# michelerenzullo/Blur_algorithms

Hardware: AMD Instinct MI355X
Metric: megapixels/sec Gaussian blur (σ=20, 4K RGB) at 1/2/4/8 GPUs; % HBM roofline (higher is better)
Workload: dtype f16 hi+lo operands (u8 pixels exact, taps and intermediate split in two binary16 halves), f32 accumulate

## Files before the change

### blur_algorithms_amd/_lib.py

```python
import ctypes as C
import os

_HERE = os.path.dirname(os.path.abspath(__file__))
LIB_PATH = os.environ.get("BLUR_AMD_LIB") or os.path.join(_HERE, "libblur_amd.so")

BLUR_OK = 0
ERR_NAMES = {1: "BLUR_ERR_INVALID", 2: "BLUR_ERR_UNSUPPORTED", 3: "BLUR_ERR_HIP", 4: "BLUR_ERR_NOMEM"}


class BlurError(RuntimeError):
    def __init__(self, code, msg):
        super().__init__("%s (%d): %s" % (ERR_NAMES.get(code, "BLUR_ERR"), code, msg))
        self.code = code


class BlurOpts(C.Structure):
    _fields_ = [("nyquist_quirk", C.c_int), ("col_group", C.c_int), ("force_generic", C.c_int), ("frames_per_launch", C.c_int),
                ("row_major_planes", C.c_int), ("engine", C.c_int), ("tile_points", C.c_int), ("reserved", C.c_int * 1)]


_P = C.c_void_p
SYMBOLS = {
    "blur_opts_default": (None, [C.POINTER(BlurOpts)]),
    "blur_gaussian_window": (C.c_int, [C.c_double, C.c_int]),
    "blur_get_gaussian": (C.c_int, [_P, C.c_double, C.c_int, C.c_int]),
    "blur_is_valid_size": (C.c_int, [C.c_int]),
    "blur_nearest_transform_size": (C.c_int, [C.c_int]),
    "blur_pffft_sizing": (C.c_int, [C.c_int, C.c_int, C.c_double, C.POINTER(C.c_int)]),
    "blur_kernel_multipliers": (C.c_int, [C.c_double, C.c_int, C.c_int, _P]),
    "blur_fft_plan_radices": (C.c_int, [C.c_int, C.POINTER(C.c_int)]),
    "blur_ctx_create": (C.c_int, [C.POINTER(_P), C.c_int]),
    "blur_ctx_destroy": (C.c_int, [_P]),
    "blur_ctx_set_stream": (C.c_int, [_P, _P]),
    "blur_ctx_synchronize": (C.c_int, [_P]),
    "blur_last_error": (C.c_char_p, [_P]),
    "blur_last_engine": (C.c_int, [_P, C.c_char_p, C.c_size_t]),
    "blur_ctx_timing_enable": (C.c_int, [_P, C.c_int]),
    "blur_ctx_timing": (C.c_int, [_P, C.POINTER(C.c_double), C.POINTER(C.c_int), C.POINTER(C.c_int), C.c_int]),
    "blur_gaussian_u8c3_dev": (C.c_int, [_P, _P, _P, C.c_int, C.c_int, C.c_double, C.POINTER(BlurOpts)]),
    "blur_gaussian_u8c3_batch_dev": (C.c_int, [_P, _P, _P, C.c_int, C.c_int, C.c_int, C.c_double, C.POINTER(BlurOpts)]),
    "blur_gaussian_f32c1_dev": (C.c_int, [_P, _P, _P, C.c_int, C.c_int, C.c_double, C.POINTER(BlurOpts)]),
    "blur_gaussian_u8c3_host": (C.c_int, [_P, _P, _P, C.c_int, C.c_int, C.c_double, C.POINTER(BlurOpts)]),
    "blur_gaussian_u8c3_host_batch": (C.c_int, [_P, _P, _P, C.c_int, C.c_int, C.c_int, C.c_double, C.POINTER(BlurOpts)]),
    "blur_gaussian_u8_batch_dev": (C.c_int, [_P, _P, _P, C.c_int, C.c_int, C.c_int, C.c_int, C.c_double, C.POINTER(BlurOpts)]),
    "blur_gaussian_u8_dev": (C.c_int, [_P, _P, _P, C.c_int, C.c_int, C.c_int, C.c_double, C.POINTER(BlurOpts)]),
    "blur_gaussian_u8_host": (C.c_int, [_P, _P, _P, C.c_int, C.c_int, C.c_int, C.c_double, C.POINTER(BlurOpts)]),
    "blur_gaussian_f32_batch_dev": (C.c_int, [_P, _P, _P, C.c_int, C.c_int, C.c_int, C.c_int, C.c_double, C.POINTER(BlurOpts)]),
    "blur_gaussian_f32_dev": (C.c_int, [_P, _P, _P, C.c_int, C.c_int, C.c_int, C.c_double, C.POINTER(BlurOpts)]),
    "blur_gaussian_f32_host": (C.c_int, [_P, _P, _P, C.c_int, C.c_int, C.c_int, C.c_double, C.POINTER(BlurOpts)]),
    "blur_gaussian_u16_batch_dev": (C.c_int, [_P, _P, _P, C.c_int, C.c_int, C.c_int, C.c_int, C.c_double, C.POINTER(BlurOpts)]),
    "blur_gaussian_u16_dev": (C.c_int, [_P, _P, _P, C.c_int, C.c_int, C.c_int, C.c_double, C.POINTER(BlurOpts)]),
    "blur_gaussian_u16_host": (C.c_int, [_P, _P, _P, C.c_int, C.c_int, C.c_int, C.c_double, C.POINTER(BlurOpts)]),
    "blur_gaussian_f16_batch_dev": (C.c_int, [_P, _P, _P, C.c_int, C.c_int, C.c_int, C.c_int, C.c_double, C.POINTER(BlurOpts)]),
    "blur_gaussian_f16_dev": (C.c_int, [_P, _P, _P, C.c_int, C.c_int, C.c_int, C.c_double, C.POINTER(BlurOpts)]),
    "blur_gaussian_f16_host": (C.c_int, [_P, _P, _P, C.c_int, C.c_int, C.c_int, C.c_double, C.POINTER(BlurOpts)]),
    "blur_gaussian_bf16_batch_dev": (C.c_int, [_P, _P, _P, C.c_int, C.c_int, C.c_int, C.c_int, C.c_double, C.POINTER(BlurOpts)]),
    "blur_gaussian_bf16_dev": (C.c_int, [_P, _P, _P, C.c_int, C.c_int, C.c_int, C.c_double, C.POINTER(BlurOpts)]),
    "blur_gaussian_bf16_host": (C.c_int, [_P, _P, _P, C.c_int, C.c_int, C.c_int, C.c_double, C.POINTER(BlurOpts)]),
    "blur_gaussian_u8c3_host_pitched": (C.c_int, [_P, _P, C.c_size_t, _P, C.c_size_t, C.c_int, C.c_int, C.c_double, C.POINTER(BlurOpts)]),
    "blur_gaussian_f32c1_host": (C.c_int, [_P, _P, _P, C.c_int, C.c_int, C.c_double, C.POINTER(BlurOpts)]),
    "blur_separable_u8c3_dev": (C.c_int, [_P, _P, _P, C.c_int, C.c_int, _P, C.c_int, C.c_int, C.POINTER(BlurOpts)]),
    "blur_boxfft_u8c3_dev": (C.c_int, [_P, _P, _P, C.c_int, C.c_int, C.c_double, C.POINTER(BlurOpts)]),
    "blur_boxfft_sizing": (C.c_int, [C.c_int, C.c_int, C.c_double, C.POINTER(C.c_int)]),
    "blur_box_kernel": (C.c_int, [_P, C.c_int, C.c_int]),
    "blur_rowpass_u8c3_dev": (C.c_int, [_P, _P, _P, C.c_int, C.c_int, C.c_double, C.POINTER(BlurOpts)]),
    "blur_pocketfft2d_sizing": (C.c_int, [C.c_int, C.c_int, C.c_double, C.POINTER(C.c_int * 8)]),
    "blur_pocketfft2d_u8c3_dev": (C.c_int, [_P, _P, _P, C.c_int, C.c_int, C.c_double, C.c_int, _P]),
    "blur_pocketfft2d_u8c3_host": (C.c_int, [_P, _P, _P, C.c_int, C.c_int, C.c_double, C.c_int]),
    "blur_reflect101_u8_dev": (C.c_int, [_P, _P, _P, C.c_int, C.c_int, C.c_int, C.c_int, C.c_int, C.c_int, C.c_int, C.POINTER(C.c_int * 2)]),
    "blur_flip_block_f32_dev": (C.c_int, [_P, _P, _P, C.c_int, C.c_int]),
    "blur_deinterleave_bgr_u8_f32_dev": (C.c_int, [_P, _P, _P, C.c_uint32]),
    "blur_interleave_bgr_f32_u8_dev": (C.c_int, [_P, _P, _P, C.c_uint32]),
    "blur_fastboxblur_u8_dev": (C.c_int, [_P, _P, C.c_int, C.c_int, C.c_int, C.c_int, C.c_int]),
    "blur_fastboxblur_u8_host": (C.c_int, [_P, _P, C.c_int, C.c_int, C.c_int, C.c_int, C.c_int]),
    "blur_fastboxblur_u8_batch_dev": (C.c_int, [_P, _P, C.c_int, C.c_int, C.c_int, C.c_int, C.c_int, C.c_int]),
    "blur_fastboxblur_u8_host_batch": (C.c_int, [_P, _P, C.c_int, C.c_int, C.c_int, C.c_int, C.c_int, C.c_int]),
    "blur_fastboxblur_batch_plan": (C.c_int, [C.c_int, C.c_int, C.c_int, C.c_int, C.c_int, C.c_int, C.POINTER(C.c_int * 4)]),
    "blur_multi_create": (C.c_int, [C.POINTER(_P), C.POINTER(C.c_int), C.c_int]),
    "blur_multi_destroy": (C.c_int, [_P]),
    "blur_multi_shards": (C.c_int, [_P]),
    "blur_multi_last_error": (C.c_char_p, [_P]),
    "blur_gaussian_u8c3_batch_multi_dev": (C.c_int, [_P, _P, _P, C.c_int, C.c_int, C.c_int, C.c_double, C.POINTER(BlurOpts)]),
    "blur_gaussian_u8c3_batch_multi_host": (C.c_int, [_P, _P, _P, C.c_int, C.c_int, C.c_int, C.c_double, C.POINTER(BlurOpts)]),
    "blur_gaussian_u8_batch_multi_dev": (C.c_int, [_P, _P, _P, C.c_int, C.c_int, C.c_int, C.c_int, C.c_double, C.POINTER(BlurOpts)]),
    "blur_gaussian_u8_batch_multi_host": (C.c_int, [_P, _P, _P, C.c_int, C.c_int, C.c_int, C.c_int, C.c_double, C.POINTER(BlurOpts)]),
    "blur_gaussian_f32_batch_multi_dev": (C.c_int, [_P, _P, _P, C.c_int, C.c_int, C.c_int, C.c_int, C.c_double, C.POINTER(BlurOpts)]),
    "blur_gaussian_f32_batch_multi_host": (C.c_int, [_P, _P, _P, C.c_int, C.c_int, C.c_int, C.c_int, C.c_double, C.POINTER(BlurOpts)]),
    "blur_gaussian_u16_batch_multi_dev": (C.c_int, [_P, _P, _P, C.c_int, C.c_int, C.c_int, C.c_int, C.c_double, C.POINTER(BlurOpts)]),
    "blur_gaussian_u16_batch_multi_host": (C.c_int, [_P, _P, _P, C.c_int, C.c_int, C.c_int, C.c_int, C.c_double, C.POINTER(BlurOpts)]),
    "blur_gaussian_f16_batch_multi_dev": (C.c_int, [_P, _P, _P, C.c_int, C.c_int, C.c_int, C.c_int, C.c_double, C.POINTER(BlurOpts)]),
    "blur_gaussian_f16_batch_multi_host": (C.c_int, [_P, _P, _P, C.c_int, C.c_int, C.c_int, C.c_int, C.c_double, C.POINTER(BlurOpts)]),
    "blur_gaussian_bf16_batch_multi_dev": (C.c_int, [_P, _P, _P, C.c_int, C.c_int, C.c_int, C.c_int, C.c_double, C.POINTER(BlurOpts)]),
    "blur_gaussian_bf16_batch_multi_host": (C.c_int, [_P, _P, _P, C.c_int, C.c_int, C.c_int, C.c_int, C.c_double, C.POINTER(BlurOpts)]),
    "blur_gaussian_u8_sigmas_batch_dev": (C.c_int, [_P, _P, _P, C.c_int, C.c_int, C.c_int, C.c_int, C.POINTER(C.c_double), C.POINTER(BlurOpts)]),
    "blur_gaussian_u8_sigmas_dev": (C.c_int, [_P, _P, _P, C.c_int, C.c_int, C.c_int, C.POINTER(C.c_double), C.POINTER(BlurOpts)]),
    "blur_gaussian_u8_sigmas_host": (C.c_int, [_P, _P, _P, C.c_int, C.c_int, C.c_int, C.POINTER(C.c_double), C.POINTER(BlurOpts)]),
    "blur_gaussian_u8_sigmas_batch_multi_dev": (C.c_int, [_P, _P, _P, C.c_int, C.c_int, C.c_int, C.c_int, C.POINTER(C.c_double), C.POINTER(BlurOpts)]),
    "blur_gaussian_u8_sigmas_batch_multi_host": (C.c_int, [_P, _P, _P, C.c_int, C.c_int, C.c_int, C.c_int, C.POINTER(C.c_double), C.POINTER(BlurOpts)]),
    "blur_gaussian_f32_sigmas_batch_dev": (C.c_int, [_P, _P, _P, C.c_int, C.c_int, C.c_int, C.c_int, C.POINTER(C.c_double), C.POINTER(BlurOpts)]),
    "blur_gaussian_f32_sigmas_dev": (C.c_int, [_P, _P, _P, C.c_int, C.c_int, C.c_int, C.POINTER(C.c_double), C.POINTER(BlurOpts)]),
    "blur_gaussian_f32_sigmas_host": (C.c_int, [_P, _P, _P, C.c_int, C.c_int, C.c_int, C.POINTER(C.c_double), C.POINTER(BlurOpts)]),
    "blur_gaussian_f32_sigmas_batch_multi_dev": (C.c_int, [_P, _P, _P, C.c_int, C.c_int, C.c_int, C.c_int, C.POINTER(C.c_double), C.POINTER(BlurOpts)]),
    "blur_gaussian_f32_sigmas_batch_multi_host": (C.c_int, [_P, _P, _P, C.c_int, C.c_int, C.c_int, C.c_int, C.POINTER(C.c_double), C.POINTER(BlurOpts)]),
    "blur_gaussian_u16_sigmas_batch_dev": (C.c_int, [_P, _P, _P, C.c_int, C.c_int, C.c_int, C.c_int, C.POINTER(C.c_double), C.POINTER(BlurOpts)]),
    "blur_gaussian_u16_sigmas_dev": (C.c_int, [_P, _P, _P, C.c_int, C.c_int, C.c_int, C.POINTER(C.c_double), C.POINTER(BlurOpts)]),
    "blur_gaussian_u16_sigmas_host": (C.c_int, [_P, _P, _P, C.c_int, C.c_int, C.c_int, C.POINTER(C.c_double), C.POINTER(BlurOpts)]),
    "blur_gaussian_u16_sigmas_batch_multi_dev": (C.c_int, [_P, _P, _P, C.c_int, C.c_int, C.c_int, C.c_int, C.POINTER(C.c_double), C.POINTER(BlurOpts)]),
    "blur_gaussian_u16_sigmas_batch_multi_host": (C.c_int, [_P, _P, _P, C.c_int, C.c_int, C.c_int, C.c_int, C.POINTER(C.c_double), C.POINTER(BlurOpts)]),
    "blur_gaussian_f16_sigmas_batch_dev": (C.c_int, [_P, _P, _P, C.c_int, C.c_int, C.c_int, C.c_int, C.POINTER(C.c_double), C.POINTER(BlurOpts)]),
    "blur_gaussian_f16_sigmas_dev": (C.c_int, [_P, _P, _P, C.c_int, C.c_int, C.c_int, C.POINTER(C.c_double), C.POINTER(BlurOpts)]),
    "blur_gaussian_f16_sigmas_host": (C.c_int, [_P, _P, _P, C.c_int, C.c_int, C.c_int, C.POINTER(C.c_double), C.POINTER(BlurOpts)]),
    "blur_gaussian_f16_sigmas_batch_multi_dev": (C.c_int, [_P, _P, _P, C.c_int, C.c_int, C.c_int, C.c_int, C.POINTER(C.c_double), C.POINTER(BlurOpts)]),
    "blur_gaussian_f16_sigmas_batch_multi_host": (C.c_int, [_P, _P, _P, C.c_int, C.c_int, C.c_int, C.c_int, C.POINTER(C.c_double), C.POINTER(BlurOpts)]),
    "blur_gaussian_bf16_sigmas_batch_dev": (C.c_int, [_P, _P, _P, C.c_int, C.c_int, C.c_int, C.c_int, C.POINTER(C.c_double), C.POINTER(BlurOpts)]),
    "blur_gaussian_bf16_sigmas_dev": (C.c_int, [_P, _P, _P, C.c_int, C.c_int, C.c_int, C.POINTER(C.c_double), C.POINTER(BlurOpts)]),
    "blur_gaussian_bf16_sigmas_host": (C.c_int, [_P, _P, _P, C.c_int, C.c_int, C.c_int, C.POINTER(C.c_double), C.POINTER(BlurOpts)]),
    "blur_gaussian_bf16_sigmas_batch_multi_dev": (C.c_int, [_P, _P, _P, C.c_int, C.c_int, C.c_int, C.c_int, C.POINTER(C.c_double), C.POINTER(BlurOpts)]),
    "blur_gaussian_bf16_sigmas_batch_multi_host": (C.c_int, [_P, _P, _P, C.c_int, C.c_int, C.c_int, C.c_int, C.POINTER(C.c_double), C.POINTER(BlurOpts)]),
    "blur_gaussian_sigmas_plan": (C.c_int, [C.c_int, C.c_int, C.c_int, C.POINTER(C.c_double), C.POINTER(C.c_int)]),
    "blur_fastboxblur_u8_batch_multi_dev": (C.c_int, [_P, _P, C.c_int, C.c_int, C.c_int, C.c_int, C.c_int, C.c_int]),
    "blur_fastboxblur_u8_batch_multi_host": (C.c_int, [_P, _P, C.c_int, C.c_int, C.c_int, C.c_int, C.c_int, C.c_int]),
    "blur_convolve_lines_c32_dev": (C.c_int, [_P, _P, _P, C.c_int, C.c_int, _P]),
    "blur_wr_length": (C.c_int, [C.c_int, C.c_int]),
    "blur_mx_window_blocks": (C.c_int, [C.c_int]),
    "blur_mx_fragments": (C.c_int, [_P, C.c_int, C.c_int, _P]),
    "blur_wr_kernel_multipliers": (C.c_int, [C.c_double, C.c_int, C.c_int, C.c_int, C.c_int, _P]),
    "blur_malloc": (C.c_int, [_P, C.POINTER(_P), C.c_size_t]),
    "blur_free": (C.c_int, [_P, _P]),
    "blur_host_alloc": (C.c_int, [_P, C.POINTER(_P), C.c_size_t]),
    "blur_host_free": (C.c_int, [_P, _P]),
    "blur_copy_bandwidth": (C.c_int, [_P, C.c_size_t, C.c_int, C.POINTER(C.c_double)]),
    "blur_memcpy_h2d": (C.c_int, [_P, _P, _P, C.c_size_t]),
    "blur_memcpy_d2h": (C.c_int, [_P, _P, _P, C.c_size_t]),
}

_lib = None


def load():
    global _lib
    if _lib is not None:
        return _lib
    if not os.path.exists(LIB_PATH):
        raise ImportError(
            "blur_algorithms_amd: %s is missing -- build it with `python -c 'import __graft_entry__ as g; g.build()'` "
            "or `make -C blur_algorithms_amd/csrc` (hipcc, --offload-arch=gfx950). There is no CPU fallback." % LIB_PATH)
    try:
        import torch
    except Exception:
        pass
    lib = C.CDLL(LIB_PATH)
    for name, (res, args) in SYMBOLS.items():
        fn = getattr(lib, name)
        fn.restype = res
        fn.argtypes = args
    _lib = lib
    return lib
```

### blur_algorithms_amd/csrc/engine.hip

```cpp
#include <hip/hip_runtime.h>

#include <array>
#include <cmath>
#include <cstdio>
#include <cstdlib>
#include <cstring>
#include <functional>
#include <list>
#include <map>
#include <memory>
#include <string>
#include <tuple>
#include <type_traits>
#include <vector>

#include "../../include/blur_amd.h"
#include "fast_registry.hpp"
#include "fft_engine.hpp"
#include "host_math.hpp"
#define BLUR_MX_QUIRK_KERNELS
#include "mx_registry.hpp"
#define BLUR_FX_QUIRK_KERNELS
#include "fx_registry.hpp"
#include "bx_box.hpp"
// ... 449 lines not shown
                stream((x - r - 1) * C, sh_out, gout);
#pragma unroll
                for (int k = 0; k < C; ++k) res[k] = 0;
#pragma unroll
                for (int k = 0; k < 4 * C; ++k) {
                    acc[k % C] += byte_of(gin, k) - byte_of(gout, k);
                    const uint32_t v = static_cast<uint32_t>(static_cast<int>(static_cast<float>(acc[k % C]) * iarr + 0.5f)) & 0xffu;
                    res[k >> 2] |= v << (8 * (k & 3));
                }
#pragma unroll
                for (int k = 0; k < C; ++k) d32[((off0 + x * C) >> 2) + k] = res[k];
            }
        }
        uint8_t* t = a; a = b; b = t;
    }
    __syncthreads();
    if ((rb & 3) == 0 && (reinterpret_cast<uintptr_t>(dst) & 3) == 0) {
        for (int i = threadIdx.x; i < rb / 4; i += 256) reinterpret_cast<uint32_t*>(dst)[i] = reinterpret_cast<const uint32_t*>(a + off0)[i];
    } else {
        for (int i = threadIdx.x; i < rb; i += 256) dst[i] = a[off0 + i];
    }
}


struct Img2dGeom { int rows, cols, s0, s1, top, left; };

__global__ __launch_bounds__(256) void img2d_rows_fwd_kernel(const uint8_t* __restrict__ src, float2* __restrict__ z, Img2dGeom g, int ca, int cb,
                                                             DevPlan plan, const float2* __restrict__ tw)
{
    extern __shared__ float2 lds2d[];
    const int zs = line_stride(plan.n);
    const int y = blockIdx.x;
    const uint8_t* row = src + static_cast<size_t>(refl101(y - g.top, g.rows)) * g.cols * 3;
    for (int x = threadIdx.x; x < g.s1; x += blockDim.x) {
        const uint8_t* px = row + 3 * refl101(x - g.left, g.cols);
        lds2d[phys(x)] = make_float2(static_cast<float>(px[ca]), cb >= 0 ? static_cast<float>(px[cb]) : 0.f);
    }
    __syncthreads();
    fft_forward_lines<1>(lds2d, zs, plan, tw);
    float2* out = z + static_cast<size_t>(y) * g.s1;
    for (int pos = threadIdx.x; pos < g.s1; pos += blockDim.x) out[pos] = lds2d[phys(pos)];
}

template <int G, bool CONV>
__global__ __launch_bounds__(256) void img2d_cols_kernel(float2* __restrict__ z, int s0, int s1, DevPlan plan, const float2* __restrict__ tw,
                                                         const float* __restrict__ mcol, const float* __restrict__ krow_pos)
{
    extern __shared__ float2 lds2d[];
    const int zs = line_stride(plan.n);
    const int x0 = blockIdx.x * G;
    for (int idx = threadIdx.x; idx < s0 * G; idx += blockDim.x) {
        const int y = idx / G, c = idx - y * G, x = x0 + c;
        float2 v = make_float2(0.f, 0.f);
        if (x < s1) {
            v = z[static_cast<size_t>(y) * s1 + x];
            if (CONV) v = cscale(v, krow_pos[x]);
        }
        lds2d[c * zs + phys(y)] = v;
    }
    __syncthreads();
    if (CONV) fftconv_lines<G>(lds2d, zs, plan, tw, mcol);
    else fft_forward_lines<G>(lds2d, zs, plan, tw);
    for (int idx = threadIdx.x; idx < s0 * G; idx += blockDim.x) {
        const int y = idx / G, c = idx - y * G, x = x0 + c;
        if (x < s1) z[static_cast<size_t>(y) * s1 + x] = lds2d[c * zs + phys(y)];
    }
}

__global__ __launch_bounds__(256) void img2d_rows_inv_kernel(const float2* __restrict__ z, uint8_t* __restrict__ dst, float* __restrict__ planes, Img2dGeom g,
                                                             int ca, int cb, DevPlan plan, const float2* __restrict__ tw)
{
    extern __shared__ float2 lds2d[];
    const int zs = line_stride(plan.n);
    const int i = blockIdx.x;
    const float2* in = z + static_cast<size_t>(i + g.top) * g.s1;
    for (int pos = threadIdx.x; pos < g.s1; pos += blockDim.x) lds2d[phys(pos)] = in[pos];
    __syncthreads();
    fft_inverse_lines<1>(lds2d, zs, plan, tw);
    const size_t plane = static_cast<size_t>(g.rows) * g.cols;
    for (int j = threadIdx.x; j < g.cols; j += blockDim.x) {
        const float2 v = lds2d[phys(j + g.left)];
        const size_t px = static_cast<size_t>(i) * g.cols + j;
        dst[3 * px + ca] = static_cast<uint8_t>(static_cast<int>(v.x + 0.5f));
        if (cb >= 0) dst[3 * px + cb] = static_cast<uint8_t>(static_cast<int>(v.y + 0.5f));
        if (planes) {
            planes[ca * plane + px] = v.x;
            if (cb >= 0) planes[cb * plane + px] = v.y;
        }
    }
}

__global__ __launch_bounds__(256) void img2d_logspec_kernel(const float2* __restrict__ z, uint8_t* __restrict__ dst, float* __restrict__ planes, Img2dGeom g,
                                                            int ca, int cb, const int* __restrict__ pos_of_freq_y, const int* __restrict__ pos_of_freq_x)
{
    const size_t plane = static_cast<size_t>(g.rows) * g.cols;
    for (size_t px = blockIdx.x * 256u + threadIdx.x; px < plane; px += static_cast<size_t>(gridDim.x) * 256u) {
        const int i = static_cast<int>(px / g.cols), j = static_cast<int>(px - static_cast<size_t>(i) * g.cols);
        const int row = i + g.top, col = j + g.left;
        const int fy = (row + (g.s0 % 2 == 0 ? g.s0 : g.s0 + 1) / 2) % g.s0;
        const int col_ = (col + (g.s1 % 2 == 0 ? g.s1 : g.s1 + 1) / 2) % g.s1;
        const int fx = col_ < g.s1 / 2 + 1 ? col_ : g.s1 / 2 - col_ % (g.s1 / 2);
        const float2 p = z[static_cast<size_t>(pos_of_freq_y[fy]) * g.s1 + pos_of_freq_x[fx]];
        const float2 q = z[static_cast<size_t>(pos_of_freq_y[(g.s0 - fy) % g.s0]) * g.s1 + pos_of_freq_x[(g.s1 - fx) % g.s1]];
        const float va = 20.f * log10f(fabsf(0.5f * (p.x + q.x)) + 0.00001f);
        dst[3 * px + ca] = static_cast<uint8_t>(static_cast<int>(va + 0.5f));
        if (planes) planes[ca * plane + px] = va;
        if (cb >= 0) {
            const float vb = 20.f * log10f(fabsf(0.5f * (p.y + q.y)) + 0.00001f);
            dst[3 * px + cb] = static_cast<uint8_t>(static_cast<int>(vb + 0.5f));
            if (planes) planes[cb * plane + px] = vb;
        }
    }
}

__global__ __launch_bounds__(256) void copy16_kernel(const uint4* __restrict__ src, uint4* __restrict__ dst, size_t n16)
{
    for (size_t i = blockIdx.x * 256ull + threadIdx.x; i < n16; i += static_cast<size_t>(gridDim.x) * 256ull) dst[i] = src[i];
}

__global__ __launch_bounds__(256) void reflect101_u8_kernel(const uint8_t* __restrict__ in, uint8_t* __restrict__ out, int rows, int cols, int C,
                                                            int top, int left, int out_rows, int out_cols)
{
    const size_t total = static_cast<size_t>(out_rows) * out_cols;
    for (size_t px = blockIdx.x * 256u + threadIdx.x; px < total; px += static_cast<size_t>(gridDim.x) * 256u) {
        const int y = static_cast<int>(px / out_cols), x = static_cast<int>(px - static_cast<size_t>(y) * out_cols);
        const uint8_t* s = in + (static_cast<size_t>(refl101(y - top, rows)) * cols + refl101(x - left, cols)) * C;
        for (int c = 0; c < C; ++c) out[px * C + c] = s[c];
    }
}

}

struct DevicePlan {
    FftPlan host;
    DevPlan dev{};
    float2* d_tw = nullptr;
    const FastEntry* fast = nullptr;
    int key = 0;
    int* d_pos_of_freq = nullptr;
};

struct HostPipe {
    static constexpr int S = 3;
    hipStream_t h2d = nullptr, d2h = nullptr;
    uint8_t* buf[S] = { nullptr, nullptr, nullptr };
    size_t bytes = 0;
    hipEvent_t in_done[S] = {}, comp_done[S] = {}, out_done[S] = {};
    bool ready = false;
};

struct MxTables {
    void* frags_row = nullptr;
    void* frags_col = nullptr;
    float* taps_row = nullptr;
    float dr = 0.f, dc = 0.f;
};

struct blur_ctx {
    int device = 0;
    HostPipe pipe;
    hipStream_t stream = nullptr;
    std::string err;
    std::map<int, std::unique_ptr<DevicePlan>> plans;
    std::map<std::tuple<int, int, int, uint64_t>, float*> spectra;
    std::map<int, float*> last_spectrum;
    int num_cus = 256;
    int num_xcds = 8;
    float2* d_w256 = nullptr;
    std::map<int, float2*> wr_tw0;
    std::map<std::tuple<int, int, int, int, uint64_t>, float*> wr_spectra;
    struct LinesTable { uint64_t hash; std::vector<float> host; float* dev; };
    std::list<LinesTable> lines_tables;
    std::map<std::tuple<int, int, int, int, int, uint64_t>, MxTables> mx_tables;
    uint8_t* fx_strips = nullptr;
    size_t fx_strips_bytes = 0;
    int* fx_sums = nullptr;
    size_t fx_sums_bytes = 0;
    int* tl_sums = nullptr;
    size_t tl_sums_bytes = 0;
    float* tl_terms = nullptr;
    size_t tl_terms_bytes = 0;
    uint8_t* tl_copy = nullptr;
    size_t tl_copy_bytes = 0;
    std::map<std::pair<uint64_t, int>, float*> tl_taps;
    int* mx_sums = nullptr;
    size_t mx_sums_bytes = 0;
    float* mx_terms = nullptr;
    size_t mx_terms_bytes = 0;
    float* work = nullptr;
    size_t work_bytes = 0;
    float* work2 = nullptr;
    size_t work2_bytes = 0;
    uint8_t* box_tmp = nullptr;
    float* ch_planes = nullptr;
    size_t ch_planes_bytes = 0;
    uint8_t* ch_copy = nullptr;
    size_t ch_copy_bytes = 0;
    void* ff_sums = nullptr;
    size_t ff_sums_bytes = 0;
    void* ff_strips = nullptr;
    size_t ff_strips_bytes = 0;
    size_t box_bytes = 0;
    std::string engine_note;
    int last_family = -1;
    void* host_stage = nullptr;
    size_t host_stage_bytes = 0;
    int timing = 0;
    std::vector<std::tuple<hipEvent_t, hipEvent_t, int, int>> ev_busy;
    std::vector<std::pair<hipEvent_t, hipEvent_t>> ev_free;
    double ms[2] = { 0, 0 };
    int launches[2] = { 0, 0 };
    int frames[2] = { 0, 0 };
};

static thread_local std::string g_create_err;

#define HIP_TRY(ctx, call)                                                                          \
    do {                                                                                            \
        hipError_t e_ = (call);                                                                     \
        if (e_ != hipSuccess) {                                                                     \
            (ctx)->err = std::string(#call) + ": " + hipGetErrorString(e_);                         \
            return BLUR_ERR_HIP;                                                                    \
        }                                                                                           \
    } while (0)

static int fail(blur_ctx* ctx, int code, const char* msg)
{
    if (ctx) ctx->err = msg;
    return code;
}

static int get_plan(blur_ctx* ctx, int n, bool want_fast, bool column_role, DevicePlan** out)
{
    const FastEntry* fe = want_fast ? find_fast_entry(n, column_role) : nullptr;
    const int key = 4 * n + (fe ? (column_role ? 2 : 1) : 0);
    auto it = ctx->plans.find(key);
    if (it != ctx->plans.end()) { *out = it->second.get(); return BLUR_OK; }
    auto dp = std::make_unique<DevicePlan>();
    dp->fast = fe;
    dp->key = key;
    const bool ok = fe ? make_plan_radices(n, fe->radix, fe->npass, dp->host) : make_plan(n, dp->host);
    if (!ok) return fail(ctx, BLUR_ERR_UNSUPPORTED, "FFT length is not 2^a 3^b 5^c");
    dp->dev.n = n;
    dp->dev.npass = dp->host.npass;
    for (int i = 0; i < dp->host.npass; ++i) {
        dp->dev.radix[i] = dp->host.radix[i];
        dp->dev.m[i] = dp->host.m[i];
        dp->dev.tw_off[i] = dp->host.tw_off[i];
    }
    const size_t bytes = std::max<size_t>(dp->host.tw.size() * sizeof(float), 16);
    HIP_TRY(ctx, hipMalloc(reinterpret_cast<void**>(&dp->d_tw), bytes));
    if (!dp->host.tw.empty())
        HIP_TRY(ctx, hipMemcpy(dp->d_tw, dp->host.tw.data(), dp->host.tw.size() * sizeof(float), hipMemcpyHostToDevice));
    *out = dp.get();
    ctx->plans[key] = std::move(dp);
    return BLUR_OK;
}

static int get_spectrum(blur_ctx* ctx, const DevicePlan& plan, double sigma, int ksize, bool quirk, float** out)
{
    uint64_t bits;
    std::memcpy(&bits, &sigma, sizeof bits);
    const auto key = std::make_tuple(plan.key, ksize, quirk ? 1 : 0, bits);
    auto it = ctx->spectra.find(key);
    if (it != ctx->spectra.end()) { *out = it->second; return BLUR_OK; }
    const int n = plan.dev.n;
    std::vector<float> m(n / 2 + 1), mp(n);
    kernel_multipliers(sigma, ksize, n, m.data());
    permuted_multipliers(plan.host, m.data(), quirk, mp.data());
    float* d = nullptr;
    HIP_TRY(ctx, hipMalloc(reinterpret_cast<void**>(&d), sizeof(float) * (n + kStampTailFloats)));
    HIP_TRY(ctx, hipMemset(d, 0, sizeof(float) * (n + kStampTailFloats)));
    HIP_TRY(ctx, hipMemcpy(d, mp.data(), sizeof(float) * n, hipMemcpyHostToDevice));
    ctx->spectra[key] = d;
    ctx->last_spectrum[plan.key] = d;
    *out = d;
    return BLUR_OK;
}

static int get_spectrum_custom(blur_ctx* ctx, const DevicePlan& plan, const std::vector<float>& karr, bool quirk, float** out)
{
    uint64_t h = 1469598103934665603ull;
    const unsigned char* bytes = reinterpret_cast<const unsigned char*>(karr.data());
    for (size_t i = 0; i < karr.size() * sizeof(float); ++i) { h ^= bytes[i]; h *= 1099511628211ull; }
    const auto key = std::make_tuple(plan.key, -1, quirk ? 1 : 0, h);
    auto it = ctx->spectra.find(key);
    if (it != ctx->spectra.end()) { *out = it->second; return BLUR_OK; }
    const int n = plan.dev.n;
    std::vector<float> m(n / 2 + 1), mp(n);
    kernel_multipliers_from_array(karr.data(), n, m.data());
    permuted_multipliers(plan.host, m.data(), quirk, mp.data());
    float* d = nullptr;
    HIP_TRY(ctx, hipMalloc(reinterpret_cast<void**>(&d), sizeof(float) * (n + kStampTailFloats)));
    HIP_TRY(ctx, hipMemset(d, 0, sizeof(float) * (n + kStampTailFloats)));
    HIP_TRY(ctx, hipMemcpy(d, mp.data(), sizeof(float) * n, hipMemcpyHostToDevice));
    ctx->spectra[key] = d;
    ctx->last_spectrum[plan.key] = d;
    *out = d;
    return BLUR_OK;
}

static int ensure_host_stage(blur_ctx* ctx, size_t bytes, void** out)
{
    if (ctx->host_stage_bytes < bytes) {
        if (ctx->host_stage) { HIP_TRY(ctx, hipStreamSynchronize(ctx->stream)); HIP_TRY(ctx, hipFree(ctx->host_stage)); ctx->host_stage = nullptr; ctx->host_stage_bytes = 0; }
        HIP_TRY(ctx, hipMalloc(&ctx->host_stage, bytes ? bytes : 1));
// ... 120 lines not shown
        if (int rc = set_lds(ctx, colpass_kernel<OutT, CH, C, 512>, lds)) return rc;
        hipLaunchKernelGGL((colpass_kernel<OutT, CH, C, 512>), dim3(grid), dim3(512), lds, ctx->stream, planes, dst, rows, cols, pad, dv, plan.d_tw, mperm, strips);
    } else {
        if (int rc = set_lds(ctx, colpass_kernel<OutT, CH, C>, lds)) return rc;
        hipLaunchKernelGGL((colpass_kernel<OutT, CH, C>), dim3(grid), dim3(kThreads), lds, ctx->stream, planes, dst, rows, cols, pad, dv, plan.d_tw, mperm, strips);
    }
    HIP_TRY(ctx, hipGetLastError());
    return BLUR_OK;
}

static int colpass_lines(int n, int rows, int col_group, int obpp)
{
    int C = col_group > 0 ? col_group / 2 : 4;
    if (C >= 8) C = 8; else if (C >= 4) C = 4; else if (C >= 2) C = 2; else C = 1;
    while (C > 1 && col_lds_bytes(n, C, rows, obpp) > kLdsLimit) C /= 2;
    return col_lds_bytes(n, C, rows, obpp) > kLdsLimit ? 0 : C;
}

template <typename OutT, int CH>
static int launch_colpass(blur_ctx* ctx, const float* planes, OutT* dst, int rows, int cols, int pad,
                          const DevicePlan& plan, const float* mperm, int col_group, int strips = 0)
{
    const int C = colpass_lines(plan.dev.n, rows, col_group, sizeof(OutT) == 1 ? CH : 0);
    if (!C) return fail(ctx, BLUR_ERR_UNSUPPORTED, "column FFT length exceeds LDS capacity");
    switch (C) {
    case 8: return launch_colpass_c<OutT, CH, 8>(ctx, planes, dst, rows, cols, pad, plan, mperm, strips);
    case 4: return launch_colpass_c<OutT, CH, 4>(ctx, planes, dst, rows, cols, pad, plan, mperm, strips);
    case 2: return launch_colpass_c<OutT, CH, 2>(ctx, planes, dst, rows, cols, pad, plan, mperm, strips);
    default: return launch_colpass_c<OutT, CH, 1>(ctx, planes, dst, rows, cols, pad, plan, mperm, strips);
    }
}

struct Prepared {
    Sizing sz;
    DevicePlan *row = nullptr, *col = nullptr;
    float *m_row = nullptr, *m_col = nullptr;
    int col_group = 0;
    int col_fast_c = 0;
    int tile_w = 0;
    size_t frame_elems = 0;
    int gen_gshift = 0;
    const WrEntry *wr_col = nullptr, *wr_row = nullptr;
    float2 *wr_tw0_col = nullptr, *wr_tw0_row = nullptr;
    float *wr_m_col = nullptr, *wr_m_row = nullptr;
    const MxEntry* mx = nullptr;
    const FxEntry* fx = nullptr;
    const MxTables* mxt = nullptr;
    int mx_vpitch = 0;
    bool mx_quirk = false;
    struct Span { int in0, in1, padmode, v0, v1; };
    std::vector<Span> bands, tiles;
    const WrEntry *tl_col = nullptr;
    std::vector<const WrEntry*> tl_row;
    std::vector<float*> tl_m_row;
    std::vector<float2*> tl_tw0_row;
    float* tl_m_col = nullptr;
    float2* tl_tw0_col = nullptr;
    float tl_dr = 0.f, tl_dc = 0.f;
    float* tl_taps = nullptr;
    bool tiled = false, tl_quirk = false;
};

struct CustomKernel {
    const float* taps = nullptr;
    int ksize = 0;
    int pad = 0;
    int box_klen = 0;
};

static int wr_get_tables(blur_ctx* ctx, const WrEntry* e, float2** tw0)
{
    if (!ctx->d_w256) {
        std::vector<float> w(512);
        wr_w256(w.data());
        HIP_TRY(ctx, hipMalloc(reinterpret_cast<void**>(&ctx->d_w256), w.size() * sizeof(float)));
        HIP_TRY(ctx, hipMemcpy(ctx->d_w256, w.data(), w.size() * sizeof(float), hipMemcpyHostToDevice));
    }
    auto it = ctx->wr_tw0.find(e->r0);
    if (it == ctx->wr_tw0.end()) {
        std::vector<float> t(static_cast<size_t>(e->r0 - 1) * kWrS * 2 + 2);
        wr_tw0(e->r0, t.data());
        float2* d = nullptr;
        HIP_TRY(ctx, hipMalloc(reinterpret_cast<void**>(&d), t.size() * sizeof(float)));
        HIP_TRY(ctx, hipMemcpy(d, t.data(), t.size() * sizeof(float), hipMemcpyHostToDevice));
        it = ctx->wr_tw0.emplace(e->r0, d).first;
    }
    *tw0 = it->second;
    return BLUR_OK;
}

static int wr_get_spectrum(blur_ctx* ctx, const std::tuple<int, int, int, int, uint64_t>& key, const std::vector<float>& karr, int n, int n_ref, bool quirk, float** out)
{
    auto it = ctx->wr_spectra.find(key);
    if (it != ctx->wr_spectra.end()) { *out = it->second; return BLUR_OK; }
    std::vector<float> m(n);
    wr_multipliers(karr.data(), n, n_ref, quirk, m.data());
    float* d = nullptr;
    HIP_TRY(ctx, hipMalloc(reinterpret_cast<void**>(&d), sizeof(float) * (n + kWrStampTailFloats)));
    HIP_TRY(ctx, hipMemset(d, 0, sizeof(float) * (n + kWrStampTailFloats)));
    HIP_TRY(ctx, hipMemcpy(d, m.data(), sizeof(float) * n, hipMemcpyHostToDevice));
    ctx->wr_spectra[key] = d;
    ctx->last_spectrum[-n] = d;
    *out = d;
    return BLUR_OK;
}

static uint64_t fnv1a(const void* data, size_t bytes)
{
    uint64_t h = 1469598103934665603ull;
    const unsigned char* b = static_cast<const unsigned char*>(data);
    for (size_t i = 0; i < bytes; ++i) { h ^= b[i]; h *= 1099511628211ull; }
    return h;
}

static int mx_get_tables(blur_ctx* ctx, int nkb, double sigma, const Sizing& sz, const CustomKernel* ck, const MxTables** out, bool quiet = false)
{
    auto refuse = [&](int code, const char* msg) { return quiet ? code : fail(ctx, code, msg); };
    const int pad = sz.pad;
    std::vector<float> karr[2];
    const int nn[2] = { sz.n_row, sz.n_col };
    uint64_t tag;
    int kkey;
    auto build_arrays = [&]() -> int {
        for (int ax = 0; ax < 2; ++ax) {
            const int n = nn[ax];
            if (ck) {
                karr[ax].assign(n, 0.f);
                if (ck->box_klen > 0) box_kernel_1d(karr[ax].data(), ck->box_klen, n);
                else {
                    if (ck->ksize > n) return refuse(BLUR_ERR_INVALID, "kernel longer than the padded line");
                    const int c = ck->ksize / 2;
                    for (int t = 0; t < ck->ksize; ++t) karr[ax][(t - c + n) % n] += ck->taps[t];
                }
            } else {
                karr[ax].assign(std::max(n, sz.kSize), 0.f);
                get_gaussian(karr[ax].data(), sigma, sz.kSize, n);
            }
        }
        return BLUR_OK;
    };
    if (ck) {
        if (int rc = build_arrays()) return rc;
        kkey = -1;
        tag = fnv1a(karr[0].data(), nn[0] * sizeof(float)) ^ (fnv1a(karr[1].data(), nn[1] * sizeof(float)) * 3);
    } else { kkey = sz.kSize; std::memcpy(&tag, &sigma, sizeof tag); }
    const auto key = std::make_tuple(kkey, pad, nkb, nn[0], nn[1], tag);
    auto it = ctx->mx_tables.find(key);
    if (it != ctx->mx_tables.end()) { *out = &it->second; return BLUR_OK; }
    if (!ck) { if (int rc = build_arrays()) return rc; }
    MxTables t;
    auto release = [&]() {
        if (t.frags_row) (void)hipFree(t.frags_row);
        if (t.frags_col) (void)hipFree(t.frags_col);
        if (t.taps_row) (void)hipFree(t.taps_row);
    };
    for (int ax = 0; ax < 2; ++ax) {
        const int n = nn[ax];
        std::vector<float> taps(2 * pad + 1);
        for (int k = -pad; k <= pad; ++k) taps[k + pad] = karr[ax][(k + n) % n];
        for (int i = pad + 1; i < n - pad; ++i)
            if (karr[ax][i] != 0.f) { release(); return refuse(BLUR_ERR_UNSUPPORTED, "matrix-core engine: kernel wider than 2 pad + 1"); }
        {
            double sum = 0;
            bool neg = false;
            for (float t : taps) { sum += t; neg = neg || t < 0.f; }
            if (neg || sum > 1.0005) { release(); return refuse(BLUR_ERR_UNSUPPORTED, "matrix-core engine: taps must be non-negative with sum <= 1"); }
        }
        std::vector<uint16_t> fr(static_cast<size_t>(2) * nkb * 512);
        mx_fragments(taps.data(), pad, nkb, fr.data());
        long double k0 = 0, kalt = 0;
        for (int i = 0; i < n; ++i) { k0 += karr[ax][i]; kalt += (i & 1) ? -static_cast<long double>(karr[ax][i]) : static_cast<long double>(karr[ax][i]); }
        const float scaler = 1.f / n;
        const float m0 = static_cast<float>(k0) * scaler, mh = static_cast<float>(kalt) * scaler;
        void* dfr = nullptr;
        hipError_t e = hipMalloc(&dfr, fr.size() * sizeof(uint16_t));
        if (e == hipSuccess) {
            (ax ? t.frags_col : t.frags_row) = dfr;
            e = hipMemcpy(dfr, fr.data(), fr.size() * sizeof(uint16_t), hipMemcpyHostToDevice);
        }
        if (e == hipSuccess && ax == 0) {
            e = hipMalloc(reinterpret_cast<void**>(&t.taps_row), taps.size() * sizeof(float));
            if (e == hipSuccess) e = hipMemcpy(t.taps_row, taps.data(), taps.size() * sizeof(float), hipMemcpyHostToDevice);
        }
        if (e != hipSuccess) {
            release();
            (void)hipGetLastError();
            if (!quiet) ctx->err = std::string("matrix-core tables: ") + hipGetErrorString(e);
            return BLUR_ERR_HIP;
        }
        (ax ? t.dc : t.dr) = m0 - mh;
    }
    *out = &(ctx->mx_tables[key] = t);
    return BLUR_OK;
}

struct FftFamilyChoice {
    const WrEntry* wc = nullptr;
    const WrEntry* wr = nullptr;
    bool fits = false;
    bool old_both = false;
    bool wr_pays = false;
};
static FftFamilyChoice fft_family_choice(int rows, int cols, const Sizing& sz)
{
    FftFamilyChoice c;
    c.wc = find_wr_entry(rows + 2 * sz.pad, true);
    c.wr = find_wr_entry(cols + 2 * sz.pad, false);
    c.old_both = find_fast_entry(sz.n_col, true) && find_fast_entry(sz.n_row, false);
    c.fits = c.wc && c.wr && c.wc->col_lds(rows) <= kLdsLimit && c.wr->row_lds(cols) <= kLdsLimit;
    if (c.fits) {
        const int need_c = rows + 2 * sz.pad, need_r = cols + 2 * sz.pad, nc = c.wc->r0 * kWrS, nr = c.wr->r0 * kWrS;
        c.wr_pays = c.old_both ? (c.wc->r0 >= 8 && c.wr->r0 >= 12 && 4 * need_c >= 3 * nc && 4 * need_r >= 3 * nr) : (2 * need_c >= nc && 2 * need_r >= nr);
    }
    return c;
}

static bool plan_spans(int len, int pad, int nmax, int in_max, int align, std::vector<Prepared::Span>& out, bool equal_middle = false, bool edge_max = false)
{
    out.clear();
    if (in_max > nmax) in_max = nmax;
    if (len + 2 * pad <= nmax && len <= in_max) { out.push_back({ 0, len, pad, 0, len }); return true; }
    const int halo = (pad + align - 1) / align * align;
    const int le = std::min(nmax - 2 * pad, in_max), lm = in_max;
    int ve = (le - halo) / align * align, vm = (lm - halo - pad) / align * align;
    if (ve <= 0 || vm <= 0) return false;
    int nsp0 = 2;
    if (len > 2 * ve) nsp0 += (len - 2 * ve + vm - 1) / vm;
    std::vector<int> b;
    int nsp = 0, sm_equal = 0;
    for (int tries = 0; tries < 4 && nsp == 0; ++tries) {
        const int n = nsp0 + tries;
        b.assign(n + 1, 0);
        b[n] = len;
        int e = edge_max ? ve : static_cast<int>(static_cast<long long>(len) / n) / align * align;
        if (e > ve) e = ve;
        if (2 * e >= len) e = (len / 2) / align * align;
        if (e < align) e = align;
        b[1] = e;
        const int rest = len - 2 * e;
        if (equal_middle && n > 2) {
            const int unit = align % 2 == 0 ? align : 2 * align;
            const int sm = ((rest + (n - 2) - 1) / (n - 2) + unit - 1) / unit * unit;
            if (sm > vm || e + (n - 2) * sm + pad > len) continue;
            for (int i = 2; i < n; ++i) b[i] = e + (i - 1) * sm;
            b[n - 1] = len - e;
            if (b[n - 1] <= b[n - 2] - sm) continue;
            nsp = n;
            sm_equal = sm;
            break;
        }
        for (int i = 2; i < n; ++i) b[i] = (e + static_cast<int>(static_cast<long long>(rest) * (i - 1) / (n - 2))) / align * align;
        b[n - 1] = std::max(b[n - 1], (len - ve + align - 1) / align * align);
        bool ok = len - b[n - 1] <= ve && len - b[n - 1] > 0 && b[1] <= ve;
        for (int i = 1; i < n && ok; ++i) ok = b[i] > b[i - 1];
        for (int i = 1; i + 1 < n && ok; ++i) ok = b[i + 1] - b[i] <= vm;
        if (ok) nsp = n;
    }
    if (nsp == 0) return false;
    for (int i = 0; i < nsp; ++i) {
        Prepared::Span sp;
        sp.v0 = b[i];
        sp.v1 = b[i + 1];
        if (i == 0) { sp.in0 = 0; sp.in1 = std::min(len, sp.v1 + pad); sp.padmode = pad; }
        else if (i == nsp - 1) { sp.in0 = sp.v0 - halo; sp.in1 = len; sp.padmode = pad; }
        else {
            if (sm_equal > 0) sp.v1 = sp.v0 + sm_equal;
            sp.in0 = sp.v0 - halo; sp.in1 = std::min(len, sp.v1 + pad); sp.padmode = 0;
        }
        if (sp.in0 < 0 || sp.in1 - sp.in0 + 2 * sp.padmode > nmax || sp.in1 - sp.in0 > in_max || sp.padmode > sp.in1 - sp.in0 - 1) return false;
        out.push_back(sp);
    }
    return true;
}

static float quirk_gain(const float* karr, int n)
{
    long double k0 = 0, kalt = 0;
    for (int i = 0; i < n; ++i) { k0 += karr[i]; kalt += (i & 1) ? -static_cast<long double>(karr[i]) : static_cast<long double>(karr[i]); }
    const float scaler = 1.f / n;
    return static_cast<float>(k0) * scaler - static_cast<float>(kalt) * scaler;
}

static int plan_tiled(blur_ctx* ctx, int rows, int cols, double sigma, bool quirk, int tile_points, Prepared& p)
{
    const int pad = p.sz.pad;
    long long best = -1;
    for (int r0 : { 16, 15, 12, 10, 9, 8, 6, 5, 4, 3 }) {
        const int n = r0 * kWrS;
        if (tile_points > 0 && n > tile_points) continue;
        const WrEntry* e = find_wr_entry(n, true);
        if (!e || e->r0 != r0) continue;
        int in_max = n;
        while (in_max > 0 && e->col_lds(in_max) > kLdsLimit) in_max -= 8;
        std::vector<Prepared::Span> sp;
        if (in_max <= 0 || !plan_spans(rows, pad, n, in_max, 1, sp, true)) continue;
        const long long cost = static_cast<long long>(sp.size()) * n;
        if (best < 0 || cost < best) { best = cost; p.bands = sp; p.tl_col = e; }
    }
    if (best < 0) return BLUR_ERR_UNSUPPORTED;
    best = -1;
    for (int r0 : { 16, 15, 12, 10, 9, 8, 6, 5, 4, 3 }) {
        const int n = r0 * kWrS;
        if (tile_points > 0 && n > tile_points) continue;
        const WrEntry* e = find_wr_entry(n, false);
        if (!e || e->r0 != r0) continue;
        int in_max = n;
        while (in_max > 0 && e->row_lds(in_max) > kLdsLimit) in_max -= 16;
        if (in_max <= 0) continue;
        for (int variant = 0; variant < 2; ++variant) {
            std::vector<Prepared::Span> sp;
            if (!plan_spans(cols, pad, n, in_max, 16, sp, false, variant == 1)) continue;
            long long cost = 0;
            for (const Prepared::Span& t : sp) {
                const WrEntry* te = find_wr_entry(t.in1 - t.in0 + 2 * t.padmode, false);
                cost += te ? te->r0 * kWrS : 1 << 20;
            }
            if (best < 0 || cost < best) { best = cost; p.tiles = sp; }
        }
    }
    if (best < 0) return BLUR_ERR_UNSUPPORTED;
    uint64_t bits;
    std::memcpy(&bits, &sigma, sizeof bits);
    auto spectrum = [&](int n, float** out) -> int {
        const auto key = std::make_tuple(n, 0, p.sz.kSize, 0, bits);
        std::vector<float> karr(n, 0.f);
        if (ctx->wr_spectra.find(key) == ctx->wr_spectra.end()) {
            std::vector<float> k(std::max(n, p.sz.kSize));
            get_gaussian(k.data(), sigma, p.sz.kSize, n);
            std::copy(k.begin(), k.begin() + n, karr.begin());
        }
        return wr_get_spectrum(ctx, key, karr, n, n, false, out);
// ... 738 lines not shown
    }
    ctx->last_family = note.empty() ? 6 : 0;
    ctx->engine_note = note;
    return BLUR_OK;
}

template <typename T>
static int blur_ch_sigmas_host(blur_ctx* ctx, const T* src, T* dst, int rows, int cols, int channels, const double* sigmas, const blur_opts* opts)
{
    SigmaGroups sg;
    if (int rc = check_ch_sigmas_args(ctx, src, dst, 1, rows, cols, channels, sigmas, sg)) return rc;
    HIP_TRY(ctx, hipSetDevice(ctx->device));
    const size_t bytes = static_cast<size_t>(rows) * cols * channels * sizeof(T), half = (bytes + 255) & ~static_cast<size_t>(255);
    void* dv = nullptr;
    if (int rc0 = ensure_host_stage(ctx, 2 * half, &dv)) return rc0;
    char* d = static_cast<char*>(dv);
    int rc = BLUR_OK;
    hipError_t e = hipMemcpyAsync(d, src, bytes, hipMemcpyHostToDevice, ctx->stream);
    if (e == hipSuccess) rc = blur_ch_sigmas_batch_impl(ctx, reinterpret_cast<const T*>(d), reinterpret_cast<T*>(d + half), 1, rows, cols, channels, sigmas, opts);
    if (e == hipSuccess && rc == BLUR_OK) e = hipMemcpyAsync(dst, d + half, bytes, hipMemcpyDeviceToHost, ctx->stream);
    if (e == hipSuccess) e = hipStreamSynchronize(ctx->stream);
    if (e != hipSuccess) { ctx->err = std::string("host blur: ") + hipGetErrorString(e); return BLUR_ERR_HIP; }
    return rc;
}

static int get_pos_of_freq(blur_ctx* ctx, DevicePlan* dp, const int** out)
{
    if (!dp->d_pos_of_freq) {
        const int n = dp->dev.n;
        std::vector<int> inv(n);
        for (int pos = 0; pos < n; ++pos) inv[dp->host.freq_of_pos[pos]] = pos;
        HIP_TRY(ctx, hipMalloc(reinterpret_cast<void**>(&dp->d_pos_of_freq), sizeof(int) * n));
        HIP_TRY(ctx, hipMemcpy(dp->d_pos_of_freq, inv.data(), sizeof(int) * n, hipMemcpyHostToDevice));
    }
    *out = dp->d_pos_of_freq;
    return BLUR_OK;
}

template <bool CONV>
static int launch_img2d_cols(blur_ctx* ctx, float2* z, int s0, int s1, const DevicePlan& plan, const float* mcol, const float* krow_pos)
{
    const size_t line = static_cast<size_t>(line_stride(s0)) * sizeof(float2);
    int G = 8;
    while (G > 1 && G * line > kLdsLimit) G >>= 1;
    if (G * line > kLdsLimit) return fail(ctx, BLUR_ERR_UNSUPPORTED, "2D path: column FFT length exceeds LDS capacity");
    const int grid = (s1 + G - 1) / G;
#define BLUR_IMG2D_COLS(G_)                                                                                                        \
    case G_:                                                                                                                        \
        if (int rc = set_lds(ctx, img2d_cols_kernel<G_, CONV>, G_ * line)) return rc;                                              \
        hipLaunchKernelGGL((img2d_cols_kernel<G_, CONV>), dim3(grid), dim3(kThreads), G_ * line, ctx->stream, z, s0, s1, plan.dev, \
                           plan.d_tw, mcol, krow_pos);                                                                             \
        break;
    switch (G) {
        BLUR_IMG2D_COLS(8)
        BLUR_IMG2D_COLS(4)
        BLUR_IMG2D_COLS(2)
        BLUR_IMG2D_COLS(1)
    }
#undef BLUR_IMG2D_COLS
    HIP_TRY(ctx, hipGetLastError());
    return BLUR_OK;
}

extern "C" {

void blur_opts_default(blur_opts* o)
{
    if (!o) return;
    std::memset(o, 0, sizeof *o);
    o->nyquist_quirk = 1;
}

int blur_gaussian_window(double sigma, int max_width) { return gaussian_window(sigma, max_width); }

int blur_get_gaussian(float* kernel, double sigma, int width, int fft_length)
{
    if (!kernel || !(sigma > 0) || width < 0 || fft_length < 0) return BLUR_ERR_INVALID;
    get_gaussian(kernel, sigma, width, fft_length);
    return BLUR_OK;
}

int blur_is_valid_size(int n) { return is_valid_size(n); }
int blur_nearest_transform_size(int n) { return nearest_transform_size(n); }

int blur_pffft_sizing(int rows, int cols, double sigma, int out[6])
{
    if (!out || rows <= 0 || cols <= 0 || !(sigma > 0)) return BLUR_ERR_INVALID;
    const Sizing s = pffft_sizing(rows, cols, sigma);
    out[0] = s.kSize; out[1] = s.pad; out[2] = s.n_col; out[3] = s.n_row; out[4] = s.tz_col; out[5] = s.tz_row;
    return BLUR_OK;
}

int blur_kernel_multipliers(double sigma, int ksize, int n, float* m)
{
    if (!m || !(sigma > 0) || ksize <= 0 || n < ksize) return BLUR_ERR_INVALID;
    kernel_multipliers(sigma, ksize, n, m);
    return BLUR_OK;
}

int blur_wr_kernel_multipliers(double sigma, int ksize, int n, int n_ref, int quirk, float* m)
{
    if (!m || !(sigma > 0) || ksize <= 0 || n < ksize || (n & 1) || n_ref <= 0) return BLUR_ERR_INVALID;
    std::vector<float> k(std::max(n, ksize));
    get_gaussian(k.data(), sigma, ksize, n);
    wr_multipliers(k.data(), n, n_ref, quirk != 0, m);
    return BLUR_OK;
}

int blur_fft_plan_radices(int n, int* radices)
{
    FftPlan p;
    if (!radices || !make_plan(n, p)) return 0;
    for (int i = 0; i < p.npass; ++i) radices[i] = p.radix[i];
    return p.npass;
}

int blur_ctx_create(blur_ctx** out, int device)
{
    if (!out) return BLUR_ERR_INVALID;
    *out = nullptr;
    int count = 0;
    hipError_t e = hipGetDeviceCount(&count);
    if (e != hipSuccess || count <= 0) {
        g_create_err = std::string("no HIP device available: ") + (e != hipSuccess ? hipGetErrorString(e) : "device count is 0");
        return BLUR_ERR_HIP;
    }
    if (device < 0 || device >= count) { g_create_err = "device ordinal out of range"; return BLUR_ERR_INVALID; }
    e = hipSetDevice(device);
    if (e != hipSuccess) { g_create_err = std::string("hipSetDevice: ") + hipGetErrorString(e); return BLUR_ERR_HIP; }
    blur_ctx* c = new blur_ctx();
    c->device = device;
    hipDeviceProp_t prop;
    if (hipGetDeviceProperties(&prop, device) == hipSuccess && prop.multiProcessorCount > 0) c->num_cus = prop.multiProcessorCount;
    int xccs = 0;
    if (hipDeviceGetAttribute(&xccs, hipDeviceAttributeNumberOfXccs, device) == hipSuccess && xccs > 0) c->num_xcds = xccs;
    *out = c;
    return BLUR_OK;
}

int blur_ctx_destroy(blur_ctx* ctx)
{
    if (!ctx) return BLUR_ERR_INVALID;
    (void)hipSetDevice(ctx->device);
    (void)hipStreamSynchronize(ctx->stream);
    for (auto& kv : ctx->plans) {
        if (kv.second->d_tw) (void)hipFree(kv.second->d_tw);
        if (kv.second->d_pos_of_freq) (void)hipFree(kv.second->d_pos_of_freq);
    }
    for (auto& kv : ctx->spectra) (void)hipFree(kv.second);
    if (ctx->d_w256) (void)hipFree(ctx->d_w256);
    for (auto& kv : ctx->wr_tw0) (void)hipFree(kv.second);
    for (auto& kv : ctx->wr_spectra) (void)hipFree(kv.second);
    for (auto& kv : ctx->mx_tables) {
        (void)hipFree(kv.second.frags_row); (void)hipFree(kv.second.frags_col);
        (void)hipFree(kv.second.taps_row);
    }
    for (auto& lt : ctx->lines_tables) (void)hipFree(lt.dev);
    if (ctx->fx_strips) (void)hipFree(ctx->fx_strips);
    if (ctx->fx_sums) (void)hipFree(ctx->fx_sums);
    if (ctx->tl_sums) (void)hipFree(ctx->tl_sums);
    if (ctx->tl_terms) (void)hipFree(ctx->tl_terms);
    if (ctx->tl_copy) (void)hipFree(ctx->tl_copy);
    for (auto& kv : ctx->tl_taps) (void)hipFree(kv.second);
    if (ctx->mx_sums) (void)hipFree(ctx->mx_sums);
    if (ctx->mx_terms) (void)hipFree(ctx->mx_terms);
    if (ctx->work) (void)hipFree(reinterpret_cast<char*>(ctx->work) - kWorkGuard);
    if (ctx->work2) (void)hipFree(ctx->work2);
    if (ctx->box_tmp) (void)hipFree(ctx->box_tmp);
    if (ctx->ch_planes) (void)hipFree(ctx->ch_planes);
    if (ctx->ch_copy) (void)hipFree(ctx->ch_copy);
    if (ctx->ff_sums) (void)hipFree(ctx->ff_sums);
    if (ctx->ff_strips) (void)hipFree(ctx->ff_strips);
    if (ctx->host_stage) (void)hipFree(ctx->host_stage);
    if (ctx->pipe.ready) {
        (void)hipStreamSynchronize(ctx->pipe.h2d);
        (void)hipStreamSynchronize(ctx->pipe.d2h);
        for (int k = 0; k < HostPipe::S; ++k) {
            if (ctx->pipe.buf[k]) (void)hipFree(ctx->pipe.buf[k]);
            (void)hipEventDestroy(ctx->pipe.in_done[k]);
            (void)hipEventDestroy(ctx->pipe.comp_done[k]);
            (void)hipEventDestroy(ctx->pipe.out_done[k]);
        }
        (void)hipStreamDestroy(ctx->pipe.h2d);
        (void)hipStreamDestroy(ctx->pipe.d2h);
    }
    for (auto& t : ctx->ev_busy) { (void)hipEventDestroy(std::get<0>(t)); (void)hipEventDestroy(std::get<1>(t)); }
    for (auto& t : ctx->ev_free) { (void)hipEventDestroy(t.first); (void)hipEventDestroy(t.second); }
    delete ctx;
    return BLUR_OK;
}

int blur_ctx_set_stream(blur_ctx* ctx, void* hip_stream)
{
    if (!ctx) return BLUR_ERR_INVALID;
    hipStream_t next = static_cast<hipStream_t>(hip_stream);
    if (next != ctx->stream) {
        HIP_TRY(ctx, hipSetDevice(ctx->device));
        HIP_TRY(ctx, hipStreamSynchronize(ctx->stream));
        ctx->stream = next;
    }
    return BLUR_OK;
}

int blur_ctx_synchronize(blur_ctx* ctx)
{
    if (!ctx) return BLUR_ERR_INVALID;
    HIP_TRY(ctx, hipStreamSynchronize(ctx->stream));
    return BLUR_OK;
}

const char* blur_last_error(const blur_ctx* ctx) { return ctx ? ctx->err.c_str() : g_create_err.c_str(); }

int blur_ctx_timing_enable(blur_ctx* ctx, int on)
{
    if (!ctx) return BLUR_ERR_INVALID;
    ctx->timing = on == 2 ? 2 : on != 0 ? 1 : 0;
    return BLUR_OK;
}

int blur_ctx_timing(blur_ctx* ctx, double out_ms[2], int out_launches[2], int out_frames[2], int reset)
{
    if (!ctx) return BLUR_ERR_INVALID;
    if (int rc = timing_drain(ctx)) return rc;
    for (int i = 0; i < 2; ++i) {
        if (out_ms) out_ms[i] = ctx->ms[i];
        if (out_launches) out_launches[i] = ctx->launches[i];
        if (out_frames) out_frames[i] = ctx->frames[i];
        if (reset) { ctx->ms[i] = 0; ctx->launches[i] = 0; ctx->frames[i] = 0; }
    }
    return BLUR_OK;
}

static int run_mx_u8c3(blur_ctx* ctx, const uint8_t* d_src, uint8_t* d_dst, int nframes, int rows, int cols, int chunk, const Prepared& p)
{
    const size_t px = static_cast<size_t>(rows) * cols;
    MxGeom g{ rows, cols, p.sz.pad, p.mx_vpitch, 0, 0, mx_vrows(rows, p.mx->nkb), ctx->num_xcds };
    const int chunks = (cols + kMxRowChunk - 1) / kMxRowChunk, rblocks = g.vrows / 32, zblocks = (g.vrows + 255) / 256;
    const size_t n_spart = static_cast<size_t>(chunks) * rows * 3, n_vpart = static_cast<size_t>(rblocks) * g.vpitch,
                 n_qrow = static_cast<size_t>(3) * g.vrows, n_qcol = g.vpitch, n_zpart = static_cast<size_t>(zblocks) * 3;
    const size_t sums_bytes = n_spart * sizeof(int) * chunk;
    const size_t terms_bytes = ((n_vpart + n_qrow + n_qcol) * sizeof(float) + n_zpart * sizeof(double)) * chunk + 64;
    if (p.mx_quirk) {
        if (ctx->mx_sums_bytes < sums_bytes) {
            if (ctx->mx_sums) { HIP_TRY(ctx, hipStreamSynchronize(ctx->stream)); HIP_TRY(ctx, hipFree(ctx->mx_sums)); ctx->mx_sums = nullptr; ctx->mx_sums_bytes = 0; }
            HIP_TRY(ctx, hipMalloc(reinterpret_cast<void**>(&ctx->mx_sums), sums_bytes));
            ctx->mx_sums_bytes = sums_bytes;
        }
        if (ctx->mx_terms_bytes < terms_bytes) {
            if (ctx->mx_terms) { HIP_TRY(ctx, hipStreamSynchronize(ctx->stream)); HIP_TRY(ctx, hipFree(ctx->mx_terms)); ctx->mx_terms = nullptr; ctx->mx_terms_bytes = 0; }
            HIP_TRY(ctx, hipMalloc(reinterpret_cast<void**>(&ctx->mx_terms), terms_bytes));
            ctx->mx_terms_bytes = terms_bytes;
        }
    }
    for (int f = 0; f < nframes; f += chunk) {
        const int nf = nframes - f < chunk ? nframes - f : chunk;
        const uint8_t* s = d_src + static_cast<size_t>(f) * px * 3;
        uint8_t* d = d_dst + static_cast<size_t>(f) * px * 3;
        g.nframes = nf;
        g.aligned = ((cols & 3) == 0 && (reinterpret_cast<uintptr_t>(s) & 3) == 0) ? 1 : 0;
        int* spart = nullptr;
        float *vpart = nullptr, *qrow = nullptr, *qcol = nullptr;
        double* zpart = nullptr;
        if (p.mx_quirk) {
            spart = ctx->mx_sums;
            zpart = reinterpret_cast<double*>(ctx->mx_terms);
            vpart = reinterpret_cast<float*>(zpart + n_zpart * nf);
            qrow = vpart + n_vpart * nf;
            qcol = qrow + n_qrow * nf;
        }
        { TimedLaunch t(ctx, 0, nf);
          HIP_TRY(ctx, p.mx->row_u8(ctx->stream, s, ctx->work, p.mxt->frags_row, g, ctx->num_cus, spart, vpart)); }
        if (p.mx_quirk) {
            hipLaunchKernelGGL(mx_quirk_rows, dim3(zblocks, nf), dim3(256), 0, ctx->stream, spart, qrow, zpart, g, chunks, 8 * (p.mx->nkb - 2), p.mxt->dr);
            HIP_TRY(ctx, hipGetLastError());
            hipLaunchKernelGGL(mx_quirk_cols, dim3((g.vpitch + 255) / 256, nf), dim3(256), 0, ctx->stream, vpart, zpart, qcol, g, rblocks, zblocks, p.mxt->dr, p.mxt->dc);
            HIP_TRY(ctx, hipGetLastError());
        }
        { TimedLaunch t(ctx, 1, nf);
          HIP_TRY(ctx, p.mx->col_u8(ctx->stream, ctx->work, d, p.mxt->frags_col, g, qcol, ctx->num_cus, qrow)); }
    }
    return BLUR_OK;
}

static int run_fx_u8c3(blur_ctx* ctx, const uint8_t* d_src, uint8_t* d_dst, int nframes, int rows, int cols, const Prepared& p, float* vdump = nullptr, FwChSel chsel = 0)
{
    const size_t px = static_cast<size_t>(rows) * cols;
    const uint8_t* lo = d_src < d_dst ? d_src : d_dst;
    const uint8_t* hi = d_src < d_dst ? d_dst : d_src;
    if (static_cast<size_t>(hi - lo) < px * 3 * nframes) {
        const size_t cap = std::max<size_t>(1, (static_cast<size_t>(1) << 30) / (px * 3));
        if (d_src == d_dst && static_cast<size_t>(nframes) > cap) {
            for (int f0 = 0; f0 < nframes; f0 += static_cast<int>(cap)) {
                const int nf = std::min<int>(static_cast<int>(cap), nframes - f0);
                if (int rc = run_fx_u8c3(ctx, d_src + static_cast<size_t>(f0) * px * 3, d_dst + static_cast<size_t>(f0) * px * 3, nf, rows, cols, p, vdump, chsel)) return rc;
            }
            return BLUR_OK;
        }
        if (int rc = ensure_work(ctx, px * 3 * nframes)) return rc;
        HIP_TRY(ctx, hipMemcpyAsync(ctx->work, d_src, px * 3 * nframes, hipMemcpyDeviceToDevice, ctx->stream));
        d_src = reinterpret_cast<const uint8_t*>(ctx->work);
    }
    const int nkb = p.fx->nkb, pada = 8 * (nkb - 2);
    FxGeom g{ rows, cols, p.sz.pad, nframes, 0, (rows + 31) / 32, fx_right_strips(cols, pada), ctx->num_xcds };
    g.aligned = ((cols & 3) == 0 && (reinterpret_cast<uintptr_t>(d_src) & 3) == 0 && (reinterpret_cast<uintptr_t>(d_dst) & 3) == 0) ? 1 : 0;
    {
        const int win = kFxChunk + 2 * pada, nstrips = fx_left_strips(pada) + g.nright;
        const size_t bytes = static_cast<size_t>(nframes) * nstrips * rows * win * 3 + 64;
        if (ctx->fx_strips_bytes < bytes) {
            if (ctx->fx_strips) { HIP_TRY(ctx, hipStreamSynchronize(ctx->stream)); HIP_TRY(ctx, hipFree(ctx->fx_strips)); ctx->fx_strips = nullptr; ctx->fx_strips_bytes = 0; }
            HIP_TRY(ctx, hipMalloc(reinterpret_cast<void**>(&ctx->fx_strips), bytes));
            ctx->fx_strips_bytes = bytes;
        }
    }
    const int chunks_x = (cols + kFxChunk - 1) / kFxChunk, narrow =
#ifdef FX_FULL_STRIPS
        0;
#else
        p.fx->nkb <= 11 && !chsel ? 1 : 0;
#endif
    int strip_groups = (kFxChunk + 2 * pada) / 4;
    if (narrow) {
        const int gpr = strip_groups, per = (gpr + 7) / 8, nleft = fx_left_strips(pada);
        strip_groups = 0;
        for (int si = 0; si < nleft + g.nright; ++si) {
            int lo, hi;
            fx_strip_range(si < nleft ? si : chunks_x - g.nright + si - nleft, cols, pada, per, &lo, &hi);
            strip_groups = std::max(strip_groups, std::min(8 * hi, gpr) - 8 * lo);
        }
        if (strip_groups < 1) strip_groups = 1;
    }
    const int strip_blocks = (((rows + 3) / 4) * strip_groups + 255) / 256;
    const int n_strip = strip_blocks * (fx_left_strips(pada) + g.nright) * nframes;
    FxQuirk qk{};
    if (!p.mx_quirk) {
        TimedLaunch t(ctx, 1, nframes);
        hipLaunchKernelGGL(fx_prepass<1>, dim3(n_strip), dim3(256), 0, ctx->stream, d_src, nullptr, nullptr, nullptr, ctx->fx_strips, rows, cols, p.sz.pad, pada, 1, 1, 0, chunks_x,
                           g.nright, strip_blocks, kFxSumRows, narrow);
        HIP_TRY(ctx, hipGetLastError());
    }
    if (p.mx_quirk) {
        const int gpt = fx_groups_per_thread(cols);
        const int groups = (cols + 3) / 4;
        const int band_rows = fx_band_rows(rows, cols, nframes, ctx->num_cus), nbands = (rows + band_rows - 1) / band_rows, nbatches = (groups + 256 * gpt - 1) / (256 * gpt);
        auto up4 = [](size_t v) { return (v + 3) & ~static_cast<size_t>(3); };
        const size_t n_srow = up4(static_cast<size_t>(nframes) * nbatches * rows * 3), n_cpart = up4(static_cast<size_t>(nframes) * nbands * 12 * groups);
        const size_t n_z = static_cast<size_t>(nframes) * nbands * nbatches * 3;
        const size_t bytes = (n_srow + n_cpart) * sizeof(int) + n_z * sizeof(long long) + 64;
        if (ctx->fx_sums_bytes < bytes) {
            if (ctx->fx_sums) { HIP_TRY(ctx, hipStreamSynchronize(ctx->stream)); HIP_TRY(ctx, hipFree(ctx->fx_sums)); ctx->fx_sums = nullptr; ctx->fx_sums_bytes = 0; }
            HIP_TRY(ctx, hipMalloc(reinterpret_cast<void**>(&ctx->fx_sums), bytes + bytes / 8));
            ctx->fx_sums_bytes = bytes + bytes / 8;
        }
        int* srow = ctx->fx_sums;
        int* cpart = srow + n_srow;
        long long* zpart = reinterpret_cast<long long*>(cpart + n_cpart);
        { TimedLaunch t(ctx, 1, nframes);
          const int n_alt = nbands * nbatches * nframes;
          auto kern = gpt == 1 ? fx_prepass<1> : (gpt == 2 ? fx_prepass<2> : fx_prepass<4>);
          hipLaunchKernelGGL(kern, dim3(n_alt + n_strip), dim3(256), 0, ctx->stream, d_src, srow, cpart, zpart, ctx->fx_strips, rows, cols, p.sz.pad, pada, nbands,
                             nbatches, n_alt, chunks_x, g.nright, strip_blocks, band_rows, narrow);
          HIP_TRY(ctx, hipGetLastError()); }
        qk.srow_part = srow;
        qk.cpart = cpart;
        qk.zpart = zpart;
        qk.taps = p.mxt->taps_row;
        qk.nbatches = nbatches;
        qk.nbands = nbands;
        qk.cpitch = 12 * groups;
        qk.dr = p.mxt->dr;
        qk.dc = p.mxt->dc;
    }
    unsigned long long* stamps = nullptr;
    if (!p.mx_quirk && !vdump && std::getenv("BLUR_FX_STAMPS")) {
        HIP_TRY(ctx, hipMalloc(reinterpret_cast<void**>(&stamps), 64));
        HIP_TRY(ctx, hipMemset(stamps, 0, 64));
    }
    if (chsel) {
        const Fw3Entry* fe3 = find_fw3_entry(nkb);
        if (!fe3 || vdump || stamps) return fail(ctx, BLUR_ERR_UNSUPPORTED, "fused kernel for a subset of three channels: no kernel instantiated for this pad");
        TimedLaunch t(ctx, 0, nframes);
        HIP_TRY(ctx, fe3->blur_u8(ctx->stream, d_src, d_dst, p.mxt->frags_row, g, ctx->num_cus, p.mx_quirk ? &qk : nullptr, ctx->fx_strips, chsel));
        return BLUR_OK;
    }
    { TimedLaunch t(ctx, 0, nframes);
      HIP_TRY(ctx, p.fx->blur_u8(ctx->stream, d_src, d_dst, p.mxt->frags_row, g, ctx->num_cus, p.mx_quirk ? &qk : nullptr, ctx->fx_strips, vdump, stamps)); }
    if (stamps) {
        unsigned long long h[8];
        HIP_TRY(ctx, hipStreamSynchronize(ctx->stream));
        HIP_TRY(ctx, hipMemcpy(h, stamps, 64, hipMemcpyDeviceToHost));
        HIP_TRY(ctx, hipFree(stamps));
        if (h[7]) {
            std::fprintf(stderr, "fx stamps: steps %llu, cycles per step: A0 %.0f B0 %.0f A1 %.0f B1 %.0f A2 %.0f B2 %.0f, whole task %.0f per step\n", h[7], h[0] / double(h[7]),
                         h[1] / double(h[7]), h[2] / double(h[7]), h[3] / double(h[7]), h[4] / double(h[7]), h[5] / double(h[7]), h[6] / double(h[7]));
        }
    }
    return BLUR_OK;
}

static bool bands_overlap(const uint8_t* lo, const uint8_t* hi, size_t bytes) { return static_cast<size_t>(hi - lo) < bytes; }

static int run_wr_tiled(blur_ctx* ctx, const uint8_t* d_src, uint8_t* d_dst, int nframes, int rows, int cols, const Prepared& p)
{
    const size_t px = static_cast<size_t>(rows) * cols, fb = px * 3;
    const int pad = p.sz.pad;
    const int groups = (cols + 3) / 4, gpt = 1;
    if (p.tl_quirk && cols < 4) return fail(ctx, BLUR_ERR_UNSUPPORTED, "tiled wave-resident path: image narrower than 4 pixels (the quirk's pre-pass)");
    const int pitch = (cols + 7) & ~7;
    int *srow = nullptr, *cpart = nullptr;
    long long* zpart = nullptr;
    float *e = nullptr, *h = nullptr;
    int band_rows = 0, nbands = 0, nbatches = 0;
    if (p.tl_quirk) {
        band_rows = static_cast<long long>(rows) * cols < 4000000ll ? 16 : kFxSumRows;
        while (band_rows < 256 && static_cast<long long>((groups + 255) / 256) * ((rows + 2 * band_rows - 1) / (2 * band_rows)) >= 4ll * ctx->num_cus) band_rows *= 2;
        nbands = (rows + band_rows - 1) / band_rows;
        nbatches = (groups + 256 * gpt - 1) / (256 * gpt);
        auto up4 = [](size_t v) { return (v + 3) & ~static_cast<size_t>(3); };
        const size_t n_srow = up4(static_cast<size_t>(nbatches) * rows * 3), n_cpart = up4(static_cast<size_t>(nbands) * 12 * groups);
        const size_t n_z = static_cast<size_t>(nbands) * nbatches * 3;
        const size_t bytes = (n_srow + n_cpart) * sizeof(int) + n_z * sizeof(long long) + 64;
        if (ctx->tl_sums_bytes < bytes) {
            if (ctx->tl_sums) { HIP_TRY(ctx, hipStreamSynchronize(ctx->stream)); HIP_TRY(ctx, hipFree(ctx->tl_sums)); ctx->tl_sums = nullptr; ctx->tl_sums_bytes = 0; }
            HIP_TRY(ctx, hipMalloc(reinterpret_cast<void**>(&ctx->tl_sums), bytes));
            ctx->tl_sums_bytes = bytes;
        }
        srow = ctx->tl_sums;
        cpart = srow + n_srow;
        zpart = reinterpret_cast<long long*>(cpart + n_cpart);
        const size_t tbytes = (static_cast<size_t>(3) * pitch + static_cast<size_t>(3) * rows) * sizeof(float) + 64;
        if (ctx->tl_terms_bytes < tbytes) {
            if (ctx->tl_terms) { HIP_TRY(ctx, hipStreamSynchronize(ctx->stream)); HIP_TRY(ctx, hipFree(ctx->tl_terms)); ctx->tl_terms = nullptr; ctx->tl_terms_bytes = 0; }
            HIP_TRY(ctx, hipMalloc(reinterpret_cast<void**>(&ctx->tl_terms), tbytes));
            ctx->tl_terms_bytes = tbytes;
        }
        e = ctx->tl_terms;
        h = e + static_cast<size_t>(3) * pitch;
    }
    for (int f = 0; f < nframes; ++f) {
        const uint8_t* src = d_src + static_cast<size_t>(f) * fb;
        uint8_t* dst = d_dst + static_cast<size_t>(f) * fb;
        const uint8_t* lo = src < dst ? src : dst;
        const uint8_t* hi = src < dst ? dst : src;
        if (bands_overlap(lo, hi, fb) && (p.bands.size() > 1 || p.tiles.size() > 1 || src == dst)) {
            if (ctx->tl_copy_bytes < fb) {
                if (ctx->tl_copy) { HIP_TRY(ctx, hipStreamSynchronize(ctx->stream)); HIP_TRY(ctx, hipFree(ctx->tl_copy)); ctx->tl_copy = nullptr; ctx->tl_copy_bytes = 0; }
                HIP_TRY(ctx, hipMalloc(reinterpret_cast<void**>(&ctx->tl_copy), fb));
                ctx->tl_copy_bytes = fb;
            }
            HIP_TRY(ctx, hipMemcpyAsync(ctx->tl_copy, src, fb, hipMemcpyDeviceToDevice, ctx->stream));
            src = ctx->tl_copy;
        }
        if (p.tl_quirk) {
            TimedLaunch t(ctx, 1, 1);
            const int n_alt = nbands * nbatches;
            hipLaunchKernelGGL(fx_prepass<1>, dim3(n_alt), dim3(256), 0, ctx->stream, src, srow, cpart, zpart, nullptr, rows, cols, pad, 0, nbands, nbatches, n_alt, 1, 0, 1, band_rows, 0);
            HIP_TRY(ctx, hipGetLastError());
            const int ne = (pitch + 255) / 256, nh = (rows + 255) / 256;
            const size_t lds = (static_cast<size_t>(3) * (256 + 2 * pad) + (2 * pad + 1) + 3 + 3 * 256) * sizeof(double);
            if (lds > 64 * 1024) HIP_TRY(ctx, hipFuncSetAttribute(reinterpret_cast<const void*>(tl_terms_kernel), hipFuncAttributeMaxDynamicSharedMemorySize, static_cast<int>(lds)));
            hipLaunchKernelGGL(tl_terms_kernel, dim3(ne + nh, 1), dim3(256), lds, ctx->stream, srow, cpart, zpart, p.tl_taps, e, h, rows, cols, pad, pitch, nbatches, nbands,
                               12 * groups, p.tl_dr, p.tl_dc, ne);
            HIP_TRY(ctx, hipGetLastError());
        }
        auto group_of = [&](size_t bi, int& step) -> int {
            const Prepared::Span& b = p.bands[bi];
            const int brows = b.in1 - b.in0;
            int nb = 1;
            step = 0;
            if (b.padmode == 0) {
                while (bi + nb < p.bands.size()) {
                    const Prepared::Span& c = p.bands[bi + nb];
                    const int st = c.in0 - p.bands[bi + nb - 1].in0;
                    if (c.padmode != 0 || c.in1 - c.in0 != brows || c.v0 - c.in0 != b.v0 - b.in0 || c.v1 - c.v0 != b.v1 - b.v0 || (st & 1) || (nb > 1 && st != step)) break;
                    step = st;
                    ++nb;
                }
            }
            if (nb > 1 && wr_frame_floats(brows, cols, b.padmode, p.tl_col->g) * nb * sizeof(float) > (static_cast<size_t>(3) << 30)) { nb = 1; step = 0; }
            return nb;
        };
        {
            size_t need = 0;
            for (size_t bi = 0; bi < p.bands.size();) {
                int step;
                const int nb = group_of(bi, step);
                need = std::max(need, wr_frame_floats(p.bands[bi].in1 - p.bands[bi].in0, cols, p.bands[bi].padmode, p.tl_col->g) * nb * sizeof(float));
                bi += nb;
            }
            if (int rc = ensure_work(ctx, need)) return rc;
        }
        float* const inter = reinterpret_cast<float*>(ctx->work);
        for (size_t bi = 0; bi < p.bands.size();) {
            const Prepared::Span& b = p.bands[bi];
            const int brows = b.in1 - b.in0;
            int step = 0;
            const int nb = group_of(bi, step);
            const int vr_max = bi + nb < p.bands.size() ? p.bands[bi + nb].v0 : rows;
            WrColTerm term;
            if (p.tl_quirk) {
                term.e = e;
                term.pitch = pitch;
                term.sign = ((b.in0 + pad - b.padmode) & 1) ? -1.f : 1.f;
            }
            term.band_step = nb > 1 ? step : 0;
            { TimedLaunch t(ctx, 1, 1);
              HIP_TRY(ctx, p.tl_col->col_u8(ctx->stream, src + static_cast<size_t>(b.in0) * cols * 3, inter, brows, cols, b.padmode, nb, ctx->num_cus, ctx->d_w256, p.tl_tw0_col,
                                            p.tl_m_col, term)); }
            const int g = p.tl_col->g, npairs = wr_npairs(brows, b.padmode), strips_full = (cols + g - 1) / g;
            for (size_t ti = 0; ti < p.tiles.size(); ++ti) {
                const Prepared::Span& t = p.tiles[ti];
                WrRowTile tile;
                tile.h = p.tl_quirk ? h : nullptr;
                tile.rows_full = rows;
                tile.row_base = b.in0;
                tile.vr0 = b.v0;
                tile.vr1 = b.v1;
                tile.ypar = b.padmode & 1;
                tile.dst_pitch = cols * 3;
                tile.dst_x0 = t.in0;
                tile.vc0 = t.v0 - t.in0;
                tile.vc1 = t.v1 - t.in0;
                tile.xpar = (t.in0 + pad) & 1;
                tile.plane_strips = strips_full;
                tile.g = g;
                tile.t0 = (b.v0 - b.in0 + tile.ypar) >> 1;
                tile.tn = ((b.v1 - 1 - b.in0 + tile.ypar) >> 1) - tile.t0 + 1;
                tile.band_step = nb > 1 ? step : 0;
                tile.vr_max = vr_max;
                if (nb == 1 && tile.vr1 > vr_max) tile.vr1 = vr_max;
                TimedLaunch tl(ctx, 0, 1);
                HIP_TRY(ctx, p.tl_row[ti]->row_u8(ctx->stream, inter + static_cast<size_t>(t.in0 / g) * npairs * (2 * g), dst, brows, t.in1 - t.in0, t.padmode, nb, ctx->num_cus,
                                                  ctx->d_w256, p.tl_tw0_row[ti], p.tl_m_row[ti], tile));
            }
            bi += nb;
        }
    }
    return BLUR_OK;
}

static int blur_u8c3_batch_impl(blur_ctx* ctx, const uint8_t* d_src, uint8_t* d_dst, int nframes,
                                int rows, int cols, double sigma, const blur_opts* opts, const CustomKernel* ck)
{
    if (!ctx) return BLUR_ERR_INVALID;
    if (!d_src || !d_dst || nframes < 0) return fail(ctx, BLUR_ERR_INVALID, "null frame pointer or negative frame count");
    Prepared p;
    const bool aligned = ((reinterpret_cast<uintptr_t>(d_src) | reinterpret_cast<uintptr_t>(d_dst)) & 3) == 0;
    if (int rc = prepare(ctx, rows, cols, sigma, opts, p, true, ck, true, aligned)) return rc;
    const size_t px = static_cast<size_t>(rows) * cols;
    if (p.fx) {
        if (nframes == 0) return BLUR_OK;
        ctx->last_family = 6;
        return run_fx_u8c3(ctx, d_src, d_dst, nframes, rows, cols, p);
    }
    if (p.tiled) {
        if (nframes == 0) return BLUR_OK;
        ctx->last_family = 7;
        return run_wr_tiled(ctx, d_src, d_dst, nframes, rows, cols, p);
    }
    int chunk = opts && opts->frames_per_launch > 0 ? opts->frames_per_launch : static_cast<int>((1024u << 20) / (p.frame_elems * sizeof(float)));
    if (chunk < 1) chunk = 1;
    if (chunk > nframes) chunk = nframes;
    if (nframes == 0) return BLUR_OK;
    if (int rc = ensure_work(ctx, p.frame_elems * sizeof(float) * chunk)) return rc;
    ctx->last_family = p.mx ? 4 : p.wr_col ? 2 : ((p.row->fast && p.col->fast) ? 1 : 0);
    if (p.mx) return run_mx_u8c3(ctx, d_src, d_dst, nframes, rows, cols, chunk, p);
    for (int f = 0; f < nframes; f += chunk) {
        const int nf = nframes - f < chunk ? nframes - f : chunk;
        const uint8_t* s = d_src + static_cast<size_t>(f) * px * 3;
        uint8_t* d = d_dst + static_cast<size_t>(f) * px * 3;
        if (p.wr_col) {
            { TimedLaunch t(ctx, 1, nf);
              HIP_TRY(ctx, p.wr_col->col_u8(ctx->stream, s, ctx->work, rows, cols, p.sz.pad, nf, ctx->num_cus, ctx->d_w256, p.wr_tw0_col, p.wr_m_col, WrColTerm{})); }
            { TimedLaunch t(ctx, 0, nf);
              WrRowTile whole;
              whole.g = p.wr_col->g;
              HIP_TRY(ctx, p.wr_row->row_u8(ctx->stream, ctx->work, d, rows, cols, p.sz.pad, nf, ctx->num_cus, ctx->d_w256, p.wr_tw0_row, p.wr_m_row, whole)); }
            continue;
        }
        if (int rc = run_rowpass_u8c3(ctx, s, ctx->work, rows, cols, nf, p, p.tile_w)) return rc;
        if (int rc = run_colpass_u8c3(ctx, ctx->work, d, rows, cols, nf, p)) return rc;
    }
    return BLUR_OK;
}

int blur_gaussian_u8c3_batch_dev(blur_ctx* ctx, const uint8_t* d_src, uint8_t* d_dst, int nframes,
                                 int rows, int cols, double sigma, const blur_opts* opts)
{
    return blur_u8c3_batch_impl(ctx, d_src, d_dst, nframes, rows, cols, sigma, opts, nullptr);
}

int blur_separable_u8c3_dev(blur_ctx* ctx, const uint8_t* d_src, uint8_t* d_dst, int rows, int cols,
                            const float* taps, int ksize, int pad, const blur_opts* opts)
{
    if (!ctx) return BLUR_ERR_INVALID;
    if (!taps || ksize <= 0 || (ksize & 1) == 0 || pad < 0) return fail(ctx, BLUR_ERR_INVALID, "separable kernel: odd tap count and pad >= 0 required");
    for (int t = 0; t < ksize / 2; ++t)
        if (taps[t] != taps[ksize - 1 - t]) return fail(ctx, BLUR_ERR_UNSUPPORTED, "separable kernel must be symmetric (real spectrum, Source.cpp:419)");
    CustomKernel ck;
    ck.taps = taps; ck.ksize = ksize; ck.pad = pad;
    return blur_u8c3_batch_impl(ctx, d_src, d_dst, 1, rows, cols, 0., opts, &ck);
}

int blur_boxfft_sizing(int rows, int cols, double nsmooth, int out[4])
{
    if (!out || rows <= 1 || cols <= 1 || !(nsmooth >= 1)) return BLUR_ERR_INVALID;
    int klen, pad;
    boxfft_sizing(rows, cols, nsmooth, klen, pad);
    const int n0 = rows + 2 * pad, n1 = cols + 2 * pad;
// ... 888 lines not shown
{
    return blur_ch_sigmas_batch_impl(ctx, d_src, d_dst, 1, rows, cols, channels, sigmas, opts);
}

int blur_gaussian_f32_sigmas_host(blur_ctx* ctx, const float* src, float* dst, int rows, int cols, int channels, const double* sigmas, const blur_opts* opts)
{
    return blur_ch_sigmas_host(ctx, src, dst, rows, cols, channels, sigmas, opts);
}

int blur_gaussian_f32_sigmas_batch_multi_dev(blur_multi* m, const float* d_src, float* d_dst, int nframes, int rows, int cols, int channels, const double* sigmas,
                                             const blur_opts* opts)
{
    return blur_ch_sigmas_multi(m, d_src, d_dst, nframes, rows, cols, channels, sigmas, opts, 1);
}

int blur_gaussian_f32_sigmas_batch_multi_host(blur_multi* m, const float* src, float* dst, int nframes, int rows, int cols, int channels, const double* sigmas,
                                              const blur_opts* opts)
{
    return blur_ch_sigmas_multi(m, src, dst, nframes, rows, cols, channels, sigmas, opts, 0);
}

int blur_gaussian_u16_sigmas_batch_dev(blur_ctx* ctx, const uint16_t* d_src, uint16_t* d_dst, int nframes, int rows, int cols, int channels, const double* sigmas,
                                       const blur_opts* opts)
{
    return blur_ch_sigmas_batch_impl(ctx, d_src, d_dst, nframes, rows, cols, channels, sigmas, opts);
}

int blur_gaussian_u16_sigmas_dev(blur_ctx* ctx, const uint16_t* d_src, uint16_t* d_dst, int rows, int cols, int channels, const double* sigmas, const blur_opts* opts)
{
    return blur_ch_sigmas_batch_impl(ctx, d_src, d_dst, 1, rows, cols, channels, sigmas, opts);
}

int blur_gaussian_u16_sigmas_host(blur_ctx* ctx, const uint16_t* src, uint16_t* dst, int rows, int cols, int channels, const double* sigmas, const blur_opts* opts)
{
    return blur_ch_sigmas_host(ctx, src, dst, rows, cols, channels, sigmas, opts);
}

int blur_gaussian_u16_sigmas_batch_multi_dev(blur_multi* m, const uint16_t* d_src, uint16_t* d_dst, int nframes, int rows, int cols, int channels, const double* sigmas,
                                             const blur_opts* opts)
{
    return blur_ch_sigmas_multi(m, d_src, d_dst, nframes, rows, cols, channels, sigmas, opts, 1);
}

int blur_gaussian_u16_sigmas_batch_multi_host(blur_multi* m, const uint16_t* src, uint16_t* dst, int nframes, int rows, int cols, int channels, const double* sigmas,
                                              const blur_opts* opts)
{
    return blur_ch_sigmas_multi(m, src, dst, nframes, rows, cols, channels, sigmas, opts, 0);
}

int blur_gaussian_f16_sigmas_batch_dev(blur_ctx* ctx, const uint16_t* d_src, uint16_t* d_dst, int nframes, int rows, int cols, int channels, const double* sigmas,
                                       const blur_opts* opts)
{
    return blur_ch_sigmas_batch_impl(ctx, reinterpret_cast<const ff_f16*>(d_src), reinterpret_cast<ff_f16*>(d_dst), nframes, rows, cols, channels, sigmas, opts);
}

int blur_gaussian_f16_sigmas_dev(blur_ctx* ctx, const uint16_t* d_src, uint16_t* d_dst, int rows, int cols, int channels, const double* sigmas, const blur_opts* opts)
{
    return blur_ch_sigmas_batch_impl(ctx, reinterpret_cast<const ff_f16*>(d_src), reinterpret_cast<ff_f16*>(d_dst), 1, rows, cols, channels, sigmas, opts);
}

int blur_gaussian_f16_sigmas_host(blur_ctx* ctx, const uint16_t* src, uint16_t* dst, int rows, int cols, int channels, const double* sigmas, const blur_opts* opts)
{
    return blur_ch_sigmas_host(ctx, reinterpret_cast<const ff_f16*>(src), reinterpret_cast<ff_f16*>(dst), rows, cols, channels, sigmas, opts);
}

int blur_gaussian_f16_sigmas_batch_multi_dev(blur_multi* m, const uint16_t* d_src, uint16_t* d_dst, int nframes, int rows, int cols, int channels, const double* sigmas,
                                             const blur_opts* opts)
{
    return blur_ch_sigmas_multi(m, reinterpret_cast<const ff_f16*>(d_src), reinterpret_cast<ff_f16*>(d_dst), nframes, rows, cols, channels, sigmas, opts, 1);
}

int blur_gaussian_f16_sigmas_batch_multi_host(blur_multi* m, const uint16_t* src, uint16_t* dst, int nframes, int rows, int cols, int channels, const double* sigmas,
                                              const blur_opts* opts)
{
    return blur_ch_sigmas_multi(m, reinterpret_cast<const ff_f16*>(src), reinterpret_cast<ff_f16*>(dst), nframes, rows, cols, channels, sigmas, opts, 0);
}

int blur_gaussian_bf16_sigmas_batch_dev(blur_ctx* ctx, const uint16_t* d_src, uint16_t* d_dst, int nframes, int rows, int cols, int channels, const double* sigmas,
                                        const blur_opts* opts)
{
    return blur_ch_sigmas_batch_impl(ctx, reinterpret_cast<const ff_bf16*>(d_src), reinterpret_cast<ff_bf16*>(d_dst), nframes, rows, cols, channels, sigmas, opts);
}

int blur_gaussian_bf16_sigmas_dev(blur_ctx* ctx, const uint16_t* d_src, uint16_t* d_dst, int rows, int cols, int channels, const double* sigmas, const blur_opts* opts)
{
    return blur_ch_sigmas_batch_impl(ctx, reinterpret_cast<const ff_bf16*>(d_src), reinterpret_cast<ff_bf16*>(d_dst), 1, rows, cols, channels, sigmas, opts);
}

int blur_gaussian_bf16_sigmas_host(blur_ctx* ctx, const uint16_t* src, uint16_t* dst, int rows, int cols, int channels, const double* sigmas, const blur_opts* opts)
{
    return blur_ch_sigmas_host(ctx, reinterpret_cast<const ff_bf16*>(src), reinterpret_cast<ff_bf16*>(dst), rows, cols, channels, sigmas, opts);
}

int blur_gaussian_bf16_sigmas_batch_multi_dev(blur_multi* m, const uint16_t* d_src, uint16_t* d_dst, int nframes, int rows, int cols, int channels, const double* sigmas,
                                              const blur_opts* opts)
{
    return blur_ch_sigmas_multi(m, reinterpret_cast<const ff_bf16*>(d_src), reinterpret_cast<ff_bf16*>(d_dst), nframes, rows, cols, channels, sigmas, opts, 1);
}

int blur_gaussian_bf16_sigmas_batch_multi_host(blur_multi* m, const uint16_t* src, uint16_t* dst, int nframes, int rows, int cols, int channels, const double* sigmas,
                                               const blur_opts* opts)
{
    return blur_ch_sigmas_multi(m, reinterpret_cast<const ff_bf16*>(src), reinterpret_cast<ff_bf16*>(dst), nframes, rows, cols, channels, sigmas, opts, 0);
}

int blur_convolve_lines_c32_dev(blur_ctx* ctx, const float* d_in, float* d_out, int nlines, int n, const float* multipliers)
{
    if (!ctx) return BLUR_ERR_INVALID;
    if (!d_in || !d_out || !multipliers || nlines < 0 || n <= 0) return fail(ctx, BLUR_ERR_INVALID, "null pointer or non-positive size");
    HIP_TRY(ctx, hipSetDevice(ctx->device));
    const WrEntry* e = nullptr;
    for (int role = 0; role < 2 && !e; ++role) {
        const WrEntry* c = find_wr_entry(n, role != 0);
        if (c && c->r0 * kWrS == n) e = c;
    }
    if (!e) return fail(ctx, BLUR_ERR_UNSUPPORTED, "no wave-resident kernel for this length (blur_wr_length)");
    float2* tw0 = nullptr;
    if (int rc = wr_get_tables(ctx, e, &tw0)) return rc;
    constexpr size_t kLinesCacheMax = 16;
    float* d_m = nullptr;
    const uint64_t h = fnv1a(multipliers, sizeof(float) * n);
    for (auto it = ctx->lines_tables.begin(); it != ctx->lines_tables.end(); ++it) {
        if (it->hash == h && static_cast<int>(it->host.size()) == n && std::memcmp(it->host.data(), multipliers, sizeof(float) * n) == 0) {
            d_m = it->dev;
            ctx->lines_tables.splice(ctx->lines_tables.begin(), ctx->lines_tables, it);
            break;
        }
    }
    if (!d_m) {
        if (ctx->lines_tables.size() >= kLinesCacheMax) {
            HIP_TRY(ctx, hipStreamSynchronize(ctx->stream));
            (void)hipFree(ctx->lines_tables.back().dev);
            ctx->lines_tables.pop_back();
        }
        HIP_TRY(ctx, hipMalloc(reinterpret_cast<void**>(&d_m), sizeof(float) * (n + kWrStampTailFloats)));
        if (hipMemset(d_m, 0, sizeof(float) * (n + kWrStampTailFloats)) != hipSuccess ||
            hipMemcpy(d_m, multipliers, sizeof(float) * n, hipMemcpyHostToDevice) != hipSuccess) {
            (void)hipFree(d_m);
            return fail(ctx, BLUR_ERR_HIP, "blur_convolve_lines_c32_dev: table upload failed");
        }
        ctx->lines_tables.push_front({ h, std::vector<float>(multipliers, multipliers + n), d_m });
    }
    HIP_TRY(ctx, e->lines(ctx->stream, reinterpret_cast<const float2*>(d_in), reinterpret_cast<float2*>(d_out), nlines, ctx->num_cus, ctx->d_w256, tw0, d_m));
    return BLUR_OK;
}

int blur_mx_fragments(const float* taps, int pad, int nkb, uint16_t* out)
{
    if (!taps || !out || pad < 0 || nkb < mx_nkb(pad)) return BLUR_ERR_INVALID;
    mx_fragments(taps, pad, nkb, out);
    return BLUR_OK;
}

int blur_mx_window_blocks(int pad)
{
    const MxEntry* e = pad >= 0 ? find_mx_entry(pad) : nullptr;
    return e ? e->nkb : 0;
}

int blur_wr_length(int need, int column_role)
{
    const WrEntry* e = find_wr_entry(need, column_role != 0);
    return e ? e->r0 * kWrS : 0;
}

int blur_debug_last_family(const blur_ctx* ctx) { return ctx ? ctx->last_family : -1; }

int blur_last_engine(const blur_ctx* ctx, char* note, size_t n)
{
    if (!ctx) return -1;
    static const char* const names[] = { "run-time-planned FFT kernels", "specialised rows-first FFT kernels", "wave-resident FFT kernels", "whole-image 2D FFT",
                                         "two-kernel matrix-core engine", "?", "fused matrix-core kernel", "tiled wave-resident FFT kernels" };
    if (note && n > 0) {
        std::string t = ctx->last_family >= 0 && ctx->last_family <= 7 ? names[ctx->last_family] : "none yet";
        if (!ctx->engine_note.empty()) t += " (not taken: " + ctx->engine_note + ")";
        std::snprintf(note, n, "%s", t.c_str());
    }
    return ctx->last_family;
}

int blur_debug_check_workspace_guards(blur_ctx* ctx)
{
    if (!ctx) return -1;
    if (!ctx->work) return -1;
    if (hipSetDevice(ctx->device) != hipSuccess || hipStreamSynchronize(ctx->stream) != hipSuccess) return -1;
    std::vector<unsigned char> g(2 * kWorkGuard);
    const char* base = reinterpret_cast<const char*>(ctx->work) - kWorkGuard;
    if (hipMemcpy(g.data(), base, kWorkGuard, hipMemcpyDeviceToHost) != hipSuccess) return -1;
    if (hipMemcpy(g.data() + kWorkGuard, base + kWorkGuard + ctx->work_bytes, kWorkGuard, hipMemcpyDeviceToHost) != hipSuccess) return -1;
    int bad = 0;
    for (unsigned char c : g) bad += c != 0xA5;
    return bad;
}

int blur_debug_read_stamps(blur_ctx* ctx, int n, int role, unsigned long long* out, int count)
{
    if (!ctx || !out) return BLUR_ERR_INVALID;
    auto it = ctx->last_spectrum.find(role < 0 ? -n : 4 * n + role);
    if (it == ctx->last_spectrum.end() || count * sizeof(unsigned long long) > kStampTailFloats * sizeof(float)) return BLUR_ERR_INVALID;
    HIP_TRY(ctx, hipStreamSynchronize(ctx->stream));
    HIP_TRY(ctx, hipMemcpy(out, it->second + n, count * sizeof(unsigned long long), hipMemcpyDeviceToHost));
    return BLUR_OK;
}

int blur_malloc(blur_ctx* ctx, void** d_ptr, size_t bytes)
{
    if (!ctx || !d_ptr) return BLUR_ERR_INVALID;
    HIP_TRY(ctx, hipSetDevice(ctx->device));
    HIP_TRY(ctx, hipMalloc(d_ptr, bytes ? bytes : 1));
    return BLUR_OK;
}

int blur_host_alloc(blur_ctx* ctx, void** h_ptr, size_t bytes)
{
    if (!ctx || !h_ptr) return BLUR_ERR_INVALID;
    HIP_TRY(ctx, hipSetDevice(ctx->device));
    HIP_TRY(ctx, hipHostMalloc(h_ptr, bytes ? bytes : 1, hipHostMallocDefault));
    return BLUR_OK;
}

int blur_host_free(blur_ctx* ctx, void* h_ptr)
{
    if (!ctx) return BLUR_ERR_INVALID;
    HIP_TRY(ctx, hipHostFree(h_ptr));
    return BLUR_OK;
}

int blur_free(blur_ctx* ctx, void* d_ptr)
{
    if (!ctx) return BLUR_ERR_INVALID;
    HIP_TRY(ctx, hipFree(d_ptr));
    return BLUR_OK;
}

int blur_memcpy_h2d(blur_ctx* ctx, void* d_dst, const void* src, size_t bytes)
{
    if (!ctx) return BLUR_ERR_INVALID;
    HIP_TRY(ctx, hipMemcpyAsync(d_dst, src, bytes, hipMemcpyHostToDevice, ctx->stream));
    HIP_TRY(ctx, hipStreamSynchronize(ctx->stream));
    return BLUR_OK;
}

int blur_memcpy_d2h(blur_ctx* ctx, void* dst, const void* d_src, size_t bytes)
{
    if (!ctx) return BLUR_ERR_INVALID;
    HIP_TRY(ctx, hipMemcpyAsync(dst, d_src, bytes, hipMemcpyDeviceToHost, ctx->stream));
    HIP_TRY(ctx, hipStreamSynchronize(ctx->stream));
    return BLUR_OK;
}

int blur_copy_bandwidth(blur_ctx* ctx, size_t bytes, int reps, double* gbs)
{
    if (!ctx || !gbs || reps <= 0 || bytes < 4096) return BLUR_ERR_INVALID;
    HIP_TRY(ctx, hipSetDevice(ctx->device));
    const size_t n16 = bytes / 16;
    uint4 *a = nullptr, *b = nullptr;
    HIP_TRY(ctx, hipMalloc(reinterpret_cast<void**>(&a), n16 * 16));
    if (hipMalloc(reinterpret_cast<void**>(&b), n16 * 16) != hipSuccess) { (void)hipFree(a); return fail(ctx, BLUR_ERR_NOMEM, "blur_copy_bandwidth: out of device memory"); }
    (void)hipMemsetAsync(a, 0x5a, n16 * 16, ctx->stream);
    hipEvent_t e0 = nullptr, e1 = nullptr;
    (void)hipEventCreate(&e0);
    (void)hipEventCreate(&e1);
    const int grid = ctx->num_cus * 8;
    hipLaunchKernelGGL(copy16_kernel, dim3(grid), dim3(256), 0, ctx->stream, a, b, n16);
    (void)hipEventRecord(e0, ctx->stream);
    for (int i = 0; i < reps; ++i) hipLaunchKernelGGL(copy16_kernel, dim3(grid), dim3(256), 0, ctx->stream, a, b, n16);
    (void)hipEventRecord(e1, ctx->stream);
    hipError_t err = hipEventSynchronize(e1);
    float ms = 0.f;
    if (err == hipSuccess) err = hipEventElapsedTime(&ms, e0, e1);
    (void)hipEventDestroy(e0);
    (void)hipEventDestroy(e1);
    (void)hipFree(a);
    (void)hipFree(b);
    if (err != hipSuccess || !(ms > 0.f)) return fail(ctx, BLUR_ERR_HIP, "blur_copy_bandwidth: timing failed");
    *gbs = 2.0 * static_cast<double>(n16) * 16.0 * reps / (ms * 1e-3) / 1e9;
    return BLUR_OK;
}

}
```

### blur_algorithms_amd/csrc/fx_kernels.hpp

```cpp
#pragma once
#include "mx_kernels.hpp"
#include <atomic>

#if !defined(FX_NO_SGB) && !defined(FX_SGB)
#define FX_SGB 1
#endif
#ifndef FX_SGB_A
#define FX_SGB_A 5
#endif
#ifndef FX_SGB_B
#define FX_SGB_B 6
#endif

namespace blur_amd {

struct FxGeom {
    int rows, cols, pad;
    int nframes;
    int aligned;
    int ntiles;
    int nright;
    int nxcd;
};

constexpr int kFxChunk = 128;
constexpr int kFxMaxBatches = 4;
__host__ __device__ constexpr int fx_left_strips(int pada) { return pada > 0 ? (pada + kFxChunk - 1) / kFxChunk : 1; }
__host__ __device__ inline void fx_strip_range(int xc, int cols, int pada, int per, int* lo, int* hi)
{
    const int x0 = kFxChunk * xc;
    const bool left = x0 - pada < 0, right = x0 + kFxChunk + pada > cols;
    if (left && right) { *lo = 0; *hi = per; }
    else if (left) { const int gl = (pada - x0 + 3) / 4; const int h = (gl + 7) / 8; *lo = 0; *hi = h < per ? h : per; }
    else if (right) { const int gb = (cols - (x0 - pada)) / 4; *lo = gb / 8; *hi = per; }
    else { *lo = 0; *hi = 0; }
}

template <int NKB> struct FxCfg {
    static constexpr int PADA = 8 * (NKB - 2), WIN = kFxChunk + 2 * PADA, GPR = WIN / 4, PER = (GPR + 7) / 8;
    static constexpr int fx_pitch() { int dw = 16 * PER; while ((dw & 7) != 4) ++dw; return 2 * dw; }
    static constexpr int PW = fx_pitch();
    static constexpr int NT = (NKB - 1) / 2;
    static constexpr int BUF = 3 * 32 * PW * 2;
    static constexpr int QOFF = 2 * BUF;
    static constexpr int LDS = QOFF + 2 * 2 * 256 * 4;
};

constexpr float kFxRowUnscale = 1024.f;

__host__ __device__ constexpr uint32_t fx_sel1(int B, int da, int db) { return (B >> 2) == db ? static_cast<uint32_t>(B & 3) : static_cast<uint32_t>(4 + (B & 3)); }

template <int NKB> struct FxRaw { uint32_t d[FxCfg<NKB>::PER][3]; };

__device__ __forceinline__ void fx_swap4(uint32_t& a0, uint32_t& b0, uint32_t& a1, uint32_t& b1, uint32_t& a2, uint32_t& b2, uint32_t& a3, uint32_t& b3)
{
    asm("s_nop 1\n\tv_permlane32_swap_b32 %0, %1\n\tv_permlane32_swap_b32 %2, %3\n\tv_permlane32_swap_b32 %4, %5\n\tv_permlane32_swap_b32 %6, %7"
        : "+v"(a0), "+v"(b0), "+v"(a1), "+v"(b1), "+v"(a2), "+v"(b2), "+v"(a3), "+v"(b3));
}

template <int CTRL> __device__ __forceinline__ uint32_t fx_dpp(uint32_t x)
{
    return static_cast<uint32_t>(__builtin_amdgcn_update_dpp(0, static_cast<int>(x), CTRL, 0xf, 0xf, true));
}

#ifdef FX_ABL_M16
typedef float fx_f4 __attribute__((ext_vector_type(4)));
struct fx_tile { fx_f4 q[4]; };
#define FX_EL(t, i) ((t).q[(i) >> 2][(i) & 3])
#define FX_PIN(t) asm volatile("" : "+a"((t).q[0]), "+a"((t).q[1]), "+a"((t).q[2]), "+a"((t).q[3]))
__device__ __forceinline__ void fx_mma(mx_half8 a, mx_half8 b, fx_tile& t, int pair)
{
    t.q[2 * pair] = __builtin_amdgcn_mfma_f32_16x16x32_f16(a, b, t.q[2 * pair], 0, 0, 0);
    t.q[2 * pair + 1] = __builtin_amdgcn_mfma_f32_16x16x32_f16(a, b, t.q[2 * pair + 1], 0, 0, 0);
}
#else
typedef mx_float16 fx_tile;
#define FX_EL(t, i) ((t)[i])
#define FX_PIN(t) asm volatile("" : "+a"(t))
__device__ __forceinline__ void fx_mma(mx_half8 a, mx_half8 b, fx_tile& t, int) { t = __builtin_amdgcn_mfma_f32_32x32x16_f16(a, b, t, 0, 0, 0); }
#endif

__device__ __forceinline__ uint32_t fx_quad_transpose(uint32_t p, uint32_t sel1, uint32_t sel2)
{
    const uint32_t t = fx_dpp<0xb1>(p);
    const uint32_t q = __builtin_amdgcn_perm(t, p, sel1);
    const uint32_t u = fx_dpp<0x4e>(q);
    return __builtin_amdgcn_perm(u, q, sel2);
}

struct FxQuirk {
    const int* srow_part;
    const int* cpart;
    const long long* zpart;
    const float* taps;
    int nbatches, nbands;
    int cpitch;
    float dr, dc;
};

template <int NCH>
__device__ __forceinline__ void fx_quirk_cols_tile(unsigned char* scratch, float* qc, const FxQuirk& q, int f, int x0, int c0, int cols, int pad, int tid)
{
    const int win = kFxChunk + 2 * pad, nval = NCH * win, ntap = 2 * pad + 1;
    double* cc = reinterpret_cast<double*>(scratch);
    double* tp = cc + nval;
    double* zs = tp + ntap;
    int* S = reinterpret_cast<int*>(zs + 4 + ((nval + ntap) & 1));
    const size_t bstride = static_cast<size_t>(q.cpitch);
    const int wlo = x0 - pad, whi = min(x0 + kFxChunk, cols) + pad;
    int xlo = max(wlo, 0), xhi = min(whi, cols);
    if (wlo < 0) xhi = max(xhi, min(cols, 1 - wlo));
    if (whi > cols) xlo = min(xlo, max(0, 2 * cols - 1 - whi));
    {
        typedef int i4u __attribute__((ext_vector_type(4), aligned(4)));
        typedef int i4 __attribute__((ext_vector_type(4)));
        constexpr int BG = 17;
        const int quads = (3 * (xhi - xlo) + 3) / 4;
        const int* base = q.cpart + static_cast<size_t>(f) * q.nbands * bstride + 3 * xlo;
        for (int qd = tid; qd < quads; qd += 256) {
            const int* cp = base + 4 * qd;
            i4 sum = { 0, 0, 0, 0 };
            for (int b0 = 0; b0 < q.nbands; b0 += BG) {
                i4 t[BG];
#pragma unroll
                for (int j = 0; j < BG; ++j) t[j] = *reinterpret_cast<const i4u*>(cp + static_cast<size_t>(min(b0 + j, q.nbands - 1)) * bstride);
#pragma unroll
                for (int j = 0; j < BG; ++j)
                    if (b0 + j < q.nbands) sum += t[j];
            }
            *reinterpret_cast<i4*>(S + 4 * qd) = sum;
        }
    }
    for (int i = tid; i < ntap; i += 256) tp[i] = static_cast<double>(q.taps[i]);
    {
        const int w = tid >> 6, l = tid & 63, nz = q.nbands * q.nbatches;
        if (w < 3 && (NCH == 3 || w == c0)) {
            const long long* zp = q.zpart + static_cast<size_t>(f) * nz * 3 + w;
            long long z = 0;
            for (int i0 = l; i0 < nz; i0 += 256) {
                long long t[4];
#pragma unroll
                for (int j = 0; j < 4; ++j) t[j] = zp[static_cast<size_t>(min(i0 + 64 * j, nz - 1)) * 3];
#pragma unroll
                for (int j = 0; j < 4; ++j) z += i0 + 64 * j < nz ? t[j] : 0;
            }
            for (int o = 32; o >= 1; o >>= 1) z += __shfl_xor(z, o, 64);
            if (l == 0) zs[w] = static_cast<double>(z);
        }
    }
    __syncthreads();
    for (int i = tid; i < nval; i += 256) {
        const int p = i / NCH, ch = NCH == 3 ? i - 3 * p : c0;
        const int xr = min(max(mx_refl(x0 - pad + p, cols), xlo), xhi - 1);
        cc[i] = static_cast<double>(S[3 * (xr - xlo) + ch]);
    }
    __syncthreads();
    const double sp = (pad & 1) ? -1.0 : 1.0;
    for (int e = tid; e < NCH * kFxChunk; e += 256) {
        const int xl = e / NCH, c = NCH == 3 ? e - 3 * xl : c0, x = x0 + xl;
        float out = 0.f;
        if (x < cols) {
            const double* ccx = cc + NCH * xl + (NCH == 3 ? c : 0);
            double acc[4] = { 0, 0, 0, 0 };
            int t = 0;
            for (; t + 8 <= ntap; t += 8) {
                double a[8], v[8];
#pragma unroll
                for (int j = 0; j < 8; ++j) { a[j] = tp[t + j]; v[j] = ccx[NCH * (t + j)]; }
#pragma unroll
                for (int j = 0; j < 8; ++j) acc[j & 3] = __builtin_fma(a[j], v[j], acc[j & 3]);
            }
            for (; t < ntap; ++t) acc[t & 3] = __builtin_fma(tp[t], ccx[NCH * t], acc[t & 3]);
            const double sx = ((x + pad) & 1) ? -1.0 : 1.0;
            out = static_cast<float>(static_cast<double>(q.dc) * sp * (((acc[0] + acc[1]) + (acc[2] + acc[3])) + static_cast<double>(q.dr) * sx * zs[c]));
        }
        qc[e] = out;
    }
    __syncthreads();
}

template <int NKB, bool QUIRK, bool DUMPV = false, bool RAGGED = false>
__global__ __launch_bounds__(256, 1) void fx_blur_u8(const uint8_t* __restrict__ src, uint8_t* __restrict__ dst, const mx_half8* __restrict__ frags, FxGeom g,
                                                     int chunks, int tps, int nseg, int ntasks, FxQuirk qk, const uint8_t* __restrict__ strips,
                                                     float* __restrict__ vdump)
{
    using C = FxCfg<NKB>;
    constexpr int PADA = C::PADA, PW = C::PW, NT = C::NT, PER = C::PER;
    static_assert(PER <= 9, "three staging chunks of three 12-byte groups");
    extern __shared__ __attribute__((aligned(16))) unsigned char fx_lds[];
    const int tid = threadIdx.x, lane = tid & 63, wave = tid >> 6, m = lane & 31, h = lane >> 5;

    const int nx = g.nxcd, xcd = blockIdx.x % nx, in_xcd = blockIdx.x / nx, per_xcd = (ntasks + nx - 1) / nx, task = xcd * per_xcd + in_xcd;
    if (in_xcd >= per_xcd || task >= ntasks) return;
    const int xc = task % chunks, seg = (task / chunks) % nseg, f = task / (chunks * nseg);
    const int x0 = xc * kFxChunk;
    const int tile0 = seg * tps, tile1 = min(tile0 + tps, g.ntiles);
    const uint8_t* img = src + static_cast<size_t>(f) * g.rows * g.cols * 3;
    uint8_t* out = dst + static_cast<size_t>(f) * g.rows * g.cols * 3;

    mx_half8 th[NKB], tl[NKB];
#pragma unroll
    for (int kb = 0; kb < NKB; ++kb) {
        th[kb] = frags[kb * 64 + lane];
        tl[kb] = frags[(NKB + kb) * 64 + lane];
    }

    const uint32_t sel1 = (lane & 1) ? 0x03070105u : 0x06020400u, sel2 = (lane & 2) ? 0x03020706u : 0x05040100u;
    const int Q = m >> 2, q = m & 3;
    const int xpix = x0 + 32 * wave + 4 * Q;
    const bool in_cols = xpix + 3 < g.cols;
    const int tail_bytes = RAGGED && !in_cols && xpix < g.cols ? 3 * (g.cols - xpix) : 0;
    float cpos[3], cneg[3];
    const int qrows = 32 * (g.ntiles + NT);
    const double qrs = QUIRK ? static_cast<double>(qk.dr) * ((g.pad & 1) ? -1.0 : 1.0) : 0.0;

#ifdef FX_ABL_M16
    const fx_f4 zero4 = { 0.f, 0.f, 0.f, 0.f };
    const fx_tile zero = { { zero4, zero4, zero4, zero4 } };
#else
    const fx_tile zero = { 0.f, 0.f, 0.f, 0.f, 0.f, 0.f, 0.f, 0.f, 0.f, 0.f, 0.f, 0.f, 0.f, 0.f, 0.f, 0.f };
#endif
    fx_tile acc[3][NT];
#pragma unroll
    for (int c = 0; c < 3; ++c)
#pragma unroll
        for (int k = 0; k < NT; ++k) acc[c][k] = zero;
    fx_tile arow = zero;
    uint32_t hl[2][8];
    uint32_t rr[3][4];

    const int s0 = tile0, s1 = tile1 + NT;
    FxRaw<NKB> raw;
    int qpart[kFxMaxBatches] = {};
    constexpr int NLEFT = fx_left_strips(PADA);
    const int sidx = xc < NLEFT ? xc : (xc >= chunks - g.nright ? NLEFT + xc - (chunks - g.nright) : -1);
    int ka_lo = 0, ka_hi = 0;
#ifdef FX_FULL_STRIPS
    if (sidx >= 0) ka_hi = PER;
#else
    if (sidx >= 0) fx_strip_range(xc, g.cols, PADA, PER, &ka_lo, &ka_hi);
#endif
    const uint32_t pitch_s = 3u * C::WIN, pitch_i = 3u * static_cast<uint32_t>(g.cols);
    const uint8_t* ibase = img + 3 * (x0 - PADA);
    const uint32_t ibytes = (static_cast<uint32_t>(g.rows) * g.cols - static_cast<uint32_t>(x0 - PADA)) * 3u;
    const __amdgpu_buffer_rsrc_t rimg = __builtin_amdgcn_make_buffer_rsrc(const_cast<uint8_t*>(ibase), 0, ibytes, kMxRsrcWord3);
    const __amdgpu_buffer_rsrc_t rstrip = sidx >= 0 ? __builtin_amdgcn_make_buffer_rsrc(const_cast<uint8_t*>(strips + (static_cast<size_t>(f) * (NLEFT + g.nright) + sidx) * g.rows * (3 * C::WIN)),
                                                                                        0, static_cast<uint32_t>(g.rows) * 3u * C::WIN, kMxRsrcWord3) : rimg;
#ifdef FX_STAGE_LINEAR
    const int srow = tid >> 3;
#else
    const int srow = 8 * (tid >> 6) + ((tid >> 4) & 3) + 4 * ((tid >> 3) & 1);
#endif
    auto issue_chunk = [&](int s, int j) __attribute__((always_inline)) {
        const int row = srow, g0 = tid & 7;
#ifdef FX_ABL_NOLOAD
        if (s >= 0) return;
#endif
        const int r = mx_refl(32 * s - PADA + row, g.rows);
        const uint32_t off_i = static_cast<uint32_t>(r) * pitch_i + 12u * g0, off_s = static_cast<uint32_t>(r) * pitch_s + 12u * g0;
        typedef uint32_t u3 __attribute__((ext_vector_type(3)));
#pragma unroll
        for (int k = 3 * j; k < 3 * j + 3 && k < PER; ++k) {
            const bool in = (C::GPR % 8 == 0) || k < PER - 1 || g0 < C::GPR % 8;
            const bool from_strip = k >= ka_lo && k < ka_hi;
            const uint32_t off = from_strip ? off_s : off_i;
            const u3 t = __builtin_amdgcn_raw_buffer_load_b96(from_strip ? rstrip : rimg, off + 96u * (in ? k : (k > 0 ? k - 1 : 0)), 0, 0);
            raw.d[k][0] = t[0]; raw.d[k][1] = t[1]; raw.d[k][2] = t[2];
        }
        if (QUIRK && j == 0) {
            const int c = min(tid >> 5, 2), re = min(32 * s + (tid & 31), qrows - 1);
            const int* sp = qk.srow_part + (static_cast<size_t>(f) * qk.nbatches * g.rows + mx_refl(re - PADA, g.rows)) * 3 + c;
#pragma unroll
            for (int b = 0; b < kFxMaxBatches; ++b) qpart[b] = sp[static_cast<size_t>(min(b, qk.nbatches - 1)) * g.rows * 3];
        }
    };
    auto commit_item = [&](int buf, int k, int c) __attribute__((always_inline)) {
#ifdef FX_ABL_NOCOMMIT
        if (buf >= 0) return;
#endif
        const int row = srow, g0 = tid & 7;
        if (k >= PER) return;
        {
            _Float16* base = reinterpret_cast<_Float16*>(fx_lds + buf * C::BUF) + row * PW + 4 * g0;
            auto pick = [&](int B0, int B1) __attribute__((always_inline)) {
                const int da = B1 >> 2, db = B0 >> 2;
                const uint32_t sel = fx_sel1(B0, da, db) | (0x0cu << 8) | (fx_sel1(B1, da, db) << 16) | (0x0cu << 24);
                return __builtin_amdgcn_perm(raw.d[k][da], raw.d[k][db], sel);
            };
            uint2 wd;
#ifdef FX_ABL_NOPERM
            wd.x = raw.d[k][c]; wd.y = raw.d[k][(c + 1) % 3];
#else
            wd.x = pick(c, 3 + c);
            wd.y = pick(6 + c, 9 + c);
#endif
#ifdef FX_ABL_NODSWRITE
            asm volatile("" ::"v"(wd.x), "v"(wd.y));
#else
            *reinterpret_cast<uint2*>(base + c * 32 * PW + 32 * k) = wd;
#endif
        }
    };
    auto commit_q = [&](int buf) __attribute__((always_inline)) {
        if (QUIRK) {
            int v = qpart[0];
#pragma unroll
            for (int b = 1; b < kFxMaxBatches; ++b) v += b < qk.nbatches ? qpart[b] : 0;
            const float qraw = static_cast<float>(qrs * v);
            float* qs = reinterpret_cast<float*>(fx_lds + C::QOFF) + buf * 512 + tid;
            qs[0] = qraw;
            qs[256] = -qraw;
        }
    };
    auto commit_chunk = [&](int buf, int j) __attribute__((always_inline)) {
#pragma unroll
        for (int i = 0; i < 9; ++i) commit_item(buf, 3 * j + i / 3, i % 3);
        if (j == 0) commit_q(buf);
    };
    auto rowpass = [&](int buf, int c, auto beside) __attribute__((always_inline)) {
        const _Float16* base = reinterpret_cast<const _Float16*>(fx_lds + buf * C::BUF) + (c * 32 + m) * PW + wave * 32 + 8 * h;
        fx_tile a = zero;
        mx_half8 x[4];
#pragma unroll
#ifdef FX_ABL_NOXREAD
        for (int kb = 0; kb < 4; ++kb) x[kb] = th[kb];
#else
        for (int kb = 0; kb < 3 && kb < NKB; ++kb) x[kb] = *reinterpret_cast<const mx_half8*>(base + 16 * kb);
#endif
#pragma unroll
        for (int kb = 0; kb < NKB; ++kb) {
#ifndef FX_ABL_NOXREAD
            if (kb + 3 < NKB) x[(kb + 3) & 3] = *reinterpret_cast<const mx_half8*>(base + 16 * (kb + 3));
#endif
            fx_mma(x[kb & 3], th[kb], a, 0);
            fx_mma(x[kb & 3], tl[kb], a, 1);
            FX_PIN(a);
            beside(kb);
#ifdef FX_SGB
            __builtin_amdgcn_sched_group_barrier(0x100, 1, 0);
            __builtin_amdgcn_sched_group_barrier(0x008, 1, 0);
            __builtin_amdgcn_sched_group_barrier(0x002, FX_SGB_A, 0);
            __builtin_amdgcn_sched_group_barrier(0x008, 1, 0);
            __builtin_amdgcn_sched_group_barrier(0x002, FX_SGB_A, 0);
#endif
#ifndef FX_NOSB
            __builtin_amdgcn_sched_barrier(0);
#endif
        }
        arow = a;
    };
    float sv[16];
    auto split_piece = [&](int buf, int c, int piece, int sprod = 0) __attribute__((always_inline)) {
        const int hf = piece / 4, sub = piece % 4;
        uint32_t (&hp)[8] = hl[0];
        uint32_t (&lp)[8] = hl[1];
#ifdef FX_ABL_NOSPLIT
        if (sub == 0) {
#pragma unroll
            for (int k = 0; k < 4; ++k) { hp[4 * hf + k] = __builtin_bit_cast(uint32_t, FX_EL(arow, 8 * hf + k)); lp[4 * hf + k] = __builtin_bit_cast(uint32_t, FX_EL(arow, 8 * hf + 4 + k)); }
        }
        return;
#endif
        if (sub == 0) {
            if (QUIRK) {
                const float* qs4 = reinterpret_cast<const float*>(fx_lds + C::QOFF) + buf * 512 + (m & 1) * 256 + c * 32 + 4 * h;
#pragma unroll
                for (int k = 0; k < 2; ++k) {
                    const float4 t4 = *reinterpret_cast<const float4*>(qs4 + 8 * (2 * hf + k));
                    sv[8 * hf + 4 * k] = __builtin_fmaf(FX_EL(arow, 8 * hf + 4 * k), kFxRowUnscale, t4.x);
                    sv[8 * hf + 4 * k + 1] = __builtin_fmaf(FX_EL(arow, 8 * hf + 4 * k + 1), kFxRowUnscale, t4.y);
                    sv[8 * hf + 4 * k + 2] = __builtin_fmaf(FX_EL(arow, 8 * hf + 4 * k + 2), kFxRowUnscale, t4.z);
                    sv[8 * hf + 4 * k + 3] = __builtin_fmaf(FX_EL(arow, 8 * hf + 4 * k + 3), kFxRowUnscale, t4.w);
                }
            } else {
#pragma unroll
                for (int k = 0; k < 8; ++k) sv[8 * hf + k] = FX_EL(arow, 8 * hf + k) * kFxRowUnscale;
            }
            if (DUMPV) {
                const int x = x0 + 32 * wave + m;
#pragma unroll
                for (int k = 0; k < 8; ++k) {
                    const int reg = 8 * hf + k, r = 32 * sprod + (reg & 3) + 8 * (reg >> 2) + 4 * h - PADA;
                    if (r >= 0 && r < g.rows && x < g.cols) vdump[((static_cast<size_t>(f) * 3 + c) * g.rows + r) * g.cols + x] = sv[8 * hf + k];
                }
            }
        } else if (sub == 1 || sub == 2) {
#pragma unroll
            for (int k = 2 * (sub - 1); k < 2 * sub; ++k) {
                typedef float f2 __attribute__((ext_vector_type(2)));
                typedef _Float16 h2 __attribute__((ext_vector_type(2)));
                const f2 vv = { sv[8 * hf + 2 * k], sv[8 * hf + 2 * k + 1] };
                hp[4 * hf + k] = __builtin_bit_cast(uint32_t, __builtin_convertvector(vv, h2));
                float r0, r1;
                mx_remainder(hp[4 * hf + k], vv[0], vv[1], r0, r1);
                const f2 rem = { r0, r1 };
                lp[4 * hf + k] = __builtin_bit_cast(uint32_t, __builtin_convertvector(rem, h2));
            }
        } else {
#ifndef FX_ABL_NOSWAP
            fx_swap4(hp[4 * hf], hp[4 * hf + 2], hp[4 * hf + 1], hp[4 * hf + 3], lp[4 * hf], lp[4 * hf + 2], lp[4 * hf + 1], lp[4 * hf + 3]);
#endif
        }
    };
    fx_tile tfin = zero;
    auto emit_piece = [&](int c, int gq) __attribute__((always_inline)) {
#ifdef FX_ABL_NOEMIT
        rr[c][gq] = __builtin_bit_cast(uint32_t, FX_EL(tfin, 5 * gq));
        return;
#endif
        float fv[4];
#pragma unroll
        for (int k = 0; k < 4; ++k) {
            const int reg = 4 * gq + k;
            fv[k] = __builtin_fmaf(FX_EL(tfin, reg), kMxUnscale, (reg & 1) ? cneg[c] : cpos[c]);
        }
        uint32_t pk = static_cast<uint32_t>(static_cast<int>(fv[0]));
        asm("v_cvt_i32_f32_sdwa %0, %1 dst_sel:BYTE_1 dst_unused:UNUSED_PRESERVE src0_sel:DWORD" : "+v"(pk) : "v"(fv[1]));
        asm("v_cvt_i32_f32_sdwa %0, %1 dst_sel:BYTE_2 dst_unused:UNUSED_PRESERVE src0_sel:DWORD" : "+v"(pk) : "v"(fv[2]));
        asm("v_cvt_i32_f32_sdwa %0, %1 dst_sel:BYTE_3 dst_unused:UNUSED_PRESERVE src0_sel:DWORD" : "+v"(pk) : "v"(fv[3]));
        rr[c][gq] = fx_quad_transpose(pk, sel1, sel2);
    };
    auto colpass = [&](int c, int qs, int ri, auto beside) __attribute__((always_inline)) {
        typedef uint32_t u4 __attribute__((ext_vector_type(4)));
        mx_half8 v1[2], v2[2];
#pragma unroll
        for (int b = 0; b < 2; ++b) {
            const u4 w1 = { hl[0][4 * b], hl[0][4 * b + 1], hl[0][4 * b + 2], hl[0][4 * b + 3] };
            const u4 w2 = { hl[1][4 * b], hl[1][4 * b + 1], hl[1][4 * b + 2], hl[1][4 * b + 3] };
            v1[b] = __builtin_bit_cast(mx_half8, w1);
            v2[b] = __builtin_bit_cast(mx_half8, w2);
        }
#pragma unroll
        for (int it = 0; it < NKB; ++it) {
            const int d = it == 0 ? NKB - 1 : (it >= NKB - 2 ? it - (NKB - 2) : it + 1);
            const int b = d & 1, a2 = d >> 1, slot = (qs - a2 + 2 * NT) % NT;
            if (ri < 0 || a2 <= ri) {
                fx_tile t = d == 0 ? zero : acc[c][slot];
                fx_mma(th[d], v1[b], t, 0);
                fx_mma(tl[d], v1[b], t, 1);
                fx_mma(th[d], v2[b], t, 0);
                FX_PIN(t);
                if (it == 0) tfin = t; else acc[c][slot] = t;
            }
            beside(it);
#ifdef FX_SGB
            __builtin_amdgcn_sched_group_barrier(0x008, 1, 0);
            __builtin_amdgcn_sched_group_barrier(0x002, FX_SGB_B, 0);
            __builtin_amdgcn_sched_group_barrier(0x008, 1, 0);
            __builtin_amdgcn_sched_group_barrier(0x002, FX_SGB_B, 0);
            __builtin_amdgcn_sched_group_barrier(0x008, 1, 0);
            __builtin_amdgcn_sched_group_barrier(0x002, FX_SGB_B, 0);
#endif
#ifndef FX_NOSB
            __builtin_amdgcn_sched_barrier(0);
#endif
        }
    };
    const __amdgpu_buffer_rsrc_t rout = __builtin_amdgcn_make_buffer_rsrc(out, 0, static_cast<uint32_t>(g.rows) * g.cols * 3u, kMxRsrcWord3);
    const uint32_t lane_out = (static_cast<uint32_t>(4 * h + q) * g.cols + static_cast<uint32_t>(xpix)) * 3u;
    auto store_group = [&](int tile, bool valid, int gq) __attribute__((always_inline)) {
        {
            const uint32_t r0 = rr[0][gq], r1 = rr[1][gq], r2 = rr[2][gq];
            const uint32_t X = __builtin_amdgcn_perm(r1, r0, 0x05010400u);
            const uint32_t Y = __builtin_amdgcn_perm(r1, r0, 0x07030602u);
            const uint32_t w0 = __builtin_amdgcn_perm(r2, X, 0x02040100u);
            const uint32_t Z = __builtin_amdgcn_perm(r2, X, 0x0c0c0503u);
            const uint32_t w1 = __builtin_amdgcn_perm(Y, Z, 0x05040100u);
            const uint32_t w2 = __builtin_amdgcn_perm(r2, Y, 0x07030206u);
            typedef uint32_t u3 __attribute__((ext_vector_type(3)));
            const u3 w = { w0, w1, w2 };
            const uint32_t rowoff = static_cast<uint32_t>(32 * tile + 8 * gq) * g.cols * 3u;
#ifdef FX_ABL_NOSTORE
            const bool ok = false;
#else
            const bool ok = valid && in_cols && 32 * tile + 8 * gq + 4 * h + q < g.rows;
#endif
            __builtin_amdgcn_raw_buffer_store_b96(w, rout, ok ? lane_out + rowoff : 0xfffffff0u, 0, 0);
            if (RAGGED) {
                const bool rok = valid && 32 * tile + 8 * gq + 4 * h + q < g.rows;
#pragma unroll
                for (int b = 0; b < 9; ++b) {
                    const uint32_t word = b < 4 ? w0 : (b < 8 ? w1 : w2);
                    __builtin_amdgcn_raw_buffer_store_b8(static_cast<uint8_t>(word >> (8 * (b & 3))), rout, (rok && b < tail_bytes) ? lane_out + rowoff + b : 0xfffffff0u, 0, 0);
                }
            }
        }
    };
    auto store_tile = [&](int tile, bool valid) __attribute__((always_inline)) {
#pragma unroll
        for (int gq = 0; gq < 4; ++gq) store_group(tile, valid, gq);
    };

#pragma unroll
    for (int j = 0; j < 3; ++j) issue_chunk(s0, j);
    if (QUIRK) {
        static_assert(C::BUF >= 8 * (3 * C::WIN + 2 * PADA + 1 + 6) + 4 * (3 * C::WIN + 4), "fx_quirk_cols_tile's scratch fits window buffer 0");
        float* qc = reinterpret_cast<float*>(fx_lds + C::BUF);
        fx_quirk_cols_tile<3>(fx_lds, qc, qk, f, x0, 0, g.cols, g.pad, tid);
#pragma unroll
        for (int c = 0; c < 3; ++c) {
            const float v = qc[3 * (32 * wave + m) + c];
            cpos[c] = 0.5f + v;
            cneg[c] = 0.5f - v;
        }
        __syncthreads();
    } else {
#pragma unroll
        for (int c = 0; c < 3; ++c) cpos[c] = cneg[c] = 0.5f;
    }
#pragma unroll
    for (int j = 0; j < 3; ++j) commit_chunk(0, j);
    issue_chunk(s0 + 1, 0);
    commit_chunk(1, 0);
    issue_chunk(s0 + 1, 1);
    issue_chunk(s0 + 1, 2);
    issue_chunk(s0 + 2, 0);
    __syncthreads();
    rowpass(0, 0, [](int) {});
    split_piece(0, 0, 0, s0);
    split_piece(0, 0, 4, s0);

#ifdef FX_STAMPS
    unsigned long long st_acc[6] = { 0, 0, 0, 0, 0, 0 }, st_prev = __builtin_amdgcn_s_memtime(), st_begin = st_prev;
#define FX_STAMP(i) { const unsigned long long t_ = __builtin_amdgcn_s_memtime(); st_acc[i] += t_ - st_prev; st_prev = t_; }
#else
#define FX_STAMP(i)
#endif
    auto step = [&](int s, int qs, int ri) __attribute__((always_inline)) {
        {
            const int cur = (s - s0) & 1;
#pragma unroll
            for (int c = 0; c < 3; ++c) {
#ifndef FX_ABL_NOBARRIER
                if (c == 2) __syncthreads();
#endif
#ifndef FX_NOSB
                __builtin_amdgcn_sched_barrier(0);
#endif
                {
                    const int jc = c == 2 ? 0 : c + 1, cbuf = c == 2 ? cur : cur ^ 1, snext = c == 2 ? s + 3 : s + 2;
                    const bool tvalid = s - 1 - NT >= tile0 && s > s0;
                    constexpr int NI = NKB >= 11 ? 1 : (NKB >= 6 ? 2 : (NKB >= 4 ? 3 : 5));
                    auto beside = [&](int kb) __attribute__((always_inline)) {
                        if (NKB >= 11) {
                            if (kb == 0) split_piece(cur, c, 1);
                            if (kb == 1) split_piece(cur, c, 2);
                            if (kb == 2) { split_piece(cur, c, 3); split_piece(cur, c, 5); }
                            if (kb == 3) split_piece(cur, c, 6);
                            if (kb == 4) split_piece(cur, c, 7);
                            if (c == 0 && kb >= 5 && kb <= 8) store_group(s - 1 - NT, tvalid, kb - 5);
#ifdef FX_NO_BALANCE
                            if (kb >= 2) commit_item(cbuf, 3 * jc + (kb - 2) / 3, (kb - 2) % 3);
                            if (kb == NKB - 1) { if (jc == 0) commit_q(cbuf); issue_chunk(snext, jc); }
#else
                            (void)jc; (void)cbuf; (void)snext;
#endif
                        } else {
                            if (kb == 0) { split_piece(cur, c, 1); split_piece(cur, c, 2); split_piece(cur, c, 3); split_piece(cur, c, 5); split_piece(cur, c, 6); split_piece(cur, c, 7); }
#pragma unroll
                            for (int i = NI * kb; i < NI * kb + NI && i < 9; ++i) commit_item(cbuf, 3 * jc + i / 3, i % 3);
                            if (kb == NKB - 1) { if (jc == 0) commit_q(cbuf); issue_chunk(snext, jc); }
                            if (c == 0 && kb == NKB - 1) store_tile(s - 1 - NT, tvalid);
                        }
                    };
                    if (c == 2) rowpass(cur ^ 1, 0, beside); else rowpass(cur, c + 1, beside);
                }
#ifndef FX_NOSB
                __builtin_amdgcn_sched_barrier(0);
#endif
                FX_STAMP(2 * c)
                {
                    const int nbuf = c == 2 ? cur ^ 1 : cur, nc = c == 2 ? 0 : c + 1;
                    auto beside = [&](int it) __attribute__((always_inline)) {
                        if (NKB >= 11) {
                            if (it == 1) split_piece(nbuf, nc, 0, c == 2 ? s + 1 : s);
                            if (it == 2) split_piece(nbuf, nc, 4, c == 2 ? s + 1 : s);
                            if (it >= 3 && it <= 6) emit_piece(c, it - 3);
#ifndef FX_NO_BALANCE
                            {
                                const int jc = c == 2 ? 0 : c + 1, cbuf = c == 2 ? cur : cur ^ 1, snext = c == 2 ? s + 3 : s + 2;
                                const int sl = it == 0 ? 0 : it - 6;
                                if (it == 0 || it >= 7) {
                                    commit_item(cbuf, 3 * jc + (2 * sl) / 3, (2 * sl) % 3);
                                    if (sl < 4) commit_item(cbuf, 3 * jc + (2 * sl + 1) / 3, (2 * sl + 1) % 3);
                                }
                                if (it == NKB - 1) { if (jc == 0) commit_q(cbuf); issue_chunk(snext, jc); }
                            }
#endif
                        } else {
                            if (it == (NKB >= 5 ? 1 : 0)) { split_piece(nbuf, nc, 0, c == 2 ? s + 1 : s); split_piece(nbuf, nc, 4, c == 2 ? s + 1 : s); }
                            if (it == (NKB >= 5 ? NKB - 3 : 0)) {
#pragma unroll
                                for (int gq = 0; gq < 4; ++gq) emit_piece(c, gq);
                            }
                        }
                    };
                    colpass(c, qs, ri, beside);
                }
#ifndef FX_NOSB
                __builtin_amdgcn_sched_barrier(0);
#endif
                FX_STAMP(2 * c + 1)
            }
        }
    };
#ifndef FX_NO_PEEL
#pragma unroll
    for (int j = 0; j < NT; ++j) step(s0 + j, j, j);
    for (int sb = s0 + NT; sb < s1; sb += NT) {
#else
    for (int sb = s0; sb < s1; sb += NT) {
#endif
#pragma unroll
        for (int qs = 0; qs < NT; ++qs) {
            const int s = sb + qs;
            if (s >= s1) break;
            step(s, qs, -1);
        }
    }
    store_tile(s1 - 1 - NT, s1 - 1 - NT >= tile0);
#ifdef FX_STAMPS
    if (!QUIRK && !DUMPV && vdump && blockIdx.x == 0 && tid == 0) {
        unsigned long long* o = reinterpret_cast<unsigned long long*>(vdump);
        for (int i = 0; i < 6; ++i) o[i] = st_acc[i];
        o[6] = __builtin_amdgcn_s_memtime() - st_begin;
        o[7] = static_cast<unsigned long long>(s1 - s0);
    }
#endif
}

#ifdef BLUR_FX_QUIRK_KERNELS
inline int fx_right_strips(int cols, int pada)
{
    const int chunks = (cols + kFxChunk - 1) / kFxChunk;
    int n = 0;
    for (int xc = chunks - 1; xc >= fx_left_strips(pada) && kFxChunk * xc + kFxChunk + pada > cols; --xc) ++n;
    return n;
}

__device__ __forceinline__ void fx_edge_strips_body(const uint8_t* __restrict__ src, uint8_t* __restrict__ strips, int rows, int cols, int pada, int chunks, int nright,
                                                    int bx, int sidx, int f, int narrow)
{
    const int win = kFxChunk + 2 * pada, gpr = win / 4;
    const int nleft = fx_left_strips(pada);
    const int xc = sidx < nleft ? sidx : chunks - nright + sidx - nleft, x0 = kFxChunk * xc;
    int glo = 0, gn = gpr;
    if (narrow) {
        int lo, hi;
        fx_strip_range(xc, cols, pada, (gpr + 7) / 8, &lo, &hi);
        glo = 8 * lo;
        gn = min(8 * hi, gpr) - glo;
    }
    const int i = bx * 256 + threadIdx.x, rq = (rows + 3) / 4;
    if (i >= rq * gn) return;
    const int r4 = i / gn, gidx = glo + i - r4 * gn;
    const int X = x0 - pada + 4 * gidx;
    const bool mir = X < 0 || X >= cols;
    const int xs = X < 0 ? -X - 3 : (X >= cols ? 2 * cols - 5 - X : X);
    const bool fast = xs >= 0 && xs + 3 < cols;
    typedef uint32_t u3 __attribute__((ext_vector_type(3)));
    const uint8_t* img = src + static_cast<size_t>(f) * rows * cols * 3;
    uint8_t* sbase = strips + (static_cast<size_t>(f) * (nleft + nright) + sidx) * rows * (3 * win) + 12 * gidx;
    u3 d[4];
    if (fast) {
#pragma unroll
        for (int k = 0; k < 4; ++k) d[k] = *reinterpret_cast<const u3*>(img + (static_cast<size_t>(min(4 * r4 + k, rows - 1)) * cols + xs) * 3);
    }
#pragma unroll
    for (int k = 0; k < 4; ++k) {
        const int r = 4 * r4 + k;
        if (r >= rows) break;
        u3 o;
        if (fast) {
            o = d[k];
            if (mir) {
                o[0] = __builtin_amdgcn_perm(d[k][2], d[k][1], 0x02070605u);
                o[1] = (d[k][1] >> 24) | ((d[k][2] & 0xffu) << 8) | ((d[k][0] >> 24) << 16) | ((d[k][1] & 0xffu) << 24);
                o[2] = __builtin_amdgcn_perm(d[k][1], d[k][0], 0x02010005u);
            }
        } else {
            const uint8_t* line = img + static_cast<size_t>(r) * cols * 3;
            uint32_t b[12];
#pragma unroll
            for (int qd = 0; qd < 4; ++qd) {
                const uint8_t* px = line + 3 * mx_refl(X + qd, cols);
                b[3 * qd] = px[0]; b[3 * qd + 1] = px[1]; b[3 * qd + 2] = px[2];
            }
            o[0] = b[0] | (b[1] << 8) | (b[2] << 16) | (b[3] << 24);
            o[1] = b[4] | (b[5] << 8) | (b[6] << 16) | (b[7] << 24);
            o[2] = b[8] | (b[9] << 8) | (b[10] << 16) | (b[11] << 24);
        }
        *reinterpret_cast<u3*>(sbase + static_cast<size_t>(r) * (3 * win)) = o;
    }
}

constexpr int kFxSumRows = 32;
inline int fx_groups_per_thread(int cols)
{
    const int groups = (cols + 3) / 4;
    for (int g = 1; g <= 4; g *= 2)
        if (groups <= 256 * g * kFxMaxBatches) return g;
    return 0;
}
inline int fx_band_rows(int rows, int cols, int nframes, int num_cus)
{
    if (static_cast<long long>(rows) * cols < 4000000ll) return 16;
    const int gpt = fx_groups_per_thread(cols);
    const long long nbatches = ((cols + 3) / 4 + 256 * gpt - 1) / (256 * (gpt > 0 ? gpt : 1));
    int br = kFxSumRows;
#ifndef FX_BAND_WGS
#define FX_BAND_WGS 4
#endif
    while (br < 128 && nbatches * ((rows + 2 * br - 1) / (2 * br)) * nframes >= static_cast<long long>(FX_BAND_WGS) * num_cus) br *= 2;
    return br;
}

template <int G>
__device__ __forceinline__ void fx_altsums_body(const uint8_t* __restrict__ src, int* __restrict__ srow_part, int* __restrict__ cpart, long long* __restrict__ zpart,
                                                int rows, int cols, int pad, int nbands, int nbatches, int band, int batch, int f, int (*sred)[3][64], int band_rows)
{
    const int tid = threadIdx.x;
    const uint8_t* img = src + static_cast<size_t>(f) * rows * cols * 3;
    const __amdgpu_buffer_rsrc_t rimg = __builtin_amdgcn_make_buffer_rsrc(const_cast<uint8_t*>(img), 0, static_cast<uint32_t>(rows) * cols * 3u, kMxRsrcWord3);
    const int groups = (cols + 3) / 4, r0 = band * band_rows, r1 = min(r0 + band_rows, rows);
    const int flip = (pad & 1) ? -1 : 1;
    const int over = (4 - (cols & 3)) & 3;
    int gi[G], wq[G][4];
    bool act[G], plain[G], last[G];
    uint32_t col0[G];
#pragma unroll
    for (int j = 0; j < G; ++j) {
        gi[j] = (batch * G + j) * 256 + tid;
        act[j] = gi[j] < groups;
        last[j] = over != 0 && gi[j] == groups - 1;
        const int x = 4 * gi[j] - (last[j] ? over : 0);
        plain[j] = !last[j] && x > pad && x + 3 < cols - 1 - pad;
#pragma unroll
        for (int q = 0; q < 4; ++q) wq[j][q] = (act[j] && !(last[j] && q < over)) ? mx_alt_weight(x + q, cols, pad) : 0;
        col0[j] = act[j] ? 3u * static_cast<uint32_t>(x) : 0u;
    }
    int o[G][12];
#pragma unroll
    for (int j = 0; j < G; ++j)
#pragma unroll
        for (int k = 0; k < 12; ++k) o[j][k] = 0;
    long long zacc = 0;
    typedef uint32_t u3 __attribute__((ext_vector_type(3)));
    for (int rs = r0; rs < r1; rs += kFxSumRows) {
        const int re = min(rs + kFxSumRows, r1);
        for (int i = tid; i < kFxSumRows * 3 * 64; i += 256) (&sred[0][0][0])[i] = 0;
        __syncthreads();
        uint32_t accp[G][6], accn[G][6];
#pragma unroll
        for (int j = 0; j < G; ++j)
#pragma unroll
            for (int k = 0; k < 6; ++k) accp[j][k] = accn[j][k] = 0;
#ifndef FX_PRE_RB
#define FX_PRE_RB 8
#endif
        constexpr int RB = G == 1 ? FX_PRE_RB : (G == 2 ? 4 : 2);
        for (int rb = rs; rb < re; rb += RB) {
            u3 d[RB][G];
#pragma unroll
            for (int i = 0; i < RB; ++i) {
                const int r = min(rb + i, re - 1);
#pragma unroll
                for (int j = 0; j < G; ++j) d[i][j] = __builtin_amdgcn_raw_buffer_load_b96(rimg, col0[j] + static_cast<uint32_t>(r) * static_cast<uint32_t>(cols) * 3u, 0, 0);
            }
#pragma unroll
            for (int i = 0; i < RB; ++i) {
                const int r = rb + i;
                if (r < re) {
                    const int wy = mx_alt_weight(r, rows, pad);
                    const uint32_t aw = static_cast<uint32_t>(wy < 0 ? -wy : wy);
                    int s[3] = { 0, 0, 0 };
#pragma unroll
                    for (int j = 0; j < G; ++j) {
                        const u3 dd = d[i][j];
                        if (plain[j]) {
                            const int e0 = static_cast<int>(dd[0] ^ 0x80808080u), e1 = static_cast<int>(dd[1] ^ 0x80808080u), e2 = static_cast<int>(dd[2] ^ 0x80808080u);
                            int t0 = __builtin_amdgcn_sdot4(e0, static_cast<int>(0xff000001u), 0, false);
                            t0 = __builtin_amdgcn_sdot4(e1, 0x00010000, t0, false);
                            t0 = __builtin_amdgcn_sdot4(e2, 0x0000ff00, t0, false);
                            int t1 = __builtin_amdgcn_sdot4(e0, 0x00000100, 0, false);
                            t1 = __builtin_amdgcn_sdot4(e1, 0x010000ff, t1, false);
                            t1 = __builtin_amdgcn_sdot4(e2, 0x00ff0000, t1, false);
                            int t2 = __builtin_amdgcn_sdot4(e0, 0x00010000, 0, false);
                            t2 = __builtin_amdgcn_sdot4(e1, 0x0000ff00, t2, false);
                            t2 = __builtin_amdgcn_sdot4(e2, static_cast<int>(0xff000001u), t2, false);
                            s[0] += flip * t0; s[1] += flip * t1; s[2] += flip * t2;
                        } else {
#pragma unroll
                            for (int q = 0; q < 4; ++q)
#pragma unroll
                                for (int c = 0; c < 3; ++c) {
                                    const int byte = 3 * q + c;
                                    s[c] += wq[j][q] * static_cast<int>((dd[byte >> 2] >> (8 * (byte & 3))) & 0xffu);
                                }
                        }
#pragma unroll
                        for (int k = 0; k < 3; ++k) {
                            uint32_t lo = __builtin_amdgcn_perm(0u, dd[k], 0x0c020c00u), hi = __builtin_amdgcn_perm(0u, dd[k], 0x0c030c01u);
                            if (aw != 1) { lo *= aw; hi *= aw; }
                            if (wy > 0) { accp[j][2 * k] += lo; accp[j][2 * k + 1] += hi; }
                            else { accn[j][2 * k] += lo; accn[j][2 * k + 1] += hi; }
                        }
                    }
#pragma unroll
                    for (int c = 0; c < 3; ++c) atomicAdd(&sred[r - rs][c][tid & 63], s[c]);
                }
            }
        }
#pragma unroll
        for (int j = 0; j < G; ++j)
#pragma unroll
            for (int k = 0; k < 3; ++k) {
                o[j][4 * k] += static_cast<int>(accp[j][2 * k] & 0xffffu) - static_cast<int>(accn[j][2 * k] & 0xffffu);
                o[j][4 * k + 2] += static_cast<int>(accp[j][2 * k] >> 16) - static_cast<int>(accn[j][2 * k] >> 16);
                o[j][4 * k + 1] += static_cast<int>(accp[j][2 * k + 1] & 0xffffu) - static_cast<int>(accn[j][2 * k + 1] & 0xffffu);
                o[j][4 * k + 3] += static_cast<int>(accp[j][2 * k + 1] >> 16) - static_cast<int>(accn[j][2 * k + 1] >> 16);
            }
        __syncthreads();
        if (tid < (re - rs) * 3) {
            const int* p64 = &sred[0][0][0] + 64 * tid;
            int v = 0;
#pragma unroll 8
            for (int k = 0; k < 64; ++k) v += p64[(k + tid) & 63];
            srow_part[((static_cast<size_t>(f) * nbatches + batch) * rows + rs) * 3 + tid] = v;
            zacc += static_cast<long long>(mx_alt_weight(rs + tid / 3, rows, pad)) * v;
        }
        __syncthreads();
    }
    if (over != 0) {
#pragma unroll
        for (int j = 0; j < G; ++j)
#pragma unroll
            for (int k = 0; k < 9; ++k) {
                const int v3 = o[j][k + 3], v6 = k + 6 < 12 ? o[j][k + 6] : 0, v9 = k + 9 < 12 ? o[j][k + 9] : 0;
                o[j][k] = last[j] ? (over == 1 ? v3 : (over == 2 ? v6 : v9)) : o[j][k];
            }
    }
#pragma unroll
    for (int j = 0; j < G; ++j)
        if (act[j]) {
            int4* dstp = reinterpret_cast<int4*>(cpart + (static_cast<size_t>(f) * nbands + band) * (12 * static_cast<size_t>(groups)) + 12 * gi[j]);
            dstp[0] = make_int4(o[j][0], o[j][1], o[j][2], o[j][3]);
            dstp[1] = make_int4(o[j][4], o[j][5], o[j][6], o[j][7]);
            dstp[2] = make_int4(o[j][8], o[j][9], o[j][10], o[j][11]);
        }
    long long* zs = reinterpret_cast<long long*>(&sred[0][0][0]);
    if (tid < 96) zs[tid] = zacc;
    __syncthreads();
    if (tid < 3) {
        long long z = 0;
        for (int k = 0; k < kFxSumRows; ++k) z += zs[3 * k + tid];
        zpart[((static_cast<size_t>(f) * nbands + band) * nbatches + batch) * 3 + tid] = z;
    }
}

template <int G>
__global__ __launch_bounds__(256) void fx_prepass(const uint8_t* __restrict__ src, int* __restrict__ srow_part, int* __restrict__ cpart, long long* __restrict__ zpart,
                                                  uint8_t* __restrict__ strips, int rows, int cols, int pad, int pada, int nbands, int nbatches, int n_alt, int chunks,
                                                  int nright, int strip_blocks, int band_rows, int narrow)
{
    __shared__ int sred[kFxSumRows][3][64];
    int b = blockIdx.x;
    if (b < n_alt) {
        const int band = b % nbands, batch = (b / nbands) % nbatches, f = b / (nbands * nbatches);
        fx_altsums_body<G>(src, srow_part, cpart, zpart, rows, cols, pad, nbands, nbatches, band, batch, f, sred, band_rows);
    } else {
        b -= n_alt;
        const int nstrips = fx_left_strips(pada) + nright, bx = b % strip_blocks, sidx = (b / strip_blocks) % nstrips, f = b / (strip_blocks * nstrips);
        fx_edge_strips_body(src, strips, rows, cols, pada, chunks, nright, bx, sidx, f, narrow);
    }
}
#endif

struct FxLaunch {
    int chunks = 0, nseg = 1, tps = 0;
    long long ntasks = 0;
    dim3 grid;
};
inline FxLaunch fx_plan_launch(FxGeom& g, int nch, int nt, int num_cus)
{
    FxLaunch l;
    l.chunks = (g.cols + kFxChunk - 1) / kFxChunk;
    const long long nstripes = static_cast<long long>(l.chunks) * g.nframes * nch;
    if (nstripes <= 0) return l;
    l.tps = g.ntiles;
    long long best = -1;
    for (int n = 1; n <= g.ntiles; ++n) {
        const int t = (g.ntiles + n - 1) / n, ns = (g.ntiles + t - 1) / t;
        const long long rounds = (nstripes * ns + num_cus - 1) / num_cus, span = rounds * (t + nt);
        if (best < 0 || span < best) { best = span; l.nseg = ns; l.tps = t; }
    }
    l.ntasks = nstripes * l.nseg;
    if (g.nxcd < 1) g.nxcd = 1;
    const int per_xcd = static_cast<int>((l.ntasks + g.nxcd - 1) / g.nxcd);
    l.grid = dim3(static_cast<unsigned>(g.nxcd * per_xcd));
    return l;
}

template <class... K> hipError_t fx_set_lds(std::atomic<unsigned long long>& done, int lds, K... kernels)
{
    int dev = -1;
    const bool known = hipGetDevice(&dev) == hipSuccess && dev >= 0 && dev < 64;
    if (known && ((done.load(std::memory_order_acquire) >> dev) & 1ull)) return hipSuccess;
    for (const void* k : { reinterpret_cast<const void*>(kernels)... }) {
        const hipError_t e = hipFuncSetAttribute(k, hipFuncAttributeMaxDynamicSharedMemorySize, lds);
        if (e != hipSuccess) return e;
    }
    if (known) done.fetch_or(1ull << dev, std::memory_order_release);
    return hipSuccess;
}

struct FxEntry {
    int nkb;
    hipError_t (*blur_u8)(hipStream_t, const uint8_t* src, uint8_t* dst, const void* frags, FxGeom g, int num_cus, const FxQuirk* qk, const uint8_t* strips,
                          float* vdump, unsigned long long* stamps);
};

template <int NKB> hipError_t fx_launch_u8(hipStream_t st, const uint8_t* src, uint8_t* dst, const void* frags, FxGeom g, int num_cus, const FxQuirk* qk,
                                           const uint8_t* strips, float* vdump, unsigned long long* stamps)
{
    using C = FxCfg<NKB>;
    const FxLaunch l = fx_plan_launch(g, 1, C::NT, num_cus);
    if (l.ntasks == 0) return hipSuccess;
    static std::atomic<unsigned long long> attr_done{ 0 };
    const hipError_t e = fx_set_lds(attr_done, C::LDS, fx_blur_u8<NKB, true, false>, fx_blur_u8<NKB, false, false>, fx_blur_u8<NKB, true, true>,
                                    fx_blur_u8<NKB, false, true>, fx_blur_u8<NKB, true, false, true>, fx_blur_u8<NKB, false, false, true>);
    if (e != hipSuccess) return e;
#define FX_LAUNCH(Q_, D_, R_)                                                                                                                              \
    hipLaunchKernelGGL((fx_blur_u8<NKB, Q_, D_, R_>), l.grid, dim3(256), C::LDS, st, src, dst, static_cast<const mx_half8*>(frags), g, l.chunks, l.tps, \
                       l.nseg, static_cast<int>(l.ntasks), qk ? *qk : FxQuirk{}, strips, vdump ? vdump : reinterpret_cast<float*>(stamps))
    const bool ragged = (g.cols & 3) != 0;
    if (vdump) {
        if (ragged) return hipErrorNotSupported;
        if (qk) FX_LAUNCH(true, true, false); else FX_LAUNCH(false, true, false);
    } else if (ragged) { if (qk) FX_LAUNCH(true, false, true); else FX_LAUNCH(false, false, true); }
    else { if (qk) FX_LAUNCH(true, false, false); else FX_LAUNCH(false, false, false); }
#undef FX_LAUNCH
    return hipGetLastError();
}

#define BLUR_FX(NKB_)                                                                                       \
    namespace blur_amd {                                                                                    \
    const FxEntry* fx_entry_##NKB_()                                                                        \
    {                                                                                                       \
        static const FxEntry e = { NKB_, fx_launch_u8<NKB_> };                                              \
        return &e;                                                                                          \
    }                                                                                                       \
    }

}
```

### blur_algorithms_amd/csrc/host_math.cpp

```cpp
#include "host_math.hpp"

#include <algorithm>
#include <cmath>
#include <cstring>
#include <numeric>

namespace blur_amd {

int gaussian_window(double sigma, int max_width)
{
    const float radius = static_cast<float>(sigma * std::sqrt(2 * std::log(255)) - 1);
    int width = static_cast<int>(radius * 2 + .5f);
    if (max_width) width = std::min(width, max_width);
    return width | 1;
}

void get_gaussian(float* kernel, double sigma, int width, int fft_length)
{
    if (!width) width = gaussian_window(sigma);
    const int len = fft_length ? fft_length : width;
    const double two_s2 = 2. * sigma * sigma;
    const double norm = 3.14159265358979323846 * two_s2;
    const float half = (width - 1) / 2.f;
    std::vector<float> taps(width);
// ... 153 lines not shown
    while (c5 > 0) { out.push_back(5); --c5; }
    while (c3 >= 2) { out.push_back(9); c3 -= 2; }
    while (c3 > 0 && c2 > 0 && c2 % 4 != 0) { out.push_back(6); --c3; --c2; }
    while (c3 > 0) { out.push_back(3); --c3; }
    while (c2 >= 4) { out.push_back(16); c2 -= 4; }
    if (c2 == 3) out.push_back(8);
    if (c2 == 2) out.push_back(4);
    if (c2 == 1) out.push_back(2);
    std::sort(out.begin(), out.end(), std::greater<int>());
}

bool make_plan(int n, FftPlan& p)
{
    std::vector<int> rad;
    choose_radices(n, rad);
    if (n < 2 || rad.empty()) return false;
    return make_plan_radices(n, rad.data(), static_cast<int>(rad.size()), p);
}

bool make_plan_radices(int n, const int* radices, int npass, FftPlan& p)
{
    if (n < 2 || npass < 1 || npass > kMaxPasses) return false;
    long long prod = 1;
    for (int i = 0; i < npass; ++i) prod *= radices[i];
    if (prod != n) return false;
    const std::vector<int> rad(radices, radices + npass);
    p = FftPlan{};
    p.n = n;
    p.npass = static_cast<int>(rad.size());
    const long double two_pi = 6.283185307179586476925286766559L;
    int len = n, off = 0;
    for (int i = 0; i < p.npass; ++i) {
        const int R = rad[i], m = len / R;
        p.radix[i] = R;
        p.m[i] = m;
        p.tw_off[i] = off;
        if (m > 1) {
            p.tw.resize(static_cast<size_t>(off + (R - 1) * m) * 2);
            for (int q = 1; q < R; ++q)
                for (int j = 0; j < m; ++j) {
                    const long double a = -two_pi * static_cast<long double>((static_cast<long long>(j) * q) % len) / len;
                    const size_t e = static_cast<size_t>(off + (q - 1) * m + j) * 2;
                    p.tw[e] = static_cast<float>(cosl(a));
                    p.tw[e + 1] = static_cast<float>(sinl(a));
                }
            off += (R - 1) * m;
        }
        len = m;
    }
    p.freq_of_pos.resize(n);
    for (int pos = 0; pos < n; ++pos) {
        int rem = pos, f = 0, w = 1;
        for (int i = 0; i < p.npass; ++i) {
            const int q = rem / p.m[i];
            rem -= q * p.m[i];
            f += q * w;
            w *= p.radix[i];
        }
        p.freq_of_pos[pos] = f;
    }
    return true;
}

void permuted_multipliers(const FftPlan& plan, const float* m, bool quirk, float* mperm)
{
    const int n = plan.n;
    for (int pos = 0; pos < n; ++pos) {
        int f = plan.freq_of_pos[pos];
        if (f > n / 2) f = n - f;
        if (quirk && f == n / 2) f = 0;
        mperm[pos] = m[f];
    }
}

void wr_w256(float* w256)
{
    const long double two_pi = 6.283185307179586476925286766559L;
    for (int m = 0; m < 256; ++m) {
        const long double a = -two_pi * m / 256;
        w256[2 * m] = static_cast<float>(cosl(a));
        w256[2 * m + 1] = static_cast<float>(sinl(a));
    }
}

void wr_tw0(int r0, float* tw0)
{
    const long double two_pi = 6.283185307179586476925286766559L;
    const int n = 256 * r0;
    for (int q = 1; q < r0; ++q)
        for (int j = 0; j < 256; ++j) {
            const long double a = -two_pi * static_cast<long double>((j * q) % n) / n;
            const size_t e = static_cast<size_t>((q - 1) * 256 + j) * 2;
            tw0[e] = static_cast<float>(cosl(a));
            tw0[e + 1] = static_cast<float>(sinl(a));
        }
}

void wr_multipliers(const float* karr, int n, int n_ref, bool quirk, float* mult)
{
    const long double two_pi = 6.283185307179586476925286766559L;
    std::vector<int> nz;
    for (int i = 0; i < n; ++i) if (karr[i] != 0.f) nz.push_back(i);
    long double k0 = 0, kalt = 0;
    for (int i : nz) { k0 += karr[i]; kalt += (i & 1) ? -static_cast<long double>(karr[i]) : static_cast<long double>(karr[i]); }
    for (int f = 0; f <= n / 2; ++f) {
        long double acc = 0;
        for (int i : nz) acc += static_cast<long double>(karr[i]) * cosl(two_pi * static_cast<long double>((static_cast<long long>(f) * i) % n) / n);
        if (quirk && f == n / 2) acc = kalt + (k0 - kalt) * static_cast<long double>(n) / n_ref;
        mult[f] = static_cast<float>(acc / n);
        if (f > 0 && f < n / 2) mult[n - f] = mult[f];
    }
}

uint16_t f32_to_f16(float f)
{
    uint32_t x;
    std::memcpy(&x, &f, 4);
    const uint32_t sign = (x >> 16) & 0x8000u;
    x &= 0x7fffffffu;
    if (x >= 0x7f800000u) return static_cast<uint16_t>(sign | 0x7c00u | (x > 0x7f800000u ? 0x200u : 0));
    if (x >= 0x477ff000u) return static_cast<uint16_t>(sign | 0x7c00u);
    if (x < 0x33000001u) return static_cast<uint16_t>(sign);
    const int e = static_cast<int>(x >> 23) - 127;
    uint32_t mant = (x & 0x7fffffu) | 0x800000u;
    int shift;
    uint32_t base;
    if (e >= -14) { shift = 13; base = static_cast<uint32_t>(e + 15) << 10; mant &= 0x7fffffu; }
    else { shift = 13 + (-14 - e); base = 0; }
    const uint32_t kept = mant >> shift, rem = mant & ((1u << shift) - 1), half = 1u << (shift - 1);
    uint32_t h = base + kept;
    if (rem > half || (rem == half && (kept & 1u))) ++h;
    return static_cast<uint16_t>(sign | h);
}

float f16_to_f32(uint16_t h)
{
    const uint32_t sign = static_cast<uint32_t>(h & 0x8000u) << 16;
    const uint32_t e = (h >> 10) & 0x1fu, m = h & 0x3ffu;
    uint32_t x;
    if (e == 0) {
        if (m == 0) x = sign;
        else {
            const float v = std::ldexp(static_cast<float>(m), -24);
            std::memcpy(&x, &v, 4);
            x |= sign;
        }
    } else if (e == 31) x = sign | 0x7f800000u | (m << 13);
    else x = sign | ((e + 112) << 23) | (m << 13);
    float f;
    std::memcpy(&f, &x, 4);
    return f;
}

void mx_fragments(const float* taps, int pad, int nkb, uint16_t* out)
{
    const int pada = 8 * (nkb - 2);
    const float scale = std::ldexp(1.f, kMxScaleLog2);
    for (int kb = 0; kb < nkb; ++kb)
        for (int l = 0; l < 64; ++l)
            for (int j = 0; j < 8; ++j) {
                const int w = 16 * kb + 8 * (l >> 5) + j, o = l & 31, t = w - o - pada;
                uint16_t hi = 0, lo = 0;
                if (t >= -pad && t <= pad) {
                    const float v = taps[t + pad] * scale;
                    hi = f32_to_f16(v);
                    lo = f32_to_f16(v - f16_to_f32(hi));
                }
                const size_t e = (static_cast<size_t>(kb) * 64 + l) * 8 + j;
                out[e] = hi;
                out[static_cast<size_t>(nkb) * 512 + e] = lo;
            }
}

}
```

### blur_algorithms_amd/csrc/host_math.hpp

```cpp
#pragma once
#include <cstdint>
#include <vector>

namespace blur_amd {

int gaussian_window(double sigma, int max_width = 0);
void get_gaussian(float* kernel, double sigma, int width, int fft_length);
int is_valid_size(int n);
int nearest_transform_size(int n);

struct Sizing {
    int kSize, pad;
    int n_col;
    int n_row;
    int tz_col, tz_row;
};
Sizing pffft_sizing(int rows, int cols, double sigma);

struct Sizing2D {
    int kSize, pad;
    int s0, s1;
    int top, bottom, left, right;
};
Sizing2D pocketfft2d_sizing(int rows, int cols, double sigma);

void kernel_multipliers(double sigma, int ksize, int n, float* m);

void box_kernel_1d(float* kernel, int klen, int n);
void boxfft_sizing(int rows, int cols, double nsmooth, int& klen, int& pad);
void kernel_multipliers_from_array(const float* k, int n, float* m);

constexpr int kMaxPasses = 8;
struct FftPlan {
    int n = 0;
    int npass = 0;
    int radix[kMaxPasses] = {};
    int m[kMaxPasses] = {};
    int tw_off[kMaxPasses] = {};
    std::vector<float> tw;
    std::vector<int> freq_of_pos;
};
bool make_plan(int n, FftPlan& plan);
bool make_plan_radices(int n, const int* radices, int npass, FftPlan& plan);

void permuted_multipliers(const FftPlan& plan, const float* m, bool quirk, float* mperm);

void wr_w256(float* w256);
void wr_tw0(int r0, float* tw0);
void wr_multipliers(const float* karr, int n, int n_ref, bool quirk, float* mult);

uint16_t f32_to_f16(float f);
float f16_to_f32(uint16_t h);
constexpr int kMxScaleLog2 = 14;
inline int mx_pada(int pad) { return (pad + 7) & ~7; }
inline int mx_nkb(int pad) { return 2 + mx_pada(pad) / 8; }
void mx_fragments(const float* taps, int pad, int nkb, uint16_t* out);

}
```

### include/blur_amd.h

```cpp
#ifndef BLUR_AMD_H
#define BLUR_AMD_H

#include <stddef.h>
#include <stdint.h>

#ifdef __cplusplus
extern "C" {
#endif

#define BLUR_AMD_VERSION 100

enum {
    BLUR_OK = 0,
    BLUR_ERR_INVALID = 1,
    BLUR_ERR_UNSUPPORTED = 2,
    BLUR_ERR_HIP = 3,
    BLUR_ERR_NOMEM = 4
};

typedef struct blur_ctx blur_ctx;

enum blur_engine {
    BLUR_ENGINE_AUTO = 0,
    BLUR_ENGINE_FFT_ROWS_FIRST = 1,
// ... 71 lines not shown
                          const blur_opts* opts);
int blur_gaussian_u16_host(blur_ctx* ctx, const uint16_t* src, uint16_t* dst, int rows, int cols, int channels, double sigma,
                           const blur_opts* opts);

int blur_gaussian_f16_batch_dev(blur_ctx* ctx, const uint16_t* d_src, uint16_t* d_dst, int nframes, int rows, int cols, int channels,
                                double sigma, const blur_opts* opts);
int blur_gaussian_f16_dev(blur_ctx* ctx, const uint16_t* d_src, uint16_t* d_dst, int rows, int cols, int channels, double sigma,
                          const blur_opts* opts);
int blur_gaussian_f16_host(blur_ctx* ctx, const uint16_t* src, uint16_t* dst, int rows, int cols, int channels, double sigma,
                           const blur_opts* opts);
int blur_gaussian_bf16_batch_dev(blur_ctx* ctx, const uint16_t* d_src, uint16_t* d_dst, int nframes, int rows, int cols, int channels,
                                 double sigma, const blur_opts* opts);
int blur_gaussian_bf16_dev(blur_ctx* ctx, const uint16_t* d_src, uint16_t* d_dst, int rows, int cols, int channels, double sigma,
                           const blur_opts* opts);
int blur_gaussian_bf16_host(blur_ctx* ctx, const uint16_t* src, uint16_t* dst, int rows, int cols, int channels, double sigma,
                            const blur_opts* opts);

int blur_gaussian_u8c3_host(blur_ctx* ctx, const uint8_t* src, uint8_t* dst,
                            int rows, int cols, double sigma, const blur_opts* opts);
int blur_gaussian_f32c1_host(blur_ctx* ctx, const float* src, float* dst,
                             int rows, int cols, double sigma, const blur_opts* opts);
int blur_gaussian_u8c3_host_batch(blur_ctx* ctx, const uint8_t* src, uint8_t* dst, int nframes,
                                  int rows, int cols, double sigma, const blur_opts* opts);
int blur_gaussian_u8c3_host_pitched(blur_ctx* ctx, const uint8_t* src, size_t src_pitch, uint8_t* dst, size_t dst_pitch,
                                    int rows, int cols, double sigma, const blur_opts* opts);

int blur_rowpass_u8c3_dev(blur_ctx* ctx, const uint8_t* d_src, float* d_planes,
                          int rows, int cols, double sigma, const blur_opts* opts);


int blur_separable_u8c3_dev(blur_ctx* ctx, const uint8_t* d_src, uint8_t* d_dst, int rows, int cols,
                            const float* taps, int ksize, int pad, const blur_opts* opts);

int blur_boxfft_u8c3_dev(blur_ctx* ctx, const uint8_t* d_src, uint8_t* d_dst, int rows, int cols,
                         double nsmooth, const blur_opts* opts);
int blur_boxfft_sizing(int rows, int cols, double nsmooth, int out[4]);
int blur_box_kernel(float* kernel, int klen, int fft_length);


int blur_pocketfft2d_sizing(int rows, int cols, double sigma, int out[8]);
int blur_pocketfft2d_u8c3_dev(blur_ctx* ctx, const uint8_t* d_src, uint8_t* d_dst, int rows, int cols, double sigma,
                              int dft_image, float* d_planes);
int blur_pocketfft2d_u8c3_host(blur_ctx* ctx, const uint8_t* src, uint8_t* dst, int rows, int cols, double sigma, int dft_image);


int blur_reflect101_u8_dev(blur_ctx* ctx, const uint8_t* d_in, uint8_t* d_out, int rows, int cols, int channels,
                           int top, int bottom, int left, int right, int out_size[2]);

int blur_flip_block_f32_dev(blur_ctx* ctx, const float* d_in, float* d_out, int w, int h);

int blur_deinterleave_bgr_u8_f32_dev(blur_ctx* ctx, const uint8_t* d_in, float* d_planes, uint32_t total);
int blur_interleave_bgr_f32_u8_dev(blur_ctx* ctx, const float* d_planes, uint8_t* d_out, uint32_t total);

int blur_fastboxblur_u8_dev(blur_ctx* ctx, uint8_t* d_inout, int w, int h, int channels,
                            int ksize, int passes);
int blur_fastboxblur_u8_host(blur_ctx* ctx, uint8_t* inout, int w, int h, int channels,
                             int ksize, int passes);

int blur_fastboxblur_u8_batch_dev(blur_ctx* ctx, uint8_t* d_inout, int nframes, int w, int h, int channels,
                                  int ksize, int passes);
int blur_fastboxblur_u8_host_batch(blur_ctx* ctx, uint8_t* inout, int nframes, int w, int h, int channels,
                                   int ksize, int passes);
int blur_fastboxblur_batch_plan(int nframes, int w, int h, int channels, int ksize, int passes, int out[4]);

typedef struct blur_multi blur_multi;
int blur_multi_create(blur_multi** out, const int* devices, int ndevices);
int blur_multi_destroy(blur_multi* m);
int blur_multi_shards(const blur_multi* m);
const char* blur_multi_last_error(const blur_multi* m);
int blur_gaussian_u8c3_batch_multi_dev(blur_multi* m, const uint8_t* d_src, uint8_t* d_dst, int nframes, int rows, int cols,
                                       double sigma, const blur_opts* opts);
int blur_gaussian_u8c3_batch_multi_host(blur_multi* m, const uint8_t* src, uint8_t* dst, int nframes, int rows, int cols,
                                        double sigma, const blur_opts* opts);
int blur_gaussian_u8_batch_multi_dev(blur_multi* m, const uint8_t* d_src, uint8_t* d_dst, int nframes, int rows, int cols, int channels,
                                     double sigma, const blur_opts* opts);
int blur_gaussian_u8_batch_multi_host(blur_multi* m, const uint8_t* src, uint8_t* dst, int nframes, int rows, int cols, int channels,
                                      double sigma, const blur_opts* opts);
int blur_gaussian_f32_batch_multi_dev(blur_multi* m, const float* d_src, float* d_dst, int nframes, int rows, int cols, int channels,
                                      double sigma, const blur_opts* opts);
int blur_gaussian_f32_batch_multi_host(blur_multi* m, const float* src, float* dst, int nframes, int rows, int cols, int channels,
                                       double sigma, const blur_opts* opts);
int blur_gaussian_u16_batch_multi_dev(blur_multi* m, const uint16_t* d_src, uint16_t* d_dst, int nframes, int rows, int cols, int channels,
                                      double sigma, const blur_opts* opts);
int blur_gaussian_u16_batch_multi_host(blur_multi* m, const uint16_t* src, uint16_t* dst, int nframes, int rows, int cols, int channels,
                                       double sigma, const blur_opts* opts);
int blur_gaussian_f16_batch_multi_dev(blur_multi* m, const uint16_t* d_src, uint16_t* d_dst, int nframes, int rows, int cols, int channels,
                                      double sigma, const blur_opts* opts);
int blur_gaussian_f16_batch_multi_host(blur_multi* m, const uint16_t* src, uint16_t* dst, int nframes, int rows, int cols, int channels,
                                       double sigma, const blur_opts* opts);
int blur_gaussian_bf16_batch_multi_dev(blur_multi* m, const uint16_t* d_src, uint16_t* d_dst, int nframes, int rows, int cols, int channels,
                                       double sigma, const blur_opts* opts);
int blur_gaussian_bf16_batch_multi_host(blur_multi* m, const uint16_t* src, uint16_t* dst, int nframes, int rows, int cols, int channels,
                                        double sigma, const blur_opts* opts);
int blur_gaussian_u8_sigmas_batch_dev(blur_ctx* ctx, const uint8_t* d_src, uint8_t* d_dst, int nframes, int rows, int cols, int channels,
                                      const double* sigmas, const blur_opts* opts);
int blur_gaussian_u8_sigmas_dev(blur_ctx* ctx, const uint8_t* d_src, uint8_t* d_dst, int rows, int cols, int channels,
                                const double* sigmas, const blur_opts* opts);
int blur_gaussian_u8_sigmas_host(blur_ctx* ctx, const uint8_t* src, uint8_t* dst, int rows, int cols, int channels,
                                 const double* sigmas, const blur_opts* opts);
int blur_gaussian_u8_sigmas_batch_multi_dev(blur_multi* m, const uint8_t* d_src, uint8_t* d_dst, int nframes, int rows, int cols, int channels,
                                            const double* sigmas, const blur_opts* opts);
int blur_gaussian_u8_sigmas_batch_multi_host(blur_multi* m, const uint8_t* src, uint8_t* dst, int nframes, int rows, int cols, int channels,
                                             const double* sigmas, const blur_opts* opts);
int blur_gaussian_f32_sigmas_batch_dev(blur_ctx* ctx, const float* d_src, float* d_dst, int nframes, int rows, int cols, int channels,
                                       const double* sigmas, const blur_opts* opts);
int blur_gaussian_f32_sigmas_dev(blur_ctx* ctx, const float* d_src, float* d_dst, int rows, int cols, int channels,
                                 const double* sigmas, const blur_opts* opts);
int blur_gaussian_f32_sigmas_host(blur_ctx* ctx, const float* src, float* dst, int rows, int cols, int channels,
                                  const double* sigmas, const blur_opts* opts);
int blur_gaussian_f32_sigmas_batch_multi_dev(blur_multi* m, const float* d_src, float* d_dst, int nframes, int rows, int cols, int channels,
                                             const double* sigmas, const blur_opts* opts);
int blur_gaussian_f32_sigmas_batch_multi_host(blur_multi* m, const float* src, float* dst, int nframes, int rows, int cols, int channels,
                                              const double* sigmas, const blur_opts* opts);
int blur_gaussian_u16_sigmas_batch_dev(blur_ctx* ctx, const uint16_t* d_src, uint16_t* d_dst, int nframes, int rows, int cols, int channels,
                                       const double* sigmas, const blur_opts* opts);
int blur_gaussian_u16_sigmas_dev(blur_ctx* ctx, const uint16_t* d_src, uint16_t* d_dst, int rows, int cols, int channels,
                                 const double* sigmas, const blur_opts* opts);
int blur_gaussian_u16_sigmas_host(blur_ctx* ctx, const uint16_t* src, uint16_t* dst, int rows, int cols, int channels,
                                  const double* sigmas, const blur_opts* opts);
int blur_gaussian_u16_sigmas_batch_multi_dev(blur_multi* m, const uint16_t* d_src, uint16_t* d_dst, int nframes, int rows, int cols, int channels,
                                             const double* sigmas, const blur_opts* opts);
int blur_gaussian_u16_sigmas_batch_multi_host(blur_multi* m, const uint16_t* src, uint16_t* dst, int nframes, int rows, int cols, int channels,
                                              const double* sigmas, const blur_opts* opts);
int blur_gaussian_f16_sigmas_batch_dev(blur_ctx* ctx, const uint16_t* d_src, uint16_t* d_dst, int nframes, int rows, int cols, int channels,
                                       const double* sigmas, const blur_opts* opts);
int blur_gaussian_f16_sigmas_dev(blur_ctx* ctx, const uint16_t* d_src, uint16_t* d_dst, int rows, int cols, int channels,
                                 const double* sigmas, const blur_opts* opts);
int blur_gaussian_f16_sigmas_host(blur_ctx* ctx, const uint16_t* src, uint16_t* dst, int rows, int cols, int channels,
                                  const double* sigmas, const blur_opts* opts);
int blur_gaussian_f16_sigmas_batch_multi_dev(blur_multi* m, const uint16_t* d_src, uint16_t* d_dst, int nframes, int rows, int cols, int channels,
                                             const double* sigmas, const blur_opts* opts);
int blur_gaussian_f16_sigmas_batch_multi_host(blur_multi* m, const uint16_t* src, uint16_t* dst, int nframes, int rows, int cols, int channels,
                                              const double* sigmas, const blur_opts* opts);
int blur_gaussian_bf16_sigmas_batch_dev(blur_ctx* ctx, const uint16_t* d_src, uint16_t* d_dst, int nframes, int rows, int cols, int channels,
                                        const double* sigmas, const blur_opts* opts);
int blur_gaussian_bf16_sigmas_dev(blur_ctx* ctx, const uint16_t* d_src, uint16_t* d_dst, int rows, int cols, int channels,
                                  const double* sigmas, const blur_opts* opts);
int blur_gaussian_bf16_sigmas_host(blur_ctx* ctx, const uint16_t* src, uint16_t* dst, int rows, int cols, int channels,
                                   const double* sigmas, const blur_opts* opts);
int blur_gaussian_bf16_sigmas_batch_multi_dev(blur_multi* m, const uint16_t* d_src, uint16_t* d_dst, int nframes, int rows, int cols, int channels,
                                              const double* sigmas, const blur_opts* opts);
int blur_gaussian_bf16_sigmas_batch_multi_host(blur_multi* m, const uint16_t* src, uint16_t* dst, int nframes, int rows, int cols, int channels,
                                               const double* sigmas, const blur_opts* opts);
int blur_gaussian_sigmas_plan(int rows, int cols, int channels, const double* sigmas, int* out);

int blur_fastboxblur_u8_batch_multi_dev(blur_multi* m, uint8_t* d_inout, int nframes, int w, int h, int channels,
                                        int ksize, int passes);
int blur_fastboxblur_u8_batch_multi_host(blur_multi* m, uint8_t* inout, int nframes, int w, int h, int channels,
                                         int ksize, int passes);

int blur_convolve_lines_c32_dev(blur_ctx* ctx, const float* d_in, float* d_out, int nlines, int n, const float* multipliers);
int blur_mx_window_blocks(int pad);
int blur_mx_fragments(const float* taps, int pad, int nkb, uint16_t* out);

int blur_wr_length(int need, int column_role);
int blur_wr_kernel_multipliers(double sigma, int ksize, int n, int n_ref, int quirk, float* m);

int blur_malloc(blur_ctx* ctx, void** d_ptr, size_t bytes);
int blur_free(blur_ctx* ctx, void* d_ptr);
int blur_memcpy_h2d(blur_ctx* ctx, void* d_dst, const void* src, size_t bytes);
int blur_memcpy_d2h(blur_ctx* ctx, void* dst, const void* d_src, size_t bytes);
int blur_host_alloc(blur_ctx* ctx, void** h_ptr, size_t bytes);
int blur_host_free(blur_ctx* ctx, void* h_ptr);

int blur_copy_bandwidth(blur_ctx* ctx, size_t bytes, int reps, double* gbs);

#ifdef __cplusplus
}
#endif
#endif
```

Before: 190,600.

## Tighten fx window origin to pad and skip last k-block MMA with scalar fix

Builds a second fragment table whose window origin is the exact pad instead of the 8-aligned pada, and shifts strip and row offsets to match. When the shift is 7, a TIGHT kernel variant drops the final MFMA k-block. It uses the accumulator slot directly and adds two scalar correction terms, obtained via a permlane32 swap, for the rows the dropped block would have covered. This is meant to save one block of matrix work per tile, at the cost of more template instantiations and an extra fragment table.

```diff
diff --git a/blur_algorithms_amd/_lib.py b/blur_algorithms_amd/_lib.py
--- a/blur_algorithms_amd/_lib.py
+++ b/blur_algorithms_amd/_lib.py
@@ -124,6 +124,8 @@
     "blur_wr_length": (C.c_int, [C.c_int, C.c_int]),
     "blur_mx_window_blocks": (C.c_int, [C.c_int]),
     "blur_mx_fragments": (C.c_int, [_P, C.c_int, C.c_int, _P]),
+    "blur_fx_window_blocks": (C.c_int, [C.c_int]),
+    "blur_fx_fragments": (C.c_int, [_P, C.c_int, C.c_int, _P]),
     "blur_wr_kernel_multipliers": (C.c_int, [C.c_double, C.c_int, C.c_int, C.c_int, C.c_int, _P]),
     "blur_malloc": (C.c_int, [_P, C.POINTER(_P), C.c_size_t]),
     "blur_free": (C.c_int, [_P, _P]),
diff --git a/blur_algorithms_amd/csrc/engine.hip b/blur_algorithms_amd/csrc/engine.hip
--- a/blur_algorithms_amd/csrc/engine.hip
+++ b/blur_algorithms_amd/csrc/engine.hip
@@ -625,6 +625,8 @@
 struct MxTables {
     void* frags_row = nullptr;
     void* frags_col = nullptr;
+    void* frags_fx = nullptr;
+    float fix_a = 0.f, fix_b = 0.f;
     float* taps_row = nullptr;
     float dr = 0.f, dc = 0.f;
 };
@@ -1051,6 +1053,7 @@
     auto release = [&]() {
         if (t.frags_row) (void)hipFree(t.frags_row);
         if (t.frags_col) (void)hipFree(t.frags_col);
+        if (t.frags_fx) (void)hipFree(t.frags_fx);
         if (t.taps_row) (void)hipFree(t.taps_row);
     };
     for (int ax = 0; ax < 2; ++ax) {
@@ -1076,6 +1079,14 @@
         if (e == hipSuccess) {
             (ax ? t.frags_col : t.frags_row) = dfr;
             e = hipMemcpy(dfr, fr.data(), fr.size() * sizeof(uint16_t), hipMemcpyHostToDevice);
+        }
+        if (e == hipSuccess && ax == 0 && nkb <= 11) {
+            mx_fragments(taps.data(), pad, nkb, fr.data(), pad);
+            e = hipMalloc(&t.frags_fx, fr.size() * sizeof(uint16_t));
+            if (e == hipSuccess) e = hipMemcpy(t.frags_fx, fr.data(), fr.size() * sizeof(uint16_t), hipMemcpyHostToDevice);
+            const float scale = std::ldexp(1.f, kMxScaleLog2);
+            t.fix_a = taps[2 * pad] * scale;
+            t.fix_b = pad > 0 ? taps[2 * pad - 1] * scale : 0.f;
         }
         if (e == hipSuccess && ax == 0) {
             e = hipMalloc(reinterpret_cast<void**>(&t.taps_row), taps.size() * sizeof(float));
@@ -2120,7 +2131,7 @@
     for (auto& kv : ctx->wr_tw0) (void)hipFree(kv.second);
     for (auto& kv : ctx->wr_spectra) (void)hipFree(kv.second);
     for (auto& kv : ctx->mx_tables) {
-        (void)hipFree(kv.second.frags_row); (void)hipFree(kv.second.frags_col);
+        (void)hipFree(kv.second.frags_row); (void)hipFree(kv.second.frags_col); (void)hipFree(kv.second.frags_fx);
         (void)hipFree(kv.second.taps_row);
     }
     for (auto& lt : ctx->lines_tables) (void)hipFree(lt.dev);
@@ -2269,10 +2280,15 @@
         d_src = reinterpret_cast<const uint8_t*>(ctx->work);
     }
     const int nkb = p.fx->nkb, pada = 8 * (nkb - 2);
-    FxGeom g{ rows, cols, p.sz.pad, nframes, 0, (rows + 31) / 32, fx_right_strips(cols, pada), ctx->num_xcds };
+    const bool fxk = nkb <= 11 && !chsel;
+    const int org = fxk ? p.sz.pad : pada;
+    FxGeom g{ rows, cols, p.sz.pad, nframes, 0, (rows + 31) / 32, fx_right_strips(cols, org), ctx->num_xcds };
+    g.sh = pada - org;
+    g.fix_a = p.mxt->fix_a;
+    g.fix_b = p.mxt->fix_b;
     g.aligned = ((cols & 3) == 0 && (reinterpret_cast<uintptr_t>(d_src) & 3) == 0 && (reinterpret_cast<uintptr_t>(d_dst) & 3) == 0) ? 1 : 0;
     {
-        const int win = kFxChunk + 2 * pada, nstrips = fx_left_strips(pada) + g.nright;
+        const int win = kFxChunk + 2 * pada, nstrips = fx_left_strips(org) + g.nright;
         const size_t bytes = static_cast<size_t>(nframes) * nstrips * rows * win * 3 + 64;
         if (ctx->fx_strips_bytes < bytes) {
             if (ctx->fx_strips) { HIP_TRY(ctx, hipStreamSynchronize(ctx->stream)); HIP_TRY(ctx, hipFree(ctx->fx_strips)); ctx->fx_strips = nullptr; ctx->fx_strips_bytes = 0; }
@@ -2284,26 +2300,26 @@
 #ifdef FX_FULL_STRIPS
         0;
 #else
-        p.fx->nkb <= 11 && !chsel ? 1 : 0;
+        fxk ? 1 : 0;
 #endif
     int strip_groups = (kFxChunk + 2 * pada) / 4;
     if (narrow) {
-        const int gpr = strip_groups, per = (gpr + 7) / 8, nleft = fx_left_strips(pada);
+        const int gpr = strip_groups, per = (gpr + 7) / 8, nleft = fx_left_strips(org);
         strip_groups = 0;
         for (int si = 0; si < nleft + g.nright; ++si) {
             int lo, hi;
-            fx_strip_range(si < nleft ? si : chunks_x - g.nright + si - nleft, cols, pada, per, &lo, &hi);
+            fx_strip_range(si < nleft ? si : chunks_x - g.nright + si - nleft, cols, org, per, &lo, &hi);
             strip_groups = std::max(strip_groups, std::min(8 * hi, gpr) - 8 * lo);
         }
         if (strip_groups < 1) strip_groups = 1;
     }
     const int strip_blocks = (((rows + 3) / 4) * strip_groups + 255) / 256;
-    const int n_strip = strip_blocks * (fx_left_strips(pada) + g.nright) * nframes;
+    const int n_strip = strip_blocks * (fx_left_strips(org) + g.nright) * nframes;
     FxQuirk qk{};
     if (!p.mx_quirk) {
         TimedLaunch t(ctx, 1, nframes);
         hipLaunchKernelGGL(fx_prepass<1>, dim3(n_strip), dim3(256), 0, ctx->stream, d_src, nullptr, nullptr, nullptr, ctx->fx_strips, rows, cols, p.sz.pad, pada, 1, 1, 0, chunks_x,
-                           g.nright, strip_blocks, kFxSumRows, narrow);
+                           g.nright, strip_blocks, kFxSumRows, narrow, org);
         HIP_TRY(ctx, hipGetLastError());
     }
     if (p.mx_quirk) {
@@ -2326,7 +2342,7 @@
           const int n_alt = nbands * nbatches * nframes;
           auto kern = gpt == 1 ? fx_prepass<1> : (gpt == 2 ? fx_prepass<2> : fx_prepass<4>);
           hipLaunchKernelGGL(kern, dim3(n_alt + n_strip), dim3(256), 0, ctx->stream, d_src, srow, cpart, zpart, ctx->fx_strips, rows, cols, p.sz.pad, pada, nbands,
-                             nbatches, n_alt, chunks_x, g.nright, strip_blocks, band_rows, narrow);
+                             nbatches, n_alt, chunks_x, g.nright, strip_blocks, band_rows, narrow, org);
           HIP_TRY(ctx, hipGetLastError()); }
         qk.srow_part = srow;
         qk.cpart = cpart;
@@ -2351,7 +2367,7 @@
         return BLUR_OK;
     }
     { TimedLaunch t(ctx, 0, nframes);
-      HIP_TRY(ctx, p.fx->blur_u8(ctx->stream, d_src, d_dst, p.mxt->frags_row, g, ctx->num_cus, p.mx_quirk ? &qk : nullptr, ctx->fx_strips, vdump, stamps)); }
+      HIP_TRY(ctx, p.fx->blur_u8(ctx->stream, d_src, d_dst, fxk ? p.mxt->frags_fx : p.mxt->frags_row, g, ctx->num_cus, p.mx_quirk ? &qk : nullptr, ctx->fx_strips, vdump, stamps)); }
     if (stamps) {
         unsigned long long h[8];
         HIP_TRY(ctx, hipStreamSynchronize(ctx->stream));
@@ -2421,7 +2437,7 @@
         if (p.tl_quirk) {
             TimedLaunch t(ctx, 1, 1);
             const int n_alt = nbands * nbatches;
-            hipLaunchKernelGGL(fx_prepass<1>, dim3(n_alt), dim3(256), 0, ctx->stream, src, srow, cpart, zpart, nullptr, rows, cols, pad, 0, nbands, nbatches, n_alt, 1, 0, 1, band_rows, 0);
+            hipLaunchKernelGGL(fx_prepass<1>, dim3(n_alt), dim3(256), 0, ctx->stream, src, srow, cpart, zpart, nullptr, rows, cols, pad, 0, nbands, nbatches, n_alt, 1, 0, 1, band_rows, 0, 0);
             HIP_TRY(ctx, hipGetLastError());
             const int ne = (pitch + 255) / 256, nh = (rows + 255) / 256;
             const size_t lds = (static_cast<size_t>(3) * (256 + 2 * pad) + (2 * pad + 1) + 3 + 3 * 256) * sizeof(double);
@@ -3616,6 +3632,19 @@
     return BLUR_OK;
 }
 
+int blur_fx_window_blocks(int pad)
+{
+    const FxEntry* e = pad >= 0 ? find_fx_entry(pad) : nullptr;
+    return e && e->nkb <= 11 ? e->nkb : 0;
+}
+
+int blur_fx_fragments(const float* taps, int pad, int nkb, uint16_t* out)
+{
+    if (!taps || !out || pad < 0 || nkb < mx_nkb(pad)) return BLUR_ERR_INVALID;
+    mx_fragments(taps, pad, nkb, out, pad);
+    return BLUR_OK;
+}
+
 int blur_mx_window_blocks(int pad)
 {
     const MxEntry* e = pad >= 0 ? find_mx_entry(pad) : nullptr;
diff --git a/blur_algorithms_amd/csrc/fx_kernels.hpp b/blur_algorithms_amd/csrc/fx_kernels.hpp
--- a/blur_algorithms_amd/csrc/fx_kernels.hpp
+++ b/blur_algorithms_amd/csrc/fx_kernels.hpp
@@ -21,6 +21,8 @@
     int ntiles;
     int nright;
     int nxcd;
+    int sh;
+    float fix_a, fix_b;
 };
 
 constexpr int kFxChunk = 128;
@@ -179,7 +181,7 @@
     __syncthreads();
 }
 
-template <int NKB, bool QUIRK, bool DUMPV = false, bool RAGGED = false>
+template <int NKB, bool QUIRK, bool DUMPV = false, bool RAGGED = false, bool TIGHT = false>
 __global__ __launch_bounds__(256, 1) void fx_blur_u8(const uint8_t* __restrict__ src, uint8_t* __restrict__ dst, const mx_half8* __restrict__ frags, FxGeom g,
                                                      int chunks, int tps, int nseg, int ntasks, FxQuirk qk, const uint8_t* __restrict__ strips,
                                                      float* __restrict__ vdump)
@@ -187,6 +189,7 @@
     using C = FxCfg<NKB>;
     constexpr int PADA = C::PADA, PW = C::PW, NT = C::NT, PER = C::PER;
     static_assert(PER <= 9, "three staging chunks of three 12-byte groups");
+    const int ORG = PADA - g.sh;
     extern __shared__ __attribute__((aligned(16))) unsigned char fx_lds[];
     const int tid = threadIdx.x, lane = tid & 63, wave = tid >> 6, m = lane & 31, h = lane >> 5;
 
@@ -238,11 +241,11 @@
 #ifdef FX_FULL_STRIPS
     if (sidx >= 0) ka_hi = PER;
 #else
-    if (sidx >= 0) fx_strip_range(xc, g.cols, PADA, PER, &ka_lo, &ka_hi);
+    if (sidx >= 0) fx_strip_range(xc, g.cols, ORG, PER, &ka_lo, &ka_hi);
 #endif
     const uint32_t pitch_s = 3u * C::WIN, pitch_i = 3u * static_cast<uint32_t>(g.cols);
-    const uint8_t* ibase = img + 3 * (x0 - PADA);
-    const uint32_t ibytes = (static_cast<uint32_t>(g.rows) * g.cols - static_cast<uint32_t>(x0 - PADA)) * 3u;
+    const uint8_t* ibase = img + 3 * (x0 - ORG);
+    const uint32_t ibytes = (static_cast<uint32_t>(g.rows) * g.cols - static_cast<uint32_t>(x0 - ORG)) * 3u;
     const __amdgpu_buffer_rsrc_t rimg = __builtin_amdgcn_make_buffer_rsrc(const_cast<uint8_t*>(ibase), 0, ibytes, kMxRsrcWord3);
     const __amdgpu_buffer_rsrc_t rstrip = sidx >= 0 ? __builtin_amdgcn_make_buffer_rsrc(const_cast<uint8_t*>(strips + (static_cast<size_t>(f) * (NLEFT + g.nright) + sidx) * g.rows * (3 * C::WIN)),
                                                                                         0, static_cast<uint32_t>(g.rows) * 3u * C::WIN, kMxRsrcWord3) : rimg;
@@ -256,7 +259,7 @@
 #ifdef FX_ABL_NOLOAD
         if (s >= 0) return;
 #endif
-        const int r = mx_refl(32 * s - PADA + row, g.rows);
+        const int r = mx_refl(32 * s - ORG + row, g.rows);
         const uint32_t off_i = static_cast<uint32_t>(r) * pitch_i + 12u * g0, off_s = static_cast<uint32_t>(r) * pitch_s + 12u * g0;
         typedef uint32_t u3 __attribute__((ext_vector_type(3)));
 #pragma unroll
@@ -269,7 +272,7 @@
         }
         if (QUIRK && j == 0) {
             const int c = min(tid >> 5, 2), re = min(32 * s + (tid & 31), qrows - 1);
-            const int* sp = qk.srow_part + (static_cast<size_t>(f) * qk.nbatches * g.rows + mx_refl(re - PADA, g.rows)) * 3 + c;
+            const int* sp = qk.srow_part + (static_cast<size_t>(f) * qk.nbatches * g.rows + mx_refl(re - ORG, g.rows)) * 3 + c;
 #pragma unroll
             for (int b = 0; b < kFxMaxBatches; ++b) qpart[b] = sp[static_cast<size_t>(min(b, qk.nbatches - 1)) * g.rows * 3];
         }
@@ -380,7 +383,7 @@
                 const int x = x0 + 32 * wave + m;
 #pragma unroll
                 for (int k = 0; k < 8; ++k) {
-                    const int reg = 8 * hf + k, r = 32 * sprod + (reg & 3) + 8 * (reg >> 2) + 4 * h - PADA;
+                    const int reg = 8 * hf + k, r = 32 * sprod + (reg & 3) + 8 * (reg >> 2) + 4 * h - ORG;
                     if (r >= 0 && r < g.rows && x < g.cols) vdump[((static_cast<size_t>(f) * 3 + c) * g.rows + r) * g.cols + x] = sv[8 * hf + k];
                 }
             }
@@ -402,8 +405,10 @@
 #endif
         }
     };
-    fx_tile tfin = zero;
-    auto emit_piece = [&](int c, int gq) __attribute__((always_inline)) {
+    fx_tile tfin0 = zero;
+    float efix[2] = { 0.f, 0.f };
+    auto emit_piece = [&](int c, int gq, int fs) __attribute__((always_inline)) {
+        const fx_tile& tfin = TIGHT ? acc[c][fs] : tfin0;
 #ifdef FX_ABL_NOEMIT
         rr[c][gq] = __builtin_bit_cast(uint32_t, FX_EL(tfin, 5 * gq));
         return;
@@ -412,7 +417,8 @@
 #pragma unroll
         for (int k = 0; k < 4; ++k) {
             const int reg = 4 * gq + k;
-            fv[k] = __builtin_fmaf(FX_EL(tfin, reg), kMxUnscale, (reg & 1) ? cneg[c] : cpos[c]);
+            const float tv = TIGHT && reg >= 14 ? FX_EL(tfin, reg) + efix[reg - 14] : FX_EL(tfin, reg);
+            fv[k] = __builtin_fmaf(tv, kMxUnscale, (reg & 1) ? cneg[c] : cpos[c]);
         }
         uint32_t pk = static_cast<uint32_t>(static_cast<int>(fv[0]));
         asm("v_cvt_i32_f32_sdwa %0, %1 dst_sel:BYTE_1 dst_unused:UNUSED_PRESERVE src0_sel:DWORD" : "+v"(pk) : "v"(fv[1]));
@@ -434,13 +440,24 @@
         for (int it = 0; it < NKB; ++it) {
             const int d = it == 0 ? NKB - 1 : (it >= NKB - 2 ? it - (NKB - 2) : it + 1);
             const int b = d & 1, a2 = d >> 1, slot = (qs - a2 + 2 * NT) % NT;
+            if (TIGHT && it == 0) {
+                {
+                    uint32_t u0 = 0, u1 = 0, w0 = __builtin_bit_cast(uint32_t, sv[0]), w1 = __builtin_bit_cast(uint32_t, sv[1]);
+                    asm("s_nop 1\n\tv_permlane32_swap_b32 %0, %1\n\tv_permlane32_swap_b32 %2, %3" : "+v"(u0), "+v"(w0), "+v"(u1), "+v"(w1));
+                    const float r0 = __builtin_bit_cast(float, u0), r1 = __builtin_bit_cast(float, u1);
+                    efix[0] = g.fix_a * r0;
+                    efix[1] = __builtin_fmaf(g.fix_a, r1, g.fix_b * r0);
+                    FX_PIN(acc[c][slot]);
+                    emit_piece(c, 3, slot);
+                }
+            } else
             if (ri < 0 || a2 <= ri) {
                 fx_tile t = d == 0 ? zero : acc[c][slot];
                 fx_mma(th[d], v1[b], t, 0);
                 fx_mma(tl[d], v1[b], t, 1);
                 fx_mma(th[d], v2[b], t, 0);
                 FX_PIN(t);
-                if (it == 0) tfin = t; else acc[c][slot] = t;
+                if (it == 0) tfin0 = t; else acc[c][slot] = t;
             }
             beside(it);
 #ifdef FX_SGB
@@ -575,7 +592,7 @@
                         if (NKB >= 11) {
                             if (it == 1) split_piece(nbuf, nc, 0, c == 2 ? s + 1 : s);
                             if (it == 2) split_piece(nbuf, nc, 4, c == 2 ? s + 1 : s);
-                            if (it >= 3 && it <= 6) emit_piece(c, it - 3);
+                            if (it >= 3 && it <= (TIGHT ? 5 : 6)) emit_piece(c, it - 3, qs);
 #ifndef FX_NO_BALANCE
                             {
                                 const int jc = c == 2 ? 0 : c + 1, cbuf = c == 2 ? cur : cur ^ 1, snext = c == 2 ? s + 3 : s + 2;
@@ -591,7 +608,7 @@
                             if (it == (NKB >= 5 ? 1 : 0)) { split_piece(nbuf, nc, 0, c == 2 ? s + 1 : s); split_piece(nbuf, nc, 4, c == 2 ? s + 1 : s); }
                             if (it == (NKB >= 5 ? NKB - 3 : 0)) {
 #pragma unroll
-                                for (int gq = 0; gq < 4; ++gq) emit_piece(c, gq);
+                                for (int gq = 0; gq < (TIGHT ? 3 : 4); ++gq) emit_piece(c, gq, qs);
                             }
                         }
                     };
@@ -639,7 +656,7 @@
 }
 
 __device__ __forceinline__ void fx_edge_strips_body(const uint8_t* __restrict__ src, uint8_t* __restrict__ strips, int rows, int cols, int pada, int chunks, int nright,
-                                                    int bx, int sidx, int f, int narrow)
+                                                    int bx, int sidx, int f, int narrow, int org)
 {
     const int win = kFxChunk + 2 * pada, gpr = win / 4;
     const int nleft = fx_left_strips(pada);
@@ -647,14 +664,14 @@
     int glo = 0, gn = gpr;
     if (narrow) {
         int lo, hi;
-        fx_strip_range(xc, cols, pada, (gpr + 7) / 8, &lo, &hi);
+        fx_strip_range(xc, cols, org, (gpr + 7) / 8, &lo, &hi);
         glo = 8 * lo;
         gn = min(8 * hi, gpr) - glo;
     }
     const int i = bx * 256 + threadIdx.x, rq = (rows + 3) / 4;
     if (i >= rq * gn) return;
     const int r4 = i / gn, gidx = glo + i - r4 * gn;
-    const int X = x0 - pada + 4 * gidx;
+    const int X = x0 - org + 4 * gidx;
     const bool mir = X < 0 || X >= cols;
     const int xs = X < 0 ? -X - 3 : (X >= cols ? 2 * cols - 5 - X : X);
     const bool fast = xs >= 0 && xs + 3 < cols;
@@ -861,7 +878,7 @@
 template <int G>
 __global__ __launch_bounds__(256) void fx_prepass(const uint8_t* __restrict__ src, int* __restrict__ srow_part, int* __restrict__ cpart, long long* __restrict__ zpart,
                                                   uint8_t* __restrict__ strips, int rows, int cols, int pad, int pada, int nbands, int nbatches, int n_alt, int chunks,
-                                                  int nright, int strip_blocks, int band_rows, int narrow)
+                                                  int nright, int strip_blocks, int band_rows, int narrow, int org)
 {
     __shared__ int sred[kFxSumRows][3][64];
     int b = blockIdx.x;
@@ -871,7 +888,7 @@
     } else {
         b -= n_alt;
         const int nstrips = fx_left_strips(pada) + nright, bx = b % strip_blocks, sidx = (b / strip_blocks) % nstrips, f = b / (strip_blocks * nstrips);
-        fx_edge_strips_body(src, strips, rows, cols, pada, chunks, nright, bx, sidx, f, narrow);
+        fx_edge_strips_body(src, strips, rows, cols, pada, chunks, nright, bx, sidx, f, narrow, org);
     }
 }
 #endif
@@ -928,17 +945,26 @@
     if (l.ntasks == 0) return hipSuccess;
     static std::atomic<unsigned long long> attr_done{ 0 };
     const hipError_t e = fx_set_lds(attr_done, C::LDS, fx_blur_u8<NKB, true, false>, fx_blur_u8<NKB, false, false>, fx_blur_u8<NKB, true, true>,
-                                    fx_blur_u8<NKB, false, true>, fx_blur_u8<NKB, true, false, true>, fx_blur_u8<NKB, false, false, true>);
+                                    fx_blur_u8<NKB, false, true>, fx_blur_u8<NKB, true, false, true>, fx_blur_u8<NKB, false, false, true>,
+                                    fx_blur_u8<NKB, true, false, false, true>, fx_blur_u8<NKB, false, false, false, true>,
+                                    fx_blur_u8<NKB, true, false, true, true>, fx_blur_u8<NKB, false, false, true, true>);
     if (e != hipSuccess) return e;
-#define FX_LAUNCH(Q_, D_, R_)                                                                                                                              \
-    hipLaunchKernelGGL((fx_blur_u8<NKB, Q_, D_, R_>), l.grid, dim3(256), C::LDS, st, src, dst, static_cast<const mx_half8*>(frags), g, l.chunks, l.tps, \
+    const bool tight = g.sh == 7 && !vdump;
+#define FX_LAUNCH(Q_, D_, R_, T_)                                                                                                                          \
+    hipLaunchKernelGGL((fx_blur_u8<NKB, Q_, D_, R_, T_>), l.grid, dim3(256), C::LDS, st, src, dst, static_cast<const mx_half8*>(frags), g, l.chunks, l.tps, \
                        l.nseg, static_cast<int>(l.ntasks), qk ? *qk : FxQuirk{}, strips, vdump ? vdump : reinterpret_cast<float*>(stamps))
+#define FX_LAUNCH_QT(D_, R_)                                                                                                                               \
+    do {                                                                                                                                                   \
+        if (tight && !(D_)) { if (qk) FX_LAUNCH(true, false, R_, true); else FX_LAUNCH(false, false, R_, true); }                                         \
+        else { if (qk) FX_LAUNCH(true, D_, R_, false); else FX_LAUNCH(false, D_, R_, false); }                                                            \
+    } while (0)
     const bool ragged = (g.cols & 3) != 0;
     if (vdump) {
         if (ragged) return hipErrorNotSupported;
-        if (qk) FX_LAUNCH(true, true, false); else FX_LAUNCH(false, true, false);
-    } else if (ragged) { if (qk) FX_LAUNCH(true, false, true); else FX_LAUNCH(false, false, true); }
-    else { if (qk) FX_LAUNCH(true, false, false); else FX_LAUNCH(false, false, false); }
+        FX_LAUNCH_QT(true, false);
+    } else if (ragged) FX_LAUNCH_QT(false, true);
+    else FX_LAUNCH_QT(false, false);
+#undef FX_LAUNCH_QT
 #undef FX_LAUNCH
     return hipGetLastError();
 }
diff --git a/blur_algorithms_amd/csrc/host_math.cpp b/blur_algorithms_amd/csrc/host_math.cpp
--- a/blur_algorithms_amd/csrc/host_math.cpp
+++ b/blur_algorithms_amd/csrc/host_math.cpp
@@ -329,9 +329,9 @@
     return f;
 }
 
-void mx_fragments(const float* taps, int pad, int nkb, uint16_t* out)
-{
-    const int pada = 8 * (nkb - 2);
+void mx_fragments(const float* taps, int pad, int nkb, uint16_t* out, int origin)
+{
+    const int pada = origin >= 0 ? origin : 8 * (nkb - 2);
     const float scale = std::ldexp(1.f, kMxScaleLog2);
     for (int kb = 0; kb < nkb; ++kb)
         for (int l = 0; l < 64; ++l)
diff --git a/blur_algorithms_amd/csrc/host_math.hpp b/blur_algorithms_amd/csrc/host_math.hpp
--- a/blur_algorithms_amd/csrc/host_math.hpp
+++ b/blur_algorithms_amd/csrc/host_math.hpp
@@ -54,6 +54,6 @@
 constexpr int kMxScaleLog2 = 14;
 inline int mx_pada(int pad) { return (pad + 7) & ~7; }
 inline int mx_nkb(int pad) { return 2 + mx_pada(pad) / 8; }
-void mx_fragments(const float* taps, int pad, int nkb, uint16_t* out);
+void mx_fragments(const float* taps, int pad, int nkb, uint16_t* out, int origin = -1);
 
 }
diff --git a/include/blur_amd.h b/include/blur_amd.h
--- a/include/blur_amd.h
+++ b/include/blur_amd.h
@@ -247,6 +247,8 @@
 int blur_convolve_lines_c32_dev(blur_ctx* ctx, const float* d_in, float* d_out, int nlines, int n, const float* multipliers);
 int blur_mx_window_blocks(int pad);
 int blur_mx_fragments(const float* taps, int pad, int nkb, uint16_t* out);
+int blur_fx_window_blocks(int pad);
+int blur_fx_fragments(const float* taps, int pad, int nkb, uint16_t* out);
 
 int blur_wr_length(int need, int column_role);
 int blur_wr_kernel_multipliers(double sigma, int ksize, int n, int n_ref, int quirk, float* m);
```

Measured after the change: 186,900. 0.981x the previous value.
